# mcveanlab/mccortex

Measured on AMD Instinct MI355X. Metric: k-mers/s inserted (build), k=31, 50M x 150bp synthetic reads, higher is better.
Workload: dtype u64

## Files before the change

### include/mcx_gpu.h

```cpp
#ifndef MCX_GPU_H_
#define MCX_GPU_H_

#include <stddef.h>
#include <stdint.h>

#ifdef __cplusplus
extern "C" {
#endif

typedef enum {
  MCX_OK = 0,
  MCX_ERR_ARG = -1,
  MCX_ERR_NODEVICE = -2,
  MCX_ERR_NOMEM = -3,
  MCX_ERR_FULL = -4,
  MCX_ERR_HIP = -5,
  MCX_ERR_SINK = -6
} mcx_status;

typedef struct {
  uint64_t num_se_reads;
  uint64_t num_good_reads;
  uint64_t num_bad_reads;
  uint64_t total_bases_read;
// ... 132 lines not shown
  uint64_t num_kmers_found;
} mcx_touch_stats;
int mcx_graph_reads_touch(mcx_graph *g, const uint8_t *bases, const uint64_t *read_offsets, uint64_t nreads,
                          uint8_t *hit , mcx_touch_stats *stats_accum );
int mcx_graph_reads_touch_stream_dev(mcx_graph *g, const void *d_stream, uint64_t nbytes,
                                     const void *d_stream_off , uint64_t nreads, void *d_hit);

enum { MCX_INFER_POP = 1, MCX_INFER_PRESENCE_COVG = 2 };
int mcx_graph_infer_edges(mcx_graph *g, void *recs, uint64_t nrecs, int ncols, uint32_t flags, uint64_t *nmodified);
int mcx_graph_infer_edges_dev(mcx_graph *g, void *d_recs, uint64_t nrecs, int ncols, uint32_t flags, uint64_t *nmodified);

int mcx_graph_kmer_covg(mcx_graph *g, uint64_t *nkmers, uint64_t *sumcov);
int mcx_graph_covg_histogram(mcx_graph *g, uint64_t *hist, uint32_t nbins);

int mcx_graph_checksum(mcx_graph *g, uint64_t *checksum, uint64_t *nkmers);
uint64_t mcx_records_checksum(const void *recs, uint64_t nrecs, int kmer_size, int ncols);

int mcx_ubench_stream(int device, uint64_t bytes, double *copy_gbs, double *read_gbs, double *write_gbs);
int mcx_ubench_random_rmw(int device, uint64_t table_bytes, uint64_t nupdates, double *rmw_per_s,
                          double *load16_per_s, double *load_rmw_per_s);

int mcx_sort_records(void *recs, uint64_t nrecs, int kmer_size, int ncols, int device);
int mcx_records_sorted(const void *recs, uint64_t nrecs, int kmer_size, int ncols, int device,
                       int64_t *first_unsorted);

int mcx_superk_supported(int kmer_size);
int mcx_superk_record_bytes(int kmer_size);
uint32_t mcx_superk_owner(const uint64_t *key_words, int kmer_size, int nparts);
int mcx_graph_superk_layout(mcx_graph *g, int nparts, uint64_t positions_per_call, uint32_t *segs_per_owner,
                            uint64_t *seg_cap);
int mcx_graph_superk_bins_dev(mcx_graph *g, const void *d_stream, uint64_t nbytes, int nparts, void *d_recs,
                              void *d_counts, uint64_t seg_cap);
int mcx_graph_add_superk_dev(mcx_graph *g, int colour, const void *d_recs, const void *d_counts, uint32_t nseg,
                             uint64_t seg_cap, uint64_t kmers_upper_bound);

void mcx_pack_bases(const uint8_t *src, uint64_t n, uint32_t *code, uint16_t *inv);

uint64_t mcx_pack_reads_host(const uint8_t *bases, const uint64_t *off, uint64_t nreads, uint32_t *code,
                             uint16_t *inv, uint64_t cap_pos, int fused);

int mcx_graph_sync(mcx_graph *g);

int mcx_graph_nkmers(mcx_graph *g, uint64_t *n);
int mcx_graph_device_stats(mcx_graph *g, mcx_load_stats *out);

typedef struct {
  uint64_t fallback_inserts;
  uint64_t foreign_inserts;
  uint64_t spilled;
  uint64_t flushes;
} mcx_insert_stats;
int mcx_graph_insert_stats(mcx_graph *g, mcx_insert_stats *out);

void *mcx_graph_stream(mcx_graph *g);

typedef int (*mcx_sink_fn)(void *ctx, const void *records, size_t nbytes);
int mcx_graph_export(mcx_graph *g, int sorted, mcx_sink_fn sink, void *ctx);

enum { MCX_UNITIGS_FASTA = 0, MCX_UNITIGS_GFA = 1, MCX_UNITIGS_DOT = 2 };
enum { MCX_UNITIGS_POINTS = 1 };
#define MCX_UNITIGS_BYTES_PER_KMER 65
#define MCX_UNITIGS_BYTES_PER_UNITIG 170
typedef struct { uint64_t num_unitigs, num_kmers, num_bytes, num_cycles; } mcx_unitigs_stats;
typedef struct {
  uint64_t *keys;
  uint32_t *unitig, *rank;
  uint8_t *orient;
  uint32_t *first, *length;
} mcx_unitigs_arrays;
int mcx_graph_unitigs(mcx_graph *g, int format, uint32_t flags, mcx_sink_fn sink, void *ctx, mcx_unitigs_stats *stats);
int mcx_graph_unitigs_dev(mcx_graph *g, const mcx_unitigs_arrays *out, mcx_unitigs_stats *stats);

void mcx_kmer_from_str(const char *seq, int kmer_size, uint64_t *words_out);
void mcx_kmer_canonical(const uint64_t *words_in, int kmer_size, uint64_t *key_out, int *orient_out);
uint32_t mcx_kmer_hash(const uint64_t *key_words, int kmer_size, uint32_t initval);

#ifdef __cplusplus
}
#endif
#endif
```

### mccortex_amd/csrc/mcx_api.hip

```cpp
#include <hip/hip_runtime.h>

#include <stdarg.h>
#include <stdio.h>
#include <stdlib.h>
#include <string.h>
#include <cstring>

#include <rocprim/device/device_radix_sort.hpp>
#include <rocprim/device/device_scan.hpp>

#include <algorithm>
#include <array>
#include <cmath>
#include <memory>
#include <vector>
#include <thread>
#include <atomic>
#include <chrono>
#include <mutex>
#include <condition_variable>
#include <functional>

#include "../../include/mcx_gpu.h"
#include "mcx_kernels.h"
// ... 112 lines not shown
constexpr uint64_t kCarry = 128;
constexpr uint32_t kL1Sets = 32;
static uint64_t stage_bytes()
{
  static uint64_t v = 0;
  if (!v) {
    const char *e = getenv("MCX_STAGE_BYTES");
    v = e ? strtoull(e, nullptr, 10) : (128ull << 20);
    if (v < 1024) v = 1024;
    v = (v + 63) / 64 * 64;
  }
  return v;
}
#define kStageBytes stage_bytes()

struct mcx_group;
struct mcx_graph {
  int k = 0, W = 0, ncols = 0, device = 0;
  hipStream_t stream = nullptr;
  TableView t{};
  uint64_t table_bytes = 0;
  uint64_t touch_bytes = 0;
  Counters *d_ctr = nullptr;
  Counters *h_ctr = nullptr;
  uint32_t *h_full = nullptr;
  static constexpr int kStageBufs = 3;
  uint8_t *h_stage[kStageBufs] = {nullptr, nullptr, nullptr};
  uint8_t *d_stage[kStageBufs] = {nullptr, nullptr, nullptr};
  hipEvent_t ev[kStageBufs] = {nullptr, nullptr, nullptr};
  hipStream_t cstream = nullptr;
  hipEvent_t ev_copy[kStageBufs] = {nullptr, nullptr, nullptr}, ev_wait0[kStageBufs] = {nullptr, nullptr, nullptr}, ev_wait1[kStageBufs] = {nullptr, nullptr, nullptr};
  bool ev_wait_used[kStageBufs] = {false, false, false};
  uint64_t stage_alloc = 0;
  int cur = 0;
  int grid = 0;
  uint64_t unitigs_chunk = 0;
  int grid_stream = 0, grid_split = 0, grid_insert = 0;
  bool defer = true;
  uint64_t defer_tuples = 0;
  uint32_t nsub = 0;
  uint32_t b1 = 0, subs_per_bin = 0;
  uint64_t cap1 = 0, cap2 = 0;
  uint32_t rep1 = 8;
  bool rep1_forced = false;
  uint64_t *l1_keys = nullptr, *l2_keys = nullptr;
  uint64_t *l2_hi = nullptr;
  uint64_t l2_hi_off = 0;
  uint64_t *l2_base = nullptr;
  int place_tries = 1;
  uint64_t l2_off = 0;
  hipStream_t stream2 = nullptr;
  hipEvent_t ev_split[2] = {nullptr, nullptr}, ev_ins[2] = {nullptr, nullptr};
  unsigned long long *l1_cnt = nullptr, *l2_cnt = nullptr;
  uint32_t nsets = 1;
  uint64_t set_cap = 0;
  std::vector<int> set_colour;
  std::vector<uint64_t> set_pending;
  uint64_t pending = 0;
  uint64_t pending_l2 = 0;
  uint32_t l2_regions = 0;
  uint32_t flush_regions = 0;
  uint32_t idle_next = 0;
  uint64_t idle_base = 0;
  std::vector<uint64_t> idle_mark;
  static constexpr uint32_t kSnap = 32;
  struct Snap { uint64_t ub; int set; int which; bool is_base; hipEvent_t ev; };
  Counters *h_snap = nullptr;
  Snap snap[kSnap] = {};
  uint32_t snap_head = 0, snap_tail = 0;
  uint64_t snap_last[2] = {0, 0};
  bool snap_base_known = true;
  uint64_t n_flushes = 0;
  int hidden = -1;
  int ncols_vis = 0;
  uint32_t *d_readstrt = nullptr;
  bool must_exist = false;
  int pending_colour = 0;
  bool profile = false;
  int overlap = -1;
  struct Span { const char *name; hipEvent_t a, b; };
  std::vector<Span> spans;
  mcx_group *group = nullptr;
  int gidx = 0;
  mcx_group *as_group = nullptr;
  uint32_t own_lbo = 0;
  unsigned long long *d_infer = nullptr;
  struct CleanCache *clean = nullptr;
  struct SubgraphState *subgraph = nullptr;
  uint32_t subgraph_narrow = 0;
  unsigned long long *d_rt_cnt = nullptr;
  uint64_t *d_rt_mask = nullptr;
  uint64_t rt_mask_bytes = 0;
  uint64_t reads_chunk = 0;
};

static uint8_t *touch_base(const mcx_graph *g) { return reinterpret_cast<uint8_t *>(g->t.touch) - kTouchHdr; }

static OwnerSpec owner_spec(const mcx_graph *g)
{
  if (g->own_lbo) return OwnerSpec{2u, g->own_lbo, (uint32_t)g->gidx, g->k};
  return OwnerSpec{g->t.lbo ? 1u : 0u, 0u, 0u, g->k};
}

static int flush_deferred(mcx_graph *g);
static void free_defer(mcx_graph *g);
static void snap_push(mcx_graph *g, bool is_base);
// ... 67 lines not shown
  while (lb1 < lb1_max && (2ull << lb1) <= nsub) lb1++;
  while (lb1 < 11 && ((nsub + (1ull << lb1) - 1) >> lb1) > (uint64_t)kMaxBins) lb1++;
  return lb1;
}

extern "C" int mcx_graph_create_shard(mcx_graph **out, int kmer_size, int ncols, uint64_t capacity_kmers, int device,
                                      int nparts, int part)
{
  if (!out) return fail(MCX_ERR_ARG, "null handle pointer");
  *out = nullptr;
  if (check_k(kmer_size) != MCX_OK) return MCX_ERR_ARG;
  if (nparts < 1 || nparts > 32 || (nparts & (nparts - 1)) || part < 0 || part >= nparts)
    return fail(MCX_ERR_ARG, "shards must be a power of two <= 32 and 0 <= part < shards (got %d of %d)", part, nparts);
  if (ncols < 1 || ncols > 4096) return fail(MCX_ERR_ARG, "ncols out of range: %d", ncols);
  if (kmer_size > 63 && nparts != 1)
    return fail(MCX_ERR_ARG, "k > 63 (three- and four-word keys) builds on one device: the exchange formats carry at most two key words");
  int ndev = 0;
  if (hipGetDeviceCount(&ndev) != hipSuccess || ndev <= 0)
    return fail(MCX_ERR_NODEVICE, "no HIP device available (this library has no CPU path)");
  if (device < 0 || device >= ndev) return fail(MCX_ERR_NODEVICE, "device %d out of range (%d devices)", device, ndev);
  HIP_TRY(hipSetDevice(device));

  mcx_graph *g = new mcx_graph();
  g->k = kmer_size;
  g->W = words_for_k(kmer_size);
  g->ncols = ncols;
  g->ncols_vis = ncols;
  g->device = device;
  const uint64_t sub_slots = 1ull << sub_shift_for_words(g->W);
  uint64_t nsub = (std::max<uint64_t>(capacity_kmers, 1024) + sub_slots - 1) / sub_slots;
  uint32_t lbo = 0;
  while ((1 << lbo) < nparts) lbo++;
  uint32_t lb1 = region_bits(nsub, lbo);
  if (const char *e = getenv("MCX_LB1")) { const uint32_t v = (uint32_t)atoi(e); if (!lbo && v >= 6 && v <= 11 && ((nsub + (1ull << v) - 1) >> v) <= (uint64_t)kMaxBins && ((nsub + (1ull << v) - 1) >> v) >= 1) lb1 = v; }
  if (lbo && lb1 + lbo > 11) {
    const uint64_t max_slots = ((uint64_t)kMaxBins << (11 - lbo)) * sub_slots;
    delete g;
    return fail(MCX_ERR_ARG, "capacity per device too large for a table split over %d devices: %llu slots requested, at most %llu "
                "(use more devices or a smaller -n / -m)", nparts, (unsigned long long)(nsub * sub_slots), (unsigned long long)max_slots);
  }
  const uint64_t spb = (nsub + (1ull << lb1) - 1) >> lb1;
  nsub = spb << lb1;
  if (nsub >= (1ull << 31)) { delete g; return fail(MCX_ERR_ARG, "capacity too large"); }
  uint64_t novf = std::max<uint64_t>(sub_slots, (nsub * sub_slots / 32 + sub_slots - 1) / sub_slots * sub_slots);
  if (const char *e = getenv("MCX_OVERFLOW_SLOTS")) novf = strtoull(e, nullptr, 10) / kBucket * kBucket;
  if (novf / kBucket >= (1ull << 32)) novf = ((1ull << 32) - 1) * kBucket;
  const uint64_t slots = nsub * sub_slots + novf;
  g->t.nmain = nsub * sub_slots;
  g->t.nslots = slots;
  g->t.lb1 = lb1;
  g->t.lbo = lbo;
  g->t.part = (uint32_t)part;
  g->t.spb = (uint32_t)spb;
  g->t.S = (uint32_t)(g->W + ncols);
  g->t.max_probe = (uint32_t)sub_slots;
  { const char *e = getenv("MCX_DEFER"); if (e) g->defer = atoi(e) != 0; }
  if (g->W > 2) g->defer = false;
  { const char *e = getenv("MCX_GRID_STREAM"); if (e) g->grid_stream = atoi(e); }
  { const char *e = getenv("MCX_REP1"); if (e && atoi(e) >= 1 && atoi(e) <= 4096) { g->rep1 = (uint32_t)atoi(e); g->rep1_forced = true; } }
  { const char *e = getenv("MCX_GRID_SPLIT"); if (e) g->grid_split = atoi(e); }
  { const char *e = getenv("MCX_GRID_INSERT"); if (e) g->grid_insert = atoi(e); }
  g->table_bytes = slots * g->t.S * 8;

  hipDeviceProp_t prop;
  HIP_TRY(hipGetDeviceProperties(&prop, device));
  g->grid = prop.multiProcessorCount * 8;

#define CREATE_TRY(expr)                                                            \
  do {                                                                              \
    hipError_t _e = (expr);                                                         \
    if (_e != hipSuccess) {                                                         \
      int rc = fail(_e == hipErrorOutOfMemory ? MCX_ERR_NOMEM : MCX_ERR_HIP, "%s: %s", #expr, hipGetErrorString(_e)); \
      mcx_graph_destroy(g);                                                         \
      return rc;                                                                    \
    }                                                                               \
  } while (0)
  CREATE_TRY(hipStreamCreateWithFlags(&g->stream, hipStreamNonBlocking));
  CREATE_TRY(hipMalloc((void **)&g->t.rec, g->table_bytes));
  if (ncols == 1) {
    g->t.KS = g->t.VS = (uint32_t)(g->W + 1);
    g->t.val = g->t.rec + g->W;
    g->t.VC = 0;
  } else {
    g->t.KS = (uint32_t)g->W;
    g->t.VS = 1;
    g->t.val = g->t.rec + g->t.nslots * (uint64_t)g->W;
    g->t.VC = g->t.nslots;
  }
  CREATE_TRY(hipMalloc((void **)&g->d_ctr, sizeof(Counters)));
  CREATE_TRY(hipHostMalloc((void **)&g->h_ctr, sizeof(Counters), hipHostMallocDefault));
  CREATE_TRY(hipHostMalloc((void **)&g->h_full, sizeof(uint32_t), hipHostMallocDefault));
  *g->h_full = 0;
  g->touch_bytes = (1 + ((g->t.nmain >> sub_shift_for_words(g->W)) + 31) / 32) * 4;
  {
    uint8_t *tb = nullptr;
    CREATE_TRY(hipMalloc((void **)&tb, kTouchHdr + g->touch_bytes));
    g->t.touch = reinterpret_cast<uint32_t *>(tb + kTouchHdr);
  }
  CREATE_TRY(hipMemsetAsync(g->t.rec, 0, g->table_bytes, g->stream));
  CREATE_TRY(hipMemsetAsync(touch_base(g), 0, kTouchHdr + g->touch_bytes, g->stream));
  CREATE_TRY(hipMemsetAsync(g->d_ctr, 0, sizeof(Counters), g->stream));
  CREATE_TRY(hipStreamSynchronize(g->stream));
#undef CREATE_TRY
  *out = g;
  return MCX_OK;
}

static void clean_drop(mcx_graph *g);
static void subgraph_drop(mcx_graph *g);

// ... 4 lines not shown
  (void)hipSetDevice(g->device);
  if (g->stream) (void)hipStreamSynchronize(g->stream);
  if (g->cstream) { (void)hipStreamSynchronize(g->cstream); (void)hipStreamDestroy(g->cstream); }
  for (int i = 0; i < mcx_graph::kStageBufs; i++) {
    if (g->h_stage[i]) (void)hipHostFree(g->h_stage[i]);
    if (g->d_stage[i]) (void)hipFree(g->d_stage[i]);
    if (g->ev[i]) (void)hipEventDestroy(g->ev[i]);
    if (g->ev_copy[i]) (void)hipEventDestroy(g->ev_copy[i]);
    if (g->ev_wait0[i]) (void)hipEventDestroy(g->ev_wait0[i]);
    if (g->ev_wait1[i]) (void)hipEventDestroy(g->ev_wait1[i]);
  }
  free_defer(g);
  for (auto &sp : g->spans) { (void)hipEventDestroy(sp.a); (void)hipEventDestroy(sp.b); }
  if (g->t.rec) (void)hipFree(g->t.rec);
  if (g->t.touch) (void)hipFree(touch_base(g));
  if (g->stream2) {
    (void)hipStreamDestroy(g->stream2);
    for (int i = 0; i < 2; i++) { (void)hipEventDestroy(g->ev_split[i]); (void)hipEventDestroy(g->ev_ins[i]); }
  }
  if (g->d_ctr) (void)hipFree(g->d_ctr);
  if (g->d_readstrt) (void)hipFree(g->d_readstrt);
  if (g->d_infer) (void)hipFree(g->d_infer);
  if (g->d_rt_cnt) (void)hipFree(g->d_rt_cnt);
  if (g->d_rt_mask) (void)hipFree(g->d_rt_mask);
  clean_drop(g);
  subgraph_drop(g);
  if (g->h_ctr) (void)hipHostFree(g->h_ctr);
  if (g->h_full) (void)hipHostFree(g->h_full);
  if (g->h_snap) {
    (void)hipHostFree(g->h_snap);
    for (uint32_t i = 0; i < mcx_graph::kSnap; i++) (void)hipEventDestroy(g->snap[i].ev);
  }
  if (g->stream) (void)hipStreamDestroy(g->stream);
  delete g;
}

extern "C" int mcx_graph_reset(mcx_graph *g)
{
  if (g && g->as_group) {
    int rc = grp_drain(g->as_group);
    for (int i = 0; rc == MCX_OK && i < grp_n(g->as_group); i++) rc = mcx_graph_reset(grp_part(g->as_group, i));
    return rc;
  }
  if (!g) return fail(MCX_ERR_ARG, "null graph");
  HIP_TRY(hipSetDevice(g->device));
  clean_drop(g);
  subgraph_drop(g);
  HIP_TRY(hipMemsetAsync(g->t.rec, 0, g->table_bytes, g->stream));
  HIP_TRY(hipMemsetAsync(touch_base(g), 0, kTouchHdr + g->touch_bytes, g->stream));
  HIP_TRY(hipMemsetAsync(g->d_ctr, 0, sizeof(Counters), g->stream));
  g->n_flushes = 0;
  if (g->h_full) { HIP_TRY(hipStreamSynchronize(g->stream)); *g->h_full = 0; }
  if (g->l1_cnt) HIP_TRY(hipMemsetAsync(g->l1_cnt, 0, (size_t)g->nsets * g->b1 * g->rep1 * 8, g->stream));
  if (g->l2_cnt) HIP_TRY(hipMemsetAsync(g->l2_cnt, 0, (size_t)g->l2_regions * g->subs_per_bin * 8, g->stream));
  if (g->d_readstrt) HIP_TRY(hipMemsetAsync(g->d_readstrt, 0xff, g->t.nslots * 8, g->stream));
  g->pending = g->pending_l2 = 0;
  g->idle_next = 0; g->idle_base = 0; g->idle_mark.clear();
  sets_release(g);
  snap_push(g, true);
  return MCX_OK;
}

extern "C" int mcx_graph_capacity(const mcx_graph *g, uint64_t *slots, uint64_t *bytes)
{
  if (g && g->as_group) {
    uint64_t s_ = 0, b_ = 0;
    for (int i = 0; i < grp_n(g->as_group); i++) { uint64_t s1 = 0, b1 = 0; mcx_graph_capacity(grp_part(g->as_group, i), &s1, &b1); s_ += s1; b_ += b1; }
    if (slots) *slots = s_;
    if (bytes) *bytes = b_;
    return MCX_OK;
  }
  if (!g) return fail(MCX_ERR_ARG, "null graph");
  if (slots) *slots = g->t.nslots;
  if (bytes) *bytes = g->table_bytes;
  return MCX_OK;
}

extern "C" void *mcx_graph_stream(mcx_graph *g) { return !g ? nullptr : g->as_group ? (void *)grp_part(g->as_group, 0)->stream : (void *)g->stream; }

struct StreamLaunch {
  const uint8_t *stream;
  uint64_t nbytes, pos_lo, pos_hi;
  unsigned char *flag;
  const uint32_t *code = nullptr;
  const uint16_t *inv = nullptr;
};

#define DISPATCH_WC(g, F, ...)                                                        \
  do {                                                                                \
    if ((g)->W == 1) { if ((g)->ncols == 1) F<1, true>(__VA_ARGS__); else F<1, false>(__VA_ARGS__); } \
    else { if ((g)->ncols == 1) F<2, true>(__VA_ARGS__); else F<2, false>(__VA_ARGS__); }            \
  } while (0)

#define DISPATCH_WC4(g, F, ...)                                                       \
  do {                                                                                \
    const bool one_ = (g)->ncols == 1;                                                \
    switch ((g)->W) {                                                                 \
      case 1: if (one_) F<1, true>(__VA_ARGS__); else F<1, false>(__VA_ARGS__); break; \
      case 2: if (one_) F<2, true>(__VA_ARGS__); else F<2, false>(__VA_ARGS__); break; \
      case 3: if (one_) F<3, true>(__VA_ARGS__); else F<3, false>(__VA_ARGS__); break; \
      default: if (one_) F<4, true>(__VA_ARGS__); else F<4, false>(__VA_ARGS__); break; \
    }                                                                                 \
  } while (0)
#define LAUNCH_W4(W_, KERNEL, ...)                                       \
  do {                                                                   \
    switch (W_) {                                                        \
      case 1: hipLaunchKernelGGL((KERNEL<1>), __VA_ARGS__); break;       \
// ... 75 lines not shown
{
  InsertSink<W, ONECOL> is{g->t, (uint32_t)colour};
  static bool once_dev[64] = {false};
  bool &once = once_dev[g->device & 63];
  if (!once) {
    allow_lds(k_stream_bin<W, ONECOL, 512, FULL, SH, PK>, sizeof(BinLds<W, 512, FULL>));
    allow_lds(k_stream_bin<W, ONECOL, 1024, FULL, SH, PK>, sizeof(BinLds<W, 1024, FULL>));
    allow_lds(k_stream_bin<W, ONECOL, kMaxBins, FULL, SH, PK>, sizeof(BinLds<W, kMaxBins, FULL>));
    once = true;
  }
  SpanGuard sp(g, "k_stream_bin");
  if constexpr (W == 1 && !FULL && SH == 0) {
    static const int fc_cap = [] { const char *e = getenv("MCX_STREAM_FC"); return e ? atoi(e) : 0; }();
    if (fc_cap && bs.nlocal <= 512) {
      const dim3 gridf((unsigned)std::min<uint64_t>(nt, (uint64_t)(g->grid_stream ? g->grid_stream : g->grid)));
#define MCX_FC_LAUNCH(CAPV, PRIVV) { \
        static bool once_f[64] = {false}; \
        if (!once_f[g->device & 63]) { allow_lds(k_stream_fc<ONECOL, PK, CAPV, PRIVV>, sizeof(FcLds<CAPV>)); once_f[g->device & 63] = true; } \
        hipLaunchKernelGGL((k_stream_fc<ONECOL, PK, CAPV, PRIVV>), gridf, dim3(kThreads), sizeof(FcLds<CAPV>), g->stream, a, bs, out, is); }
      if (bs.rep >= gridf.x && bs.rep > 8) MCX_FC_LAUNCH(10, true)
      else MCX_FC_LAUNCH(10, false)
#undef MCX_FC_LAUNCH
      return;
    }
    static const bool wide = [] { const char *e = getenv("MCX_STREAM_T"); return !e || atoi(e) == 512; }();
    if (wide && bs.nlocal <= 512) {
      using GeoW = Geo<512, 512 * kPosPerLane>;
      static bool once_w[64] = {false};
      if (!once_w[g->device & 63]) { allow_lds(k_stream_bin<W, ONECOL, 512, FULL, SH, PK, 512>, sizeof(BinLds<W, 512, FULL, GeoW>)); once_w[g->device & 63] = true; }
      const dim3 gridw((unsigned)std::min<uint64_t>((nt + 1) / 2, (uint64_t)(g->grid_stream ? g->grid_stream : g->grid)));
      hipLaunchKernelGGL((k_stream_bin<W, ONECOL, 512, FULL, SH, PK, 512>), gridw, dim3(512), sizeof(BinLds<W, 512, FULL, GeoW>), g->stream, a, bs, out, is);
      return;
    }
  }
  const dim3 grid((unsigned)std::min<uint64_t>(nt, (uint64_t)(g->grid_stream ? g->grid_stream : g->grid)));
  if (bs.nlocal <= 512)
    hipLaunchKernelGGL((k_stream_bin<W, ONECOL, 512, FULL, SH, PK>), grid, dim3(kThreads), sizeof(BinLds<W, 512, FULL>), g->stream, a, bs, out, is);
  else if (bs.nlocal <= 1024)
    hipLaunchKernelGGL((k_stream_bin<W, ONECOL, 1024, FULL, SH, PK>), grid, dim3(kThreads), sizeof(BinLds<W, 1024, FULL>), g->stream, a, bs, out, is);
  else
    hipLaunchKernelGGL((k_stream_bin<W, ONECOL, kMaxBins, FULL, SH, PK>), grid, dim3(kThreads), sizeof(BinLds<W, kMaxBins, FULL>), g->stream, a, bs, out, is);
}

template <int W, bool ONECOL, bool FULL, int SH>
static void launch_bin_stream_t(mcx_graph *g, const StreamLaunch &L, int colour, BinSpec bs, BinOut out)
{
  const StreamArgs a = make_args(g, L);
  const uint64_t nt = a.ntiles > a.tile0 ? a.ntiles - a.tile0 : 0;
  if (!nt) return;
  if (!FULL && a.code) launch_bin_stream_pk<W, ONECOL, FULL, SH, !FULL>(g, a, nt, colour, bs, out);
  else launch_bin_stream_pk<W, ONECOL, FULL, SH, false>(g, a, nt, colour, bs, out);
}

template <int W, bool ONECOL, bool IN_FULL, bool SHARD>
static void launch_bin_tuples_t(mcx_graph *g, TupleIn in, int colour, BinSpec bs, BinOut out)
{
  constexpr bool kWide = W == 1 && !IN_FULL;
  static const bool wide = kWide && [] { const char *e = getenv("MCX_SPLIT_T"); return !e || atoi(e) == 512; }();
  const bool use_wide = wide && bs.nlocal <= 1024;
  const bool use_huge = wide && !use_wide && bs.nlocal <= (uint32_t)kMaxBins;
  const uint64_t tile = use_huge ? 1024 * 16 : use_wide ? 512 * 16 : kTile;
  const uint64_t nchunks = (in.seg_cap + tile - 1) / tile * in.nseg;
  if (!nchunks) return;
  InsertSink<W, ONECOL> is{g->t, (uint32_t)colour};
  using GeoW = Geo<512, 512 * 16>;
  static bool once_dev[64] = {false};
  bool &once = once_dev[g->device & 63];
  if (!once) {
    allow_lds(k_tuples_bin<W, ONECOL, 512, IN_FULL, SHARD>, sizeof(BinLds<W, 512, false>));
    allow_lds(k_tuples_bin<W, ONECOL, 1024, IN_FULL, SHARD>, sizeof(BinLds<W, 1024, false>));
    allow_lds(k_tuples_bin<W, ONECOL, kMaxBins, IN_FULL, SHARD>, sizeof(BinLds<W, kMaxBins, false>));
    if constexpr (kWide) allow_lds(k_tuples_bin<W, ONECOL, 512, IN_FULL, SHARD, 512>, sizeof(BinLds<W, 512, false, GeoW>));
    if constexpr (kWide) allow_lds(k_tuples_bin<W, ONECOL, 1024, IN_FULL, SHARD, 512>, sizeof(BinLds<W, 1024, false, GeoW>));
    if constexpr (kWide) allow_lds(k_tuples_bin<W, ONECOL, kMaxBins, IN_FULL, SHARD, 1024>, sizeof(BinLds<W, kMaxBins, false, Geo<1024, 1024 * 16>>));
    once = true;
  }
  SpanGuard sp(g, "k_tuples_bin");
  const uint64_t gmax = (uint64_t)(g->grid_split ? g->grid_split : g->grid * 4);
  if constexpr (kWide) {
    if (use_huge) {
      using GeoH = Geo<1024, 1024 * 16>;
      const dim3 gridh((unsigned)std::min<uint64_t>(nchunks, g->grid_split ? gmax : gmax / 4));
      hipLaunchKernelGGL((k_tuples_bin<W, ONECOL, kMaxBins, IN_FULL, SHARD, 1024>), gridh, dim3(1024), sizeof(BinLds<W, kMaxBins, false, GeoH>), g->stream, in, bs, out, is, g->d_ctr);
      return;
    }
    if (use_wide) {
      const dim3 gridw((unsigned)std::min<uint64_t>(nchunks, g->grid_split ? gmax : gmax / 2));
      if (bs.nlocal <= 512)
        hipLaunchKernelGGL((k_tuples_bin<W, ONECOL, 512, IN_FULL, SHARD, 512>), gridw, dim3(512), sizeof(BinLds<W, 512, false, GeoW>), g->stream, in, bs, out, is, g->d_ctr);
      else
        hipLaunchKernelGGL((k_tuples_bin<W, ONECOL, 1024, IN_FULL, SHARD, 512>), gridw, dim3(512), sizeof(BinLds<W, 1024, false, GeoW>), g->stream, in, bs, out, is, g->d_ctr);
      return;
    }
  }
  const dim3 grid((unsigned)std::min<uint64_t>(nchunks, gmax));
  if (bs.nlocal <= 512)
    hipLaunchKernelGGL((k_tuples_bin<W, ONECOL, 512, IN_FULL, SHARD>), grid, dim3(kThreads), sizeof(BinLds<W, 512, false>), g->stream, in, bs, out, is, g->d_ctr);
  else if (bs.nlocal <= 1024)
    hipLaunchKernelGGL((k_tuples_bin<W, ONECOL, 1024, IN_FULL, SHARD>), grid, dim3(kThreads), sizeof(BinLds<W, 1024, false>), g->stream, in, bs, out, is, g->d_ctr);
  else
    hipLaunchKernelGGL((k_tuples_bin<W, ONECOL, kMaxBins, IN_FULL, SHARD>), grid, dim3(kThreads), sizeof(BinLds<W, kMaxBins, false>), g->stream, in, bs, out, is, g->d_ctr);
}
template <int W, bool ONECOL> static void launch_bin_region_stream(mcx_graph *g, const StreamLaunch &L, int colour, BinSpec bs, BinOut out)
{
  if (g->t.lbo) launch_bin_stream_t<W, ONECOL, false, 1>(g, L, colour, bs, out);
  else launch_bin_stream_t<W, ONECOL, false, 0>(g, L, colour, bs, out);
}
template <int W, bool ONECOL> static void launch_split_regions(mcx_graph *g, TupleIn in, int colour, BinSpec bs, BinOut out)
{ launch_bin_tuples_t<W, ONECOL, false, false>(g, in, colour, bs, out); }
template <int W, bool ONECOL> static void launch_bin_received(mcx_graph *g, TupleIn in, int colour, BinSpec bs, BinOut out)
{
  if (g->t.lbo) launch_bin_tuples_t<W, ONECOL, true, true>(g, in, colour, bs, out);
  else launch_bin_tuples_t<W, ONECOL, true, false>(g, in, colour, bs, out);
}

static uint64_t *l2_ptr(const mcx_graph *g, uint64_t off)
{
  if (g->l2_hi && off >= g->l2_hi_off) return g->l2_hi + (off - g->l2_hi_off) * g->cap2 * g->W;
  return g->l2_keys + off * g->cap2 * g->W;
}

template <int W, bool ONECOL> static void launch_lds_insert_t(mcx_graph *g, int colour, uint32_t sub0, uint32_t nsub)
{
  const size_t lds = Sub<W>::kSlots * (W + 1) * 8 + LdsQueue<W>::kTuples * 8 * W;
  static bool once_dev[64] = {false};
  bool &once = once_dev[g->device & 63];
  if (!once) { allow_lds(k_lds_insert<W, ONECOL>, lds); once = true; }
  BinOut bins{l2_ptr(g, g->l2_off), nullptr, g->l2_cnt + g->l2_off, g->cap2, nullptr, nullptr, nullptr, 0};
  SpanGuard sp(g, "k_lds_insert");
  hipLaunchKernelGGL((k_lds_insert<W, ONECOL>), dim3((unsigned)std::min<uint64_t>(nsub, (uint64_t)(g->grid_insert ? g->grid_insert : g->grid * 4))),
                     dim3(LdsCfg<W>::kThreads), lds, g->stream, g->t, (uint32_t)colour, bins, sub0, nsub, g->d_ctr);
}

template <int W, bool ONECOL>
static void launch_insert_tuples_t(mcx_graph *g, int colour, const uint64_t *keys, const uint8_t *edges, uint64_t n, uint32_t only_own = 0)
{
  const int grid = (int)std::min<uint64_t>((n + kThreads * kBatch - 1) / (kThreads * kBatch), (uint64_t)g->grid);
  InsertSink<W, ONECOL> s{g->t, (uint32_t)colour};
  SpanGuard sp(g, "k_insert_tuples");
  hipLaunchKernelGGL((k_insert_tuples<W, ONECOL>), dim3(grid), dim3(kThreads), 0, g->stream, s, keys, edges, n, g->d_ctr, only_own);
}

static void free_defer(mcx_graph *g)
{
  (void)hipFree(g->l1_keys); (void)hipFree(g->l1_cnt);
  (void)hipFree(g->l2_base); (void)hipFree(g->l2_hi); (void)hipFree(g->l2_cnt);
  g->l1_keys = g->l2_keys = g->l2_base = g->l2_hi = nullptr; g->l1_cnt = g->l2_cnt = nullptr;
  g->cap1 = g->cap2 = 0;
  g->l2_regions = 0;
  g->set_colour.clear(); g->set_pending.clear();
}

__global__ __launch_bounds__(512) void k_l2_probe(uint64_t *keys, uint64_t cap, uint32_t nregions, uint32_t spb, uint32_t iters,
                                                  uint32_t jit_mask = 0 )
{
  const uint32_t region = blockIdx.x % nregions, blk = blockIdx.x / nregions, nblk = gridDim.x / nregions;
  const uint32_t w = threadIdx.x >> 6, l = threadIdx.x & 63u;
  for (uint32_t it = 0; it < iters; it++)
    for (uint32_t k = 0; k < spb / 32u; k++) {
      const uint32_t front = w * 4u + (l >> 4) + 32u * k;
      const uint32_t seg = region * spb + front;
      const uint64_t jit = ((seg * 0x9E3779B1u) >> 8) & jit_mask & ~15u;
      const uint64_t at = (uint64_t)seg * cap + jit + ((uint64_t)it * nblk + blk) * 16u + (l & 15u);
      if (jit + ((uint64_t)it * nblk + blk) * 16u + 16u <= cap) keys[at] = at;
    }
}

static uint64_t *l2_place(mcx_graph *g, size_t bytes, uint32_t nreg, int tries, float *ms_out)
{
  std::vector<uint64_t *> cand;
  std::vector<float> ms;
  hipEvent_t e0 = nullptr, e1 = nullptr;
  if (tries > 1 && (hipEventCreate(&e0) != hipSuccess || hipEventCreate(&e1) != hipSuccess)) { (void)hipGetLastError(); tries = 1; }
  const uint32_t iters = (uint32_t)std::max<uint64_t>(8, g->cap2 * g->W / 1024);
  for (int i = 0; i < std::max(tries, 1); i++) {
    if (i > 0) {
      size_t fr = 0, tot = 0;
      if (hipMemGetInfo(&fr, &tot) != hipSuccess || fr < bytes + (size_t)(tot / 16)) { (void)hipGetLastError(); break; }
    }
    uint64_t *p = nullptr;
    if (hipMalloc((void **)&p, bytes) != hipSuccess) { (void)hipGetLastError(); break; }
    cand.push_back(p);
    float t = 0.f;
    if (tries > 1)
      for (int rep = 0; rep < 2; rep++) {
        (void)hipEventRecord(e0, g->stream);
        hipLaunchKernelGGL(k_l2_probe, dim3(nreg * 64), dim3(512), 0, g->stream, p, g->cap2 * g->W, nreg, g->subs_per_bin, iters);
        (void)hipEventRecord(e1, g->stream);
        if (hipEventSynchronize(e1) != hipSuccess || hipEventElapsedTime(&t, e0, e1) != hipSuccess) { (void)hipGetLastError(); t = 0.f; }
      }
    ms.push_back(t);
    float worst = 0.f, best_t = 0.f;
    for (float x : ms) { worst = std::max(worst, x); if (x > 0.f && (best_t == 0.f || x < best_t)) best_t = x; }
    if (tries > 1 && best_t > 0.f && best_t < 0.70f * worst) break;
  }
  if (e0) (void)hipEventDestroy(e0);
  if (e1) (void)hipEventDestroy(e1);
  if (cand.empty()) return nullptr;
  size_t best = 0;
  for (size_t i = 1; i < cand.size(); i++) if (ms[i] > 0.f && (ms[best] <= 0.f || ms[i] < ms[best])) best = i;
  for (size_t i = 0; i < cand.size(); i++) if (i != best) (void)hipFree(cand[i]);
  if (getenv("MCX_TIMING") && cand.size() > 1) {
    fprintf(stderr, "[timing] sub-table bins (%u regions): %zu placements probed:", nreg, cand.size());
    for (size_t i = 0; i < cand.size(); i++) fprintf(stderr, " %.3f%s", ms[i], i == best ? "*" : "");
    fprintf(stderr, " ms\n");
  }
  if (ms_out) *ms_out = ms[best];
  return cand[best];
}

static uint32_t flush_group(const mcx_graph *g);
static int ensure_l2(mcx_graph *g, uint32_t regions, bool whole = false)
{
  if (g->l2_keys && g->l2_regions >= regions && !(g->l2_hi && (whole || (regions > g->l2_regions / 2 && regions != g->l2_regions)))) return MCX_OK;
  if (g->pending_l2) return fail(MCX_ERR_ARG, "internal: sub-table bins resized while in use");
  HIP_TRY(hipStreamSynchronize(g->stream));
  (void)hipFree(g->l2_base); (void)hipFree(g->l2_hi); (void)hipFree(g->l2_cnt);
  g->l2_keys = g->l2_base = g->l2_hi = nullptr; g->l2_cnt = nullptr; g->l2_regions = 0; g->l2_hi_off = 0;
  const uint64_t nb = (uint64_t)regions * g->subs_per_bin;
  int tries = g->place_tries;
  { const char *e = getenv("MCX_PLACE_BINS"); if (e) tries = atoi(e); }
  if (g->subs_per_bin % 32 || regions < 8) tries = 1;
  const uint32_t G = flush_group(g);
  const bool halves = !whole && tries > 1 && regions == 2 * G && !g->t.lbo && !g->group;
  if (halves) {
    const size_t hbytes = (nb / 2) * g->cap2 * 8 * g->W;
    g->l2_base = l2_place(g, hbytes, G, tries, nullptr);
    if (g->l2_base) g->l2_hi = l2_place(g, hbytes, G, tries, nullptr);
    if (g->l2_base && !g->l2_hi) { (void)hipFree(g->l2_base); g->l2_base = nullptr; }
    g->l2_hi_off = nb / 2;
  } else {
    g->l2_base = l2_place(g, nb * g->cap2 * 8 * g->W, std::min<uint32_t>(regions, 32), tries, nullptr);
  }
  if (!g->l2_base || hipMalloc((void **)&g->l2_cnt, nb * 8) != hipSuccess) {
    (void)hipGetLastError();
    (void)hipFree(g->l2_base); (void)hipFree(g->l2_hi); g->l2_base = g->l2_hi = nullptr;
    return fail(MCX_ERR_NOMEM, "out of device memory for the sub-table bins (%llu regions)", (unsigned long long)regions);
  }
  HIP_TRY(hipMemsetAsync(g->l2_cnt, 0, nb * 8, g->stream));
  g->l2_keys = g->l2_base;
  g->l2_regions = regions;
  return MCX_OK;
}

static bool flush_overlap(const mcx_graph *g)
{
  static const bool on = [] { const char *e = getenv("MCX_FLUSH_OVERLAP"); return !e || atoi(e) != 0; }();
  return g->overlap < 0 ? on : g->overlap != 0;
}

static uint32_t flush_group(const mcx_graph *g)
{
  uint32_t G = g->flush_regions;
  if (!G) {
    const char *e = getenv("MCX_FLUSH_REGIONS");
    G = e ? (uint32_t)strtoul(e, nullptr, 10) : 0;
  }
  if (!G) G = std::max<uint32_t>(32u, 16384u / std::max<uint32_t>(1u, g->subs_per_bin));
  return std::min<uint32_t>(G, g->b1);
}

static int ensure_defer(mcx_graph *g)
{
  if (g->l1_keys) return MCX_OK;
  g->nsub = (uint32_t)(g->t.nmain >> sub_shift_for_words(g->W));
  g->b1 = 1u << g->t.lb1;
  g->subs_per_bin = g->t.spb;
  if (g->t.lb1 < 6 || g->b1 > (uint32_t)kMaxBins || g->subs_per_bin > (uint32_t)kMaxBins) { g->defer = false; return MCX_OK; }
  uint64_t tcap = g->defer_tuples;
  if (!tcap) {
    const char *e = getenv("MCX_DEFER_TUPLES");
    if (e) {
      tcap = strtoull(e, nullptr, 10);
    } else {
      size_t fr = 0, tot = 0;
      (void)hipMemGetInfo(&fr, &tot);
      const uint64_t per_tuple = 8ull * g->W * (g->t.lbo ? 240 : 118) / 100 + 1;
      const uint64_t by_mem = (uint64_t)((double)fr * 0.40) / per_tuple;
      tcap = std::max<uint64_t>(std::min<uint64_t>(std::min<uint64_t>(64 * g->t.nslots, by_mem), 1ull << 33), 1ull << 20);
    }
  }
  for (;; tcap /= 2) {
    if (tcap < (1ull << 20)) { g->defer = false; g->defer_tuples = 0; (void)hipGetLastError(); return MCX_OK; }
    g->defer_tuples = tcap;
    g->nsets = g->ncols > 1 ? kL1Sets : 1;
    if (const char *e = getenv("MCX_L1_SETS")) { const int v = atoi(e); if (v >= 1 && v <= 32) g->nsets = (uint32_t)v; }
    g->set_cap = tcap / g->nsets;
    if (!g->rep1_forced) g->rep1 = g->nsets != 1 ? 8 : g->set_cap / g->b1 / 64 >= (1u << 16) ? 64 : g->set_cap / g->b1 / 32 >= (1u << 16) ? 32 : 8;
    g->cap1 = (uint64_t)((double)g->set_cap / g->b1 / g->rep1 * (g->b1 == 1 ? 1.02 : 1.06)) + (g->nsets > 1 ? 2048 : 8192);
    static const double cap2_slack = [] { const char *e = getenv("MCX_CAP2_SLACK"); const double v = e ? atof(e) : 0; return v >= 1.0 && v <= 4.0 ? v : 1.25; }();
    g->cap2 = g->nsub == 1 ? tcap + 8192 : (uint64_t)((double)tcap / g->nsub * cap2_slack) + 1024;
    g->cap1 = (g->cap1 + 1) & ~1ull;
    g->cap2 = (g->cap2 + 1) & ~1ull;
    if (g->cap1 >= 0xFFFFFFFFull || g->cap2 >= 0xFFFFFFFFull) continue;
    const uint64_t n1 = (uint64_t)g->nsets * g->b1 * g->rep1 * g->cap1;
    const bool ok = hipMalloc((void **)&g->l1_keys, n1 * 8 * g->W) == hipSuccess &&
                    hipMalloc((void **)&g->l1_cnt, (size_t)g->nsets * g->b1 * g->rep1 * 8) == hipSuccess &&
                    ensure_l2(g, flush_overlap(g) ? std::min<uint32_t>(2 * flush_group(g), g->b1) : flush_group(g)) == MCX_OK;
    if (ok) break;
    free_defer(g);
    (void)hipGetLastError();
  }
  HIP_TRY(hipMemsetAsync(g->l1_cnt, 0, (size_t)g->nsets * g->b1 * g->rep1 * 8, g->stream));
  g->set_colour.assign(g->nsets, -1);
  g->set_pending.assign(g->nsets, 0);
  return MCX_OK;
}

static BinOut l1_out(const mcx_graph *g, int set)
{
  const uint64_t segs = (uint64_t)g->b1 * g->rep1;
  return BinOut{g->l1_keys + (uint64_t)set * segs * g->cap1 * g->W, nullptr, g->l1_cnt + (uint64_t)set * segs, g->cap1, nullptr, nullptr, nullptr, 0};
}

static int ensure_flush_stream(mcx_graph *g)
{
  if (g->stream2) return MCX_OK;
  HIP_TRY(hipStreamCreateWithFlags(&g->stream2, hipStreamNonBlocking));
  for (int i = 0; i < 2; i++) {
    if (!g->ev_split[i]) HIP_TRY(hipEventCreateWithFlags(&g->ev_split[i], hipEventDisableTiming));
    if (!g->ev_ins[i]) HIP_TRY(hipEventCreateWithFlags(&g->ev_ins[i], hipEventDisableTiming));
  }
  return MCX_OK;
}

static int flush_deferred(mcx_graph *g)
{
  if (!g->pending && !g->pending_l2) {
    sets_release(g);
    if (!g->idle_mark.empty()) {
      g->idle_next = 0; g->idle_base = 0; g->idle_mark.clear();
      snap_push(g, true);
    }
    return MCX_OK;
  }
  HIP_TRY(hipSetDevice(g->device));
  const uint32_t G = g->pending_l2 ? g->b1 : std::min(flush_group(g), g->l2_regions);
  if (g->pending_l2 && g->l2_regions < g->b1) return fail(MCX_ERR_ARG, "internal: split tuples without bins");
  const bool overlap = flush_overlap(g) && g->pending && !g->pending_l2 && g->l2_regions >= 2 * G && G < g->b1;
  hipStream_t s1 = g->stream;
  if (overlap) {
    int rc2 = ensure_flush_stream(g);
    if (rc2 != MCX_OK) return rc2;
    HIP_TRY(hipEventRecord(g->ev_split[0], s1));
    HIP_TRY(hipStreamWaitEvent(g->stream2, g->ev_split[0], 0));
  }
  std::vector<int> colours;
  if (g->pending_l2) colours.push_back(g->pending_colour);
  for (uint32_t s = 0; s < g->nsets && g->pending; s++) {
    const int c = g->set_colour[s];
    if (c >= 0 && g->set_pending[s] && std::find(colours.begin(), colours.end(), c) == colours.end()) colours.push_back(c);
  }
  uint32_t gi = 0;
  for (size_t ci = 0; ci < colours.size(); ci++) {
    const int colour = colours[ci];
    TupleIn in{};
    uint32_t nmine = 0;
    for (uint32_t s = 0; s < g->nsets && g->pending; s++)
      if (g->set_colour[s] == colour && g->set_pending[s]) in.set_map[nmine++] = (uint8_t)s;
    for (uint32_t r0 = 0; r0 < g->b1; r0 += G, gi++) {
      const uint32_t ng = std::min(G, g->b1 - r0);
      const int hb = overlap ? (int)(gi & 1u) : 0;
      g->l2_off = (uint64_t)hb * G * g->subs_per_bin;
      if (overlap && gi >= 2) HIP_TRY(hipStreamWaitEvent(s1, g->ev_ins[hb], 0));
      if (nmine) {
        in.keys = g->l1_keys + (uint64_t)r0 * g->cap1 * g->W;
        in.edges = nullptr;
        in.counts = g->l1_cnt + r0;
        in.seg_cap = g->cap1;
        in.nseg = ng * g->rep1 * nmine;
        in.seg_group = ng;
        in.seg_stride = g->b1;
        in.set_rep = g->nsets > 1 ? g->rep1 : 0;
        BinSpec bs{BIN_SUBLOCAL, 0, g->subs_per_bin, 1, ng * g->subs_per_bin, ng, 0, r0};
        BinOut out{l2_ptr(g, g->l2_off), nullptr, g->l2_cnt + g->l2_off, g->cap2, nullptr, nullptr, nullptr, 0};
        DISPATCH_WC(g, launch_split_regions, g, in, colour, bs, out);
        HIP_TRY(hipGetLastError());
      }
      if (overlap) {
        HIP_TRY(hipEventRecord(g->ev_split[hb], s1));
        HIP_TRY(hipStreamWaitEvent(g->stream2, g->ev_split[hb], 0));
        g->stream = g->stream2;
      }
      DISPATCH_WC(g, launch_lds_insert_t, g, colour, r0 * g->subs_per_bin, ng * g->subs_per_bin);
      g->stream = s1;
      HIP_TRY(hipGetLastError());
      if (overlap) HIP_TRY(hipEventRecord(g->ev_ins[hb], g->stream2));
    }
  }
  g->l2_off = 0;
  if (overlap)
    for (int i = 0; i < 2; i++) HIP_TRY(hipStreamWaitEvent(s1, g->ev_ins[i], 0));
  if (g->pending) HIP_TRY(hipMemsetAsync(g->l1_cnt, 0, (size_t)g->nsets * g->b1 * g->rep1 * 8, g->stream));
  g->pending = 0;
  g->pending_l2 = 0;
  g->n_flushes++;
  g->idle_next = 0; g->idle_base = 0; g->idle_mark.clear();
  sets_release(g);
  snap_push(g, true);
  return MCX_OK;
}

static void snap_push(mcx_graph *g, bool is_base, uint64_t ub, int set, int which)
{
  if (!g->h_snap) {
    if (hipHostMalloc((void **)&g->h_snap, sizeof(Counters) * mcx_graph::kSnap, hipHostMallocDefault) != hipSuccess) { (void)hipGetLastError(); g->h_snap = nullptr; return; }
    for (uint32_t i = 0; i < mcx_graph::kSnap; i++)
      if (hipEventCreateWithFlags(&g->snap[i].ev, hipEventDisableTiming) != hipSuccess) {
        (void)hipGetLastError();
        for (uint32_t j = 0; j < i; j++) { (void)hipEventDestroy(g->snap[j].ev); g->snap[j].ev = nullptr; }
        (void)hipHostFree(g->h_snap);
        g->h_snap = nullptr;
        return;
      }
  }
  if (is_base) {
    g->snap_tail = g->snap_head;
    g->snap_base_known = false;
  }
  if (g->snap_head - g->snap_tail >= mcx_graph::kSnap) return;
  const uint32_t i = g->snap_head % mcx_graph::kSnap;
  if (hipMemcpyAsync(&g->h_snap[i], g->d_ctr, sizeof(Counters), hipMemcpyDeviceToHost, g->stream) != hipSuccess ||
      hipEventRecord(g->snap[i].ev, g->stream) != hipSuccess) { (void)hipGetLastError(); return; }
  g->snap[i].ub = ub;
  g->snap[i].set = set;
  g->snap[i].which = which;
  g->snap[i].is_base = is_base;
  g->snap_head++;
}
static void snap_push(mcx_graph *g, bool is_base) { snap_push(g, is_base, 0, 0, 0); }

static void snap_poll(mcx_graph *g)
{
  if (!g->h_snap) return;
  while (g->snap_tail != g->snap_head) {
    const uint32_t i = g->snap_tail % mcx_graph::kSnap;
    if (hipEventQuery(g->snap[i].ev) != hipSuccess) { (void)hipGetLastError(); break; }
    const uint64_t v[2] = {g->h_snap[i].kmers, g->h_snap[i].binned};
    const mcx_graph::Snap &e = g->snap[i];
    if (e.is_base) {
      g->snap_base_known = true;
    } else if (g->snap_base_known && g->idle_mark.empty() && (size_t)e.set < g->set_pending.size()) {
      const uint64_t yielded = std::min<uint64_t>(e.ub, v[e.which] - g->snap_last[e.which]);
      const uint64_t d = e.ub - yielded;
      g->pending -= std::min(g->pending, d);
      g->set_pending[e.set] -= std::min(g->set_pending[e.set], d);
    }
    g->snap_last[0] = v[0];
    g->snap_last[1] = v[1];
    g->snap_tail++;
  }
}

static bool defer_has_room(const mcx_graph *g, int colour, uint64_t need)
{
  for (uint32_t s = 0; s < g->nsets; s++)
    if (g->set_colour[s] < 0 || (g->set_colour[s] == colour && g->set_pending[s] + need <= g->set_cap)) return true;
  return false;
}
static void settle_for_room(mcx_graph *g, int colour, uint64_t need)
{
  if (!g->h_snap) return;
  while (!defer_has_room(g, colour, need) && g->snap_tail != g->snap_head) {
    if (hipEventSynchronize(g->snap[g->snap_tail % mcx_graph::kSnap].ev) != hipSuccess) { (void)hipGetLastError(); return; }
    const uint32_t before = g->snap_tail;
    snap_poll(g);
    if (g->snap_tail == before) return;
  }
}

static int defer_reserve(mcx_graph *g, int colour, uint64_t ub, int *set_out = nullptr)
{
  if (set_out) *set_out = 0;
  int rc = ensure_defer(g);
  if (rc != MCX_OK || !g->defer) return rc;
  snap_poll(g);
  settle_for_room(g, colour, ub);
  for (int pass = 0; pass < 2; pass++) {
    int free_set = -1;
    for (uint32_t s = 0; s < g->nsets; s++) {
      if (g->set_colour[s] == colour && g->set_pending[s] + ub <= g->set_cap) {
        g->set_pending[s] += ub; g->pending += ub;
        if (set_out) *set_out = (int)s;
        return MCX_OK;
      }
      if (g->set_colour[s] < 0 && free_set < 0) free_set = (int)s;
    }
    if (free_set >= 0) {
      g->set_colour[free_set] = colour;
      g->set_pending[free_set] = ub; g->pending += ub;
      if (set_out) *set_out = free_set;
      return MCX_OK;
    }
    rc = flush_deferred(g);
    if (rc != MCX_OK) return rc;
  }
  return fail(MCX_ERR_ARG, "internal: no L1 bin set after a flush");
}

static int l2_reserve(mcx_graph *g, int colour, uint64_t ub)
{
  int rc = ensure_defer(g);
  if (rc != MCX_OK || !g->defer) return rc;
  if ((g->pending_l2 && colour != g->pending_colour) ||
      ((g->pending_l2 || g->pending) && g->pending_l2 + g->pending + ub > g->defer_tuples)) {
    rc = flush_deferred(g);
    if (rc != MCX_OK) return rc;
  }
  g->pending_colour = colour;
  return MCX_OK;
}

static int full_poll(mcx_graph *g)
{
  if (!g->h_full || !g->t.touch) return MCX_OK;
  if (*g->h_full) return fail(MCX_ERR_FULL, "Hash table is full");
  HIP_TRY(hipMemcpyAsync(g->h_full, g->t.touch - 2, sizeof(uint32_t), hipMemcpyDeviceToHost, g->stream));
  return MCX_OK;
}

static int submit_stream(mcx_graph *g, const StreamLaunch &L, int colour)
{
  if (g->group) return group_submit_stream(g->group, g->gidx, L, colour);
  { int rc = full_poll(g); if (rc != MCX_OK) return rc; }
  if (g->defer) { int rc = ensure_defer(g); if (rc != MCX_OK) return rc; }
  if (!g->defer) {
    DISPATCH_WC4(g, launch_direct_t, g, L, colour);
    HIP_TRY(hipGetLastError());
    return MCX_OK;
  }
  snap_poll(g);
  for (uint64_t lo = L.pos_lo; lo < L.pos_hi;) {
    settle_for_room(g, colour, std::min<uint64_t>(L.pos_hi - lo, g->set_cap));
    uint64_t room = g->set_cap;
    for (uint32_t s = 0; s < g->nsets; s++)
      if (g->set_colour[s] == colour && g->set_pending[s] < g->set_cap) { room = g->set_cap - g->set_pending[s]; break; }
    if (room < (uint64_t)kTile * 16 && room < L.pos_hi - lo) room = g->set_cap;
    const uint64_t hi = std::min(L.pos_hi, lo + room);
    int set = 0;
    int rc = defer_reserve(g, colour, hi - lo, &set);
    if (rc != MCX_OK) return rc;
    StreamLaunch P = L;
    P.pos_lo = lo; P.pos_hi = hi;
    BinSpec bs{BIN_GROUP, 0, g->b1, g->rep1, g->b1, 1, 0, 0};
    BinOut out = l1_out(g, set);
    DISPATCH_WC(g, launch_bin_region_stream, g, P, colour, bs, out);
    HIP_TRY(hipGetLastError());
    snap_push(g, false, hi - lo, set, 0);
    lo = hi;
  }
  return MCX_OK;
}

static int ensure_stage(mcx_graph *g);



extern "C" int mcx_graph_configure(mcx_graph *g, const char *key, uint64_t value)
{
  if (g && key && g->as_group) {
    const bool isec = !strcmp(key, "intersect");
    if (isec && g->ncols < 2) return fail(MCX_ERR_ARG, "intersect mode needs one colour more than the output has");
    if (!strcmp(key, "defer") && !value) return fail(MCX_ERR_ARG, "a multi-GPU table always uses the partitioned insert");
    int rc = grp_drain(g->as_group);
    for (int i = 0; rc == MCX_OK && i < grp_n(g->as_group); i++) rc = mcx_graph_configure(grp_part(g->as_group, i), key, value);
    if (isec && rc == MCX_OK) {
      g->hidden = g->ncols - 1;
      g->ncols_vis = g->ncols - 1;
    }
    return rc;
  }
  if (!g || !key) return fail(MCX_ERR_ARG, "null argument");
  HIP_TRY(hipSetDevice(g->device));
  if (!strcmp(key, "defer")) {
    int rc = flush_deferred(g);
    if (rc != MCX_OK) return rc;
    g->defer = value != 0 && g->W <= 2;
    return MCX_OK;
  }
  if (!strcmp(key, "debug_realloc_l2")) {
    int rc = flush_deferred(g);
    if (rc != MCX_OK) return rc;
    if (!g->l2_keys || g->l2_hi) return MCX_OK;
    HIP_TRY(hipStreamSynchronize(g->stream));
    if (g->stream2) HIP_TRY(hipStreamSynchronize(g->stream2));
    static std::vector<void *> holes;
    void *hole = nullptr;
    if (value && hipMalloc(&hole, value) == hipSuccess) holes.push_back(hole);
    uint64_t *nk = nullptr;
    HIP_TRY(hipMalloc((void **)&nk, (uint64_t)g->l2_regions * g->subs_per_bin * g->cap2 * 8 * g->W));
    (void)hipFree(g->l2_base);
    g->l2_base = g->l2_keys = nk;
    return MCX_OK;
  }
  if (!strcmp(key, "place_bins")) {
    if (value < 1 || value > 32) return fail(MCX_ERR_ARG, "place_bins: 1..32");
    g->place_tries = (int)value;
    return MCX_OK;
  }
  if (!strcmp(key, "defer_tuples")) {
    int rc = flush_deferred(g);
    if (rc != MCX_OK) return rc;
    HIP_TRY(hipStreamSynchronize(g->stream));
    free_defer(g);
    g->defer_tuples = value;
    return MCX_OK;
  }
  if (!strcmp(key, "flush_overlap")) {
    int rc = flush_deferred(g);
    if (rc != MCX_OK) return rc;
    HIP_TRY(hipStreamSynchronize(g->stream));
    g->overlap = value != 0;
    if (g->l1_keys && g->overlap) return ensure_l2(g, std::min<uint32_t>(2 * flush_group(g), g->b1));
    return MCX_OK;
  }
  if (!strcmp(key, "flush_regions")) {
    int rc = flush_deferred(g);
    if (rc != MCX_OK) return rc;
    g->flush_regions = (uint32_t)value;
    if (g->l1_keys) return ensure_l2(g, flush_group(g));
    return MCX_OK;
  }
  if (!strcmp(key, "intersect")) {
    if (!value) return fail(MCX_ERR_ARG, "intersect mode cannot be switched off");
    if (g->ncols < 2) return fail(MCX_ERR_ARG, "intersect mode needs one colour more than the output has");
    HIP_TRY(hipStreamSynchronize(g->stream));
    g->hidden = g->ncols - 1;
    g->ncols_vis = g->ncols - 1;
    g->defer = false;
    return MCX_OK;
  }
  if (!strcmp(key, "must_exist")) {
    int rc = flush_deferred(g);
    if (rc != MCX_OK) return rc;
    g->must_exist = value != 0;
    if (g->must_exist) g->defer = false;
    return MCX_OK;
  }
  if (!strcmp(key, "prepare")) {
    const double t0 = now_s();
    int rc = ensure_stage(g);
    const double t1 = now_s();
    if (rc == MCX_OK && g->defer && !g->must_exist) rc = ensure_defer(g);
    const double t2 = now_s();
    if (rc == MCX_OK && g->defer && !g->must_exist && flush_overlap(g)) rc = ensure_flush_stream(g);
    if (getenv("MCX_TIMING"))
      fprintf(stderr, "[timing] prepare: pinned staging + copy stream %.1f ms, partition workspace (%.1f GB) %.1f ms, flush stream %.1f ms\n", (t1 - t0) * 1e3,
// ... 105 lines not shown
  if (!npos) return MCX_OK;
  if (g->must_exist) return fail(MCX_ERR_ARG, "device streams cannot be loaded in must-exist mode");
  HIP_TRY(hipSetDevice(g->device));
  StreamLaunch L{nullptr, npos, 0, npos, nullptr, (const uint32_t *)d_code, (const uint16_t *)d_inv};
  return submit_stream(g, L, colour);
}

extern "C" int mcx_graph_partition_stream_dev(mcx_graph *g, const void *d_stream, uint64_t nbytes, int nparts,
                                              uint64_t bin_capacity, void *d_keys, void *d_edges, void *d_counts)
{
  NO_GROUP(g, "mcx_graph_partition_stream_dev");
  if (!g) return fail(MCX_ERR_ARG, "null graph");
  NO_WIDE(g, "mcx_graph_partition_stream_dev");
  if (nparts < 1 || nparts > kMaxBins) return fail(MCX_ERR_ARG, "nparts must be 1..%d", kMaxBins);
  if (bin_capacity >= 0xFFFFFFFFull) return fail(MCX_ERR_ARG, "bin capacity must be below 2^32 tuples");
  if (((uintptr_t)d_stream & 15) != 0) return fail(MCX_ERR_ARG, "stream must be 16-byte aligned");
  if (!nbytes) return MCX_OK;
  HIP_TRY(hipSetDevice(g->device));
  StreamLaunch L{(const uint8_t *)d_stream, nbytes, 0, nbytes, nullptr};
  BinSpec bs{BIN_OWNER, (uint32_t)nparts, (uint32_t)nparts, 1, (uint32_t)nparts, 1, 0, 0};
  BinOut out{(uint64_t *)d_keys, (uint8_t *)d_edges, (unsigned long long *)d_counts, bin_capacity, nullptr, nullptr, nullptr, 0};
  if (g->W == 1) launch_bin_stream_t<1, true, true, 0>(g, L, 0, bs, out);
  else launch_bin_stream_t<2, true, true, 0>(g, L, 0, bs, out);
  HIP_TRY(hipGetLastError());
  return MCX_OK;
}

extern "C" int mcx_graph_insert_tuples_dev(mcx_graph *g, int colour, const void *d_keys, const void *d_edges, uint64_t n)
{
  NO_GROUP(g, "mcx_graph_insert_tuples_dev");
  if (!g) return fail(MCX_ERR_ARG, "null graph");
  if (colour < 0 || colour >= g->ncols) return fail(MCX_ERR_ARG, "colour %d out of range", colour);
  if (!n) return MCX_OK;
  HIP_TRY(hipSetDevice(g->device));
  if (g->defer) { int rc = ensure_defer(g); if (rc != MCX_OK) return rc; }
  if (!g->defer) {
    DISPATCH_WC4(g, launch_insert_tuples_t, g, colour, (const uint64_t *)d_keys, (const uint8_t *)d_edges, n);
    HIP_TRY(hipGetLastError());
    return MCX_OK;
  }
  for (uint64_t lo = 0; lo < n;) {
    const uint64_t cnt = std::min(n - lo, g->set_cap);
    int set = 0;
    int rc = defer_reserve(g, colour, cnt, &set);
    if (rc != MCX_OK) return rc;
    TupleIn in{(const uint64_t *)d_keys + lo * g->W, (const uint8_t *)d_edges + lo, nullptr, cnt, 1, 1, 1};
    BinSpec bs{BIN_GROUP, 0, g->b1, g->rep1, g->b1, 1, 0, 0};
    BinOut out = l1_out(g, set);
    DISPATCH_WC(g, launch_bin_received, g, in, colour, bs, out);
    HIP_TRY(hipGetLastError());
    lo += cnt;
  }
  return MCX_OK;
}

extern "C" int mcx_debug_probe(void *d_buf, uint64_t cap_words, uint32_t nregions, uint32_t spb, uint32_t iters, uint32_t jit_mask, float *ms_out)
{
  hipEvent_t e0, e1;
  HIP_TRY(hipEventCreate(&e0)); HIP_TRY(hipEventCreate(&e1));
  float t = 0.f;
  for (int rep = 0; rep < 2; rep++) {
    (void)hipEventRecord(e0, 0);
    hipLaunchKernelGGL(k_l2_probe, dim3(nregions * 64), dim3(512), 0, 0, (uint64_t *)d_buf, cap_words, nregions, spb, iters, jit_mask);
    (void)hipEventRecord(e1, 0);
    HIP_TRY(hipEventSynchronize(e1));
    HIP_TRY(hipEventElapsedTime(&t, e0, e1));
  }
  (void)hipEventDestroy(e0); (void)hipEventDestroy(e1);
  if (ms_out) *ms_out = t;
  return MCX_OK;
}

template <int W> __global__ void k_hashtest_keys(uint64_t *keys, uint64_t first, uint64_t n)
{
  for (uint64_t i = (uint64_t)blockIdx.x * blockDim.x + threadIdx.x; i < n; i += (uint64_t)gridDim.x * blockDim.x) {
    keys[i * W] = first + i;
    for (int w = 1; w < W; w++) keys[i * W + w] = 0;
  }
}
template <int W> __global__ void k_hashtest_func(uint64_t lo, uint64_t hi, unsigned int *out)
{
  uint32_t h = 0;
  for (uint64_t i = lo + (uint64_t)blockIdx.x * blockDim.x + threadIdx.x; i < hi; i += (uint64_t)gridDim.x * blockDim.x) {
    Kmer<W> key;
    key.w[0] = i;
    for (int w = 1; w < W; w++) key.w[w] = 0;
    h ^= kmer_hash<W>(key, 0, nullptr);
  }
  for (int d = 32; d; d >>= 1) h ^= __shfl_xor(h, d, 64);
  if ((threadIdx.x & 63) == 0 && h) atomicXor(out, h);
}

extern "C" int mcx_graph_hashtest(mcx_graph *g, uint64_t first, uint64_t n)
{
  NO_GROUP(g, "mcx_graph_hashtest");
  if (!g) return fail(MCX_ERR_ARG, "null graph");
  if (first + n < first) return fail(MCX_ERR_ARG, "key range wraps");
  HIP_TRY(hipSetDevice(g->device));
  const uint64_t chunk = std::min<uint64_t>(n, 1ull << 26);
  if (!chunk) return mcx_graph_sync(g);
  uint64_t *d_keys = nullptr;
  uint8_t *d_edges = nullptr;
  if (hipMalloc((void **)&d_keys, chunk * 8 * g->W) != hipSuccess || hipMalloc((void **)&d_edges, chunk) != hipSuccess) {
    (void)hipGetLastError(); (void)hipFree(d_keys); (void)hipFree(d_edges);
    return fail(MCX_ERR_NOMEM, "out of device memory for the hashtest key buffer");
  }
  int rc = MCX_OK;
  if (hipMemsetAsync(d_edges, 0, chunk, g->stream) != hipSuccess) rc = fail(MCX_ERR_HIP, "hipMemsetAsync failed");
  for (uint64_t lo = 0; lo < n && rc == MCX_OK; lo += chunk) {
    const uint64_t cnt = std::min(chunk, n - lo);
    LAUNCH_W4(g->W, k_hashtest_keys, dim3(4096), dim3(256), 0, g->stream, d_keys, first + lo, cnt);
    rc = mcx_graph_insert_tuples_dev(g, 0, d_keys, d_edges, cnt);
  }
  const int rc2 = mcx_graph_sync(g);
  (void)hipFree(d_keys); (void)hipFree(d_edges);
  return rc != MCX_OK ? rc : rc2;
}

extern "C" int mcx_hashtest_func(int device, int kmer_size, uint64_t n, uint32_t nparts, uint64_t *hash_out)
{
  int ndev = 0;
  if (hipGetDeviceCount(&ndev) != hipSuccess || device < 0 || device >= ndev) return fail(MCX_ERR_NODEVICE, "no HIP device %d", device);
  if (kmer_size < 3 || kmer_size > 127 || !(kmer_size & 1)) return fail(MCX_ERR_ARG, "kmer size %d", kmer_size);
  if (!nparts || !hash_out) return fail(MCX_ERR_ARG, "nparts / hash_out");
  HIP_TRY(hipSetDevice(device));
  unsigned int *d = nullptr;
  HIP_TRY(hipMalloc((void **)&d, (size_t)nparts * 4));
  std::vector<unsigned int> h(nparts, 0);
  bool ok = hipMemset(d, 0, (size_t)nparts * 4) == hipSuccess;
  const int W = words_for_k(kmer_size);
  for (uint32_t p = 0; p < nparts && ok; p++) {
    const uint64_t lo = (uint64_t)p * (n / nparts), hi = p + 1 == nparts ? n : lo + n / nparts;
    if (hi <= lo) continue;
    const unsigned grid = (unsigned)std::min<uint64_t>((hi - lo + 255) / 256, 8192);
    LAUNCH_W4(W, k_hashtest_func, dim3(grid), dim3(256), 0, 0, lo, hi, d + p);
  }
  ok = ok && hipMemcpy(h.data(), d, (size_t)nparts * 4, hipMemcpyDeviceToHost) == hipSuccess;
  (void)hipFree(d);
  if (!ok) { (void)hipGetLastError(); return fail(MCX_ERR_HIP, "hashtest kernels failed"); }
  uint64_t sum = 0;
  for (uint32_t p = 0; p < nparts; p++) sum += h[p];
  *hash_out = sum;
  return MCX_OK;
}

extern "C" int mcx_graph_insert_tuple_segments_dev(mcx_graph *g, int colour, const void *d_keys, const void *d_edges,
                                                   const void *d_counts, uint32_t nseg, uint64_t seg_cap)
{
  NO_GROUP(g, "mcx_graph_insert_tuple_segments_dev");
  if (!g) return fail(MCX_ERR_ARG, "null graph");
  if (colour < 0 || colour >= g->ncols) return fail(MCX_ERR_ARG, "colour %d out of range", colour);
  if (!nseg || !seg_cap) return MCX_OK;
  if (!d_keys || !d_edges || !d_counts) return fail(MCX_ERR_ARG, "null tuple buffers");
  HIP_TRY(hipSetDevice(g->device));
  int rc = ensure_defer(g);
  if (rc != MCX_OK) return rc;
  if (!g->defer) return fail(MCX_ERR_ARG, "tuple segments need the deferred insert path (table too small or defer=0)");
  const uint64_t ub = std::min<uint64_t>((uint64_t)nseg * seg_cap, g->set_cap);
  int set = 0;
  rc = defer_reserve(g, colour, ub, &set);
  if (rc != MCX_OK) return rc;
  TupleIn in{(const uint64_t *)d_keys, (const uint8_t *)d_edges, (const unsigned long long *)d_counts, seg_cap, nseg, nseg, nseg};
  BinSpec bs{BIN_GROUP, 0, g->b1, g->rep1, g->b1, 1, 0, 0};
  BinOut out = l1_out(g, set);
  DISPATCH_WC(g, launch_bin_received, g, in, colour, bs, out);
  HIP_TRY(hipGetLastError());
  return MCX_OK;
}

static const uint32_t kShardRep = 8;

extern "C" int mcx_graph_shard_layout(mcx_graph *g, uint64_t tuples_per_call, uint32_t *segs_per_owner,
                                      uint64_t *seg_cap, uint64_t *ov_cap)
{
  NO_GROUP(g, "mcx_graph_shard_layout");
  if (!g) return fail(MCX_ERR_ARG, "null graph");
  NO_WIDE(g, "mcx_graph_shard_layout");
  const uint32_t nparts = 1u << g->t.lbo, b1 = 1u << g->t.lb1;
  const uint64_t nseg = (uint64_t)nparts * kShardRep * b1;
  if (segs_per_owner) *segs_per_owner = kShardRep * b1;
  if (seg_cap) *seg_cap = (uint64_t)((double)tuples_per_call / (double)nseg * 1.06) + 2048;
  if (ov_cap) *ov_cap = std::max<uint64_t>(1u << 16, tuples_per_call / nparts / 64);
  return MCX_OK;
}

static int shard_bins_launch(mcx_graph *g, const StreamLaunch &L, void *d_keys, void *d_counts, uint64_t seg_cap,
                             void *d_ov_keys, void *d_ov_edges, void *d_ov_counts, uint64_t ov_cap, bool spill = false);

extern "C" int mcx_graph_shard_bins_dev(mcx_graph *g, const void *d_stream, uint64_t nbytes, void *d_keys,
                                        void *d_counts, uint64_t seg_cap, void *d_ov_keys, void *d_ov_edges,
                                        void *d_ov_counts, uint64_t ov_cap)
{
  if (!g) return fail(MCX_ERR_ARG, "null graph");
  NO_WIDE(g, "mcx_graph_shard_bins_dev");
  if (g->as_group) return fail(MCX_ERR_ARG, "device-pointer exchange calls take a shard, not the multi-GPU handle");
  if (!nbytes) return MCX_OK;
  StreamLaunch L{(const uint8_t *)d_stream, nbytes, 0, nbytes, nullptr};
  return shard_bins_launch(g, L, d_keys, d_counts, seg_cap, d_ov_keys, d_ov_edges, d_ov_counts, ov_cap);
}

static int shard_bins_launch(mcx_graph *g, const StreamLaunch &L, void *d_keys, void *d_counts, uint64_t seg_cap,
                             void *d_ov_keys, void *d_ov_edges, void *d_ov_counts, uint64_t ov_cap, bool spill)
{
  if (!L.code && ((uintptr_t)L.stream & 15) != 0) return fail(MCX_ERR_ARG, "stream must be 16-byte aligned");
  if (g->t.lb1 + g->t.lbo > 11) return fail(MCX_ERR_ARG, "too many (owner, region) bins");
  if (seg_cap >= 0xFFFFFFFFull) return fail(MCX_ERR_ARG, "segment capacity must be below 2^32 tuples");
  HIP_TRY(hipSetDevice(g->device));
  const uint32_t nparts = 1u << g->t.lbo, b1 = 1u << g->t.lb1;
  BinSpec bs{BIN_GLOBAL, nparts, nparts * b1, kShardRep, b1, 1, g->t.lb1, spill ? 1u : 0u};
  BinOut out{(uint64_t *)d_keys, nullptr, (unsigned long long *)d_counts, seg_cap,
             (uint64_t *)d_ov_keys, (uint8_t *)d_ov_edges, (unsigned long long *)d_ov_counts, ov_cap};
  if (g->W == 1) launch_bin_stream_t<1, true, false, 2>(g, L, 0, bs, out);
  else launch_bin_stream_t<2, true, false, 2>(g, L, 0, bs, out);
// ... 84 lines not shown
  const StreamArgs a = make_args(g, L);
  const uint64_t nt = a.ntiles > a.tile0 ? a.ntiles - a.tile0 : 0;
  if (!nt) return MCX_OK;
  SpanGuard sp(g, "k_stream_superk");
  const dim3 grid((unsigned)std::min<uint64_t>(nt, (uint64_t)g->grid));
  if (g->W == 1) {
    if (a.code) hipLaunchKernelGGL((k_stream_superk<1, true>), grid, dim3(kThreads), 0, g->stream, a, out);
    else hipLaunchKernelGGL((k_stream_superk<1, false>), grid, dim3(kThreads), 0, g->stream, a, out);
  } else {
    if (a.code) hipLaunchKernelGGL((k_stream_superk<2, true>), grid, dim3(kThreads), 0, g->stream, a, out);
    else hipLaunchKernelGGL((k_stream_superk<2, false>), grid, dim3(kThreads), 0, g->stream, a, out);
  }
  HIP_TRY(hipGetLastError());
  return MCX_OK;
}

template <int W, bool ONECOL> static void launch_superk_bin(mcx_graph *g, SuperkIn in, int colour, BinSpec bs, BinOut out)
{
  const uint64_t nunits = (in.seg_cap + kSkChunk - 1) / kSkChunk * in.nseg;
  InsertSink<W, ONECOL> is{g->t, (uint32_t)colour};
  const size_t lds512 = ((sizeof(BinLds<W, 512, false>) + 15) & ~(size_t)15) + kSkMapBytes;
  const size_t ldsmax = ((sizeof(BinLds<W, kMaxBins, false>) + 15) & ~(size_t)15) + kSkMapBytes;
  static bool once_dev[64] = {false};
  bool &once = once_dev[g->device & 63];
  if (!once) {
    allow_lds(k_superk_bin<W, ONECOL, 512>, lds512);
    allow_lds(k_superk_bin<W, ONECOL, kMaxBins>, ldsmax);
    once = true;
  }
  SpanGuard sp(g, "k_superk_bin");
  const dim3 grid((unsigned)std::min<uint64_t>(nunits, (uint64_t)g->grid * 4));
  if (bs.nlocal <= 512)
    hipLaunchKernelGGL((k_superk_bin<W, ONECOL, 512>), grid, dim3(kThreads), lds512, g->stream, in, g->k, bs, out, is, g->d_ctr);
  else
    hipLaunchKernelGGL((k_superk_bin<W, ONECOL, kMaxBins>), grid, dim3(kThreads), ldsmax, g->stream, in, g->k, bs, out, is, g->d_ctr);
}

extern "C" int mcx_graph_add_superk_dev(mcx_graph *g, int colour, const void *d_recs, const void *d_counts, uint32_t nseg,
                                        uint64_t seg_cap, uint64_t kmers_upper_bound)
{
  NO_GROUP(g, "mcx_graph_add_superk_dev");
  if (!g) return fail(MCX_ERR_ARG, "null graph");
  NO_WIDE(g, "mcx_graph_add_superk_dev");
  if (colour < 0 || colour >= g->ncols_vis) return fail(MCX_ERR_ARG, "colour %d out of range", colour);
  if (!mcx_superk_supported(g->k)) return fail(MCX_ERR_ARG, "super-k-mer records need an odd k in %d..63 (got %d)", kSuperkMinK, g->k);
  if (g->t.lbo) return fail(MCX_ERR_ARG, "super-k-mer shards use ordinary (unsharded) tables");
  if (!nseg || !seg_cap) return MCX_OK;
  HIP_TRY(hipSetDevice(g->device));
  int rc = ensure_defer(g);
  if (rc != MCX_OK) return rc;
  if (!g->defer) return fail(MCX_ERR_ARG, "super-k-mer records need the deferred insert path (table too small or defer=0)");
  int set = 0;
  const uint64_t ub = std::min(kmers_upper_bound, g->set_cap);
  rc = defer_reserve(g, colour, ub, &set);
  if (rc != MCX_OK) return rc;
  SuperkIn in{d_recs, (const unsigned long long *)d_counts, seg_cap, nseg};
  BinSpec bs{BIN_GROUP, 0, g->b1, g->rep1, g->b1, 1, 0, 0};
  BinOut out = l1_out(g, set);
  DISPATCH_WC(g, launch_superk_bin, g, in, colour, bs, out);
  HIP_TRY(hipGetLastError());
  snap_push(g, false, ub, set, 1);
  return MCX_OK;
}

extern "C" uint32_t mcx_graph_key_owner(const mcx_graph *g, const uint64_t *key_words)
{
  if (!g) return 0;
  if (g->as_group) g = grp_part(g->as_group, 0);
  if (g->W > 2) return 0;
  if (g->own_lbo) return g->W == 1 ? superk_owner(0, key_words[0], g->k, g->own_lbo) : superk_owner(key_words[0], key_words[1], g->k, g->own_lbo);
  const uint32_t lbq = g->t.lb1 + g->t.lbo;
  uint32_t r = 0, m;
  if (g->W == 1) {
    m = region_mix<1>(key_quot<1>(Kmer<1>{{key_words[0]}}, lbq, r));
  } else {
    m = region_mix<2>(key_quot<2>(Kmer<2>{{key_words[0], key_words[1]}}, lbq, r));
  }
  return (r ^ mix_g(m, lbq)) >> g->t.lb1;
}

extern "C" uint32_t mcx_key_owner(const uint64_t *key_words, int kmer_size, int nparts)
{
  uint32_t h2 = 0;
  if (words_for_k(kmer_size) == 1) {
    Kmer<1> k{{key_words[0]}};
    kmer_hash<1>(k, 0, &h2);
  } else {
    Kmer<2> k{{key_words[0], key_words[1]}};
    kmer_hash<2>(k, 0, &h2);
  }
  return (uint32_t)(((uint64_t)h2 * (uint32_t)nparts) >> 32);
}

static inline void pack16_swar(const uint8_t *src, uint32_t *code, uint16_t *inv)
{
  uint32_t c = 0, v = 0;
  for (int h = 0; h < 2; h++) {
    uint64_t x;
    memcpy(&x, src + 8 * h, 8);
    const uint64_t t = ((x >> 1) ^ (x >> 2)) & 0x0303030303030303ULL;
    const uint32_t lo = (uint32_t)t, hi = (uint32_t)(t >> 32);
    c = (c << 16) | ((lo * 0x40100401u) >> 24 << 8) | ((hi * 0x40100401u) >> 24);
    const uint64_t u = x & 0xDFDFDFDFDFDFDFDFULL;
#define MCX_NZ64(z) ((((z) & 0x7F7F7F7F7F7F7F7FULL) + 0x7F7F7F7F7F7F7F7FULL) | (z))
    const uint64_t bad = MCX_NZ64(u ^ 0x4141414141414141ULL) & MCX_NZ64(u ^ 0x4343434343434343ULL) &
                         MCX_NZ64(u ^ 0x4747474747474747ULL) & MCX_NZ64(u ^ 0x5454545454545454ULL) & 0x8080808080808080ULL;
#undef MCX_NZ64
// ... 154 lines not shown
    uint8_t sep[kCarry];
    memset(sep, '\n', sizeof(sep));
    pack_block(sep, (size_t)kCarry, code, inv);
    const PackReads PR{bases, off, 0, nreads, kCarry, false, 0, 0};
    uint64_t p = kCarry;
    for (uint64_t step = 64; p < total; step = total > (1u << 24) ? (1u << 18) : step * 3 % 8191 / 64 * 64 + 64) {
      const uint64_t q = std::min(total, p + step);
      pack_reads_avx512(PR, p, q, code, inv);
      p = q;
    }
#endif
    return total;
  }
  std::vector<uint8_t> txt(total, (uint8_t)'\n');
  for (uint64_t i = 0, p = kCarry; i < nreads; i++) {
    const uint64_t len = off[i + 1] - off[i];
    memcpy(txt.data() + p, bases + off[i], len);
    p += len + 1;
  }
  pack_block(txt.data(), (size_t)total, code, inv);
  return total;
}

extern "C" void mcx_pack_bases(const uint8_t *src, uint64_t n, uint32_t *code, uint16_t *inv)
{
  pack_block(src, (size_t)n, code, inv);
}

static int stage_threads()
{
  static const int n = [] {
    const char *e = getenv("MCX_STAGE_THREADS");
    const int hw = (int)std::thread::hardware_concurrency();
    const int v = e ? atoi(e) : std::max(1, std::min(24, hw / 2));
    return v < 1 ? 1 : v > 64 ? 64 : v;
  }();
  return n;
}

struct StageTiming {
  double wait = 0, prep = 0, pack = 0, submit = 0; uint64_t chunks = 0, flushes = 0;
  ~StageTiming() { if (chunks && getenv("MCX_STAGE_TIMING")) fprintf(stderr, "[stage] %llu chunks: wait for buffer %.1f ms, prepare %.1f ms, pack %.1f ms, copy + launches %.1f ms (%llu background flushes)\n",
                                          (unsigned long long)chunks, wait * 1e3, prep * 1e3, pack * 1e3, submit * 1e3, (unsigned long long)flushes); }
};
static StageTiming g_stage_timing;

static int flush_if_device_idle(mcx_graph *g, int starved = -1 )
{
  static const int mode_env = [] { const char *e = getenv("MCX_IDLE_FLUSH"); return e ? atoi(e) : 1; }();
  if (mode_env == 3 && !(g->idle_base || g->pending >= g->defer_tuples / 4 * 3)) return MCX_OK;
  const int mode = mode_env == 3 ? 2 : mode_env;
  const bool on = mode != 0;
  if (!on || !g->defer || g->group || g->nsets != 1 || !g->pending || g->pending_l2 || g->set_colour.empty() || g->set_colour[0] < 0) return MCX_OK;
  const uint32_t G = std::min(flush_group(g), g->l2_regions);
  if (G >= g->b1) return MCX_OK;
  const uint32_t ngroups = (g->b1 + G - 1) / G;
  if (mode != 2 && g->pending / ngroups < std::max<uint64_t>(g->defer_tuples / 8 / ngroups, 1ull << 24)) return MCX_OK;
  if (mode != 2 && starved == 0) return MCX_OK;
  if (mode != 2 && starved < 0 && hipStreamQuery(g->stream) != hipSuccess) { (void)hipGetLastError(); return MCX_OK; }
  const uint32_t r0 = g->idle_next * G < g->b1 ? g->idle_next * G : 0;
  g->idle_next = (r0 / G + 1) % ngroups;
  g_stage_timing.flushes++;
  const uint32_t ng = std::min(G, g->b1 - r0);
  const int colour = g->set_colour[0];
  g->l2_off = 0;
  TupleIn in{g->l1_keys + (uint64_t)r0 * g->cap1 * g->W, nullptr, g->l1_cnt + r0, g->cap1, ng * g->rep1, ng, g->b1};
  BinSpec bs{BIN_SUBLOCAL, 0, g->subs_per_bin, 1, ng * g->subs_per_bin, ng, 0, r0};
  BinOut out{g->l2_keys, nullptr, g->l2_cnt, g->cap2, nullptr, nullptr, nullptr, 0};
  DISPATCH_WC(g, launch_split_regions, g, in, colour, bs, out);
  HIP_TRY(hipGetLastError());
  DISPATCH_WC(g, launch_lds_insert_t, g, colour, r0 * g->subs_per_bin, ng * g->subs_per_bin);
  HIP_TRY(hipGetLastError());
  HIP_TRY(hipMemset2DAsync(g->l1_cnt + r0, (size_t)g->b1 * 8, 0, (size_t)ng * 8, g->rep1, g->stream));
  if (g->idle_mark.size() != ngroups) g->idle_mark.assign(ngroups, g->idle_base);
  g->idle_mark[r0 / G] = g->idle_base + g->pending;
  const uint64_t base = *std::min_element(g->idle_mark.begin(), g->idle_mark.end());
  const uint64_t freed = base - g->idle_base;
  g->idle_base = base;
  g->pending -= std::min(g->pending, freed);
  g->set_pending[0] -= std::min(g->set_pending[0], freed);
  return MCX_OK;
}

static bool stage_packed()
{
  static const bool packed = [] { const char *e = getenv("MCX_PACKED"); return !e || atoi(e) != 0; }();
  return packed;
}
static uint64_t stage_inv_at() { return (((kCarry + kStageBytes + 64) / 16 * 4) + 63) & ~63ull; }
static uint64_t stage_off_region()
{
  if (!stage_packed()) return kCarry + kStageBytes + 256;
  return (stage_inv_at() + (kCarry + kStageBytes + 64) / 16 * 2 + 255) & ~255ull;
}

static int ensure_stage(mcx_graph *g)
{
  if (g->stage_alloc) return MCX_OK;
  const uint64_t bytes = stage_off_region() + (kStageBytes / 16 + 2) * sizeof(uint64_t);
  for (int i = 0; i < mcx_graph::kStageBufs; i++) {
    if (!g->h_stage[i]) HIP_TRY(hipHostMalloc((void **)&g->h_stage[i], bytes, hipHostMallocDefault));
    if (!g->d_stage[i]) HIP_TRY(hipMalloc((void **)&g->d_stage[i], bytes));
    if (!g->ev[i]) HIP_TRY(hipEventCreateWithFlags(&g->ev[i], hipEventDisableTiming));
    if (!g->ev_copy[i]) HIP_TRY(hipEventCreateWithFlags(&g->ev_copy[i], hipEventDisableTiming));
    if (!g->ev_wait0[i]) HIP_TRY(hipEventCreate(&g->ev_wait0[i]));
    if (!g->ev_wait1[i]) HIP_TRY(hipEventCreate(&g->ev_wait1[i]));
  }
  if (!g->cstream) HIP_TRY(hipStreamCreateWithFlags(&g->cstream, hipStreamNonBlocking));
  g->stage_alloc = bytes;
  return MCX_OK;
}

static int add_reads_qh(mcx_graph *g, int colour, const uint8_t *bases, const uint8_t *quals,
                        const uint64_t *off, uint64_t nreads, uint8_t fq, uint8_t hp);
static int add_reads_must_exist(mcx_graph *g, int colour, const uint8_t *bases, const uint8_t *quals,
                                const uint64_t *off, uint64_t nreads, uint8_t fq, uint8_t hp);

static int add_reads_packed(mcx_graph *g, int colour, const uint8_t *bases, const uint64_t *off, uint64_t nreads,
                            unsigned char *d_flags)
{
  const uint64_t off_region = stage_off_region();
// ... 2248 lines not shown
```

### mccortex_amd/csrc/mcx_defer.h

```cpp
#pragma once
#include "mcx_kernels.h"

namespace mcx {

enum : int { BIN_OWNER = 0, BIN_GROUP = 1, BIN_SUBLOCAL = 2, BIN_GLOBAL = 3 };

struct BinSpec {
  int mode;
  uint32_t nparts;
  uint32_t nlocal;
  uint32_t rep;
  uint32_t nout;
  uint32_t seg_mod;
  uint32_t lb1;
  uint32_t region0;
};

__device__ __forceinline__ uint32_t out_seg(const BinSpec &bs, uint32_t ob0, uint32_t b)
{
  if (bs.mode == BIN_GLOBAL)
    return ((((b >> bs.lb1) * bs.rep + blockIdx.x % bs.rep) << bs.lb1) | (b & ((1u << bs.lb1) - 1u)));
  return ob0 + b;
}

struct BinOut {
  uint64_t *keys;
  uint8_t *edges;
  unsigned long long *counts;
  uint64_t cap;
  uint64_t *ov_keys;
  uint8_t *ov_edges;
  unsigned long long *ov_counts;
  uint64_t ov_cap;
};

#define MCX_LDS_AS __attribute__((address_space(3)))

#ifdef MCX_PHASES
__device__ unsigned long long g_phase[3][8];
#define MCX_PH_DECL unsigned long long ph_t = wall_clock64(), ph_acc[8] = {0, 0, 0, 0, 0, 0, 0, 0};
#define MCX_PH(i) { const unsigned long long n_ = wall_clock64(); ph_acc[i] += n_ - ph_t; ph_t = n_; }
#define MCX_PH_COUNT ph_acc[7]++;
#define MCX_PH_DUMP(kid) { if (threadIdx.x == 0) for (int i_ = 0; i_ < 8; i_++) atomicAdd(&g_phase[kid][i_], ph_acc[i_]); }
#else
#define MCX_PH_DECL
#define MCX_PH(i)
#define MCX_PH_COUNT
#define MCX_PH_DUMP(kid)
#endif
constexpr int kMaxBins = 2048;
constexpr uint64_t kQMask = (1ull << 56) - 1;

template <int W> __device__ __forceinline__ Kmer<W> tuple_pack(const Kmer<W> &q, uint32_t e)
{
  Kmer<W> t = q;
  t.w[0] |= (uint64_t)e << 56;
  return t;
}
template <int W> __device__ __forceinline__ Kmer<W> tuple_q(const Kmer<W> &t)
{
  Kmer<W> q = t;
  q.w[0] &= kQMask;
  return q;
}

constexpr int kRounds = 2;
constexpr int kStage = kTile / kRounds;

template <int T_, int TILE_, int R_ = kRounds> struct Geo {
  static constexpr int kT = T_, kTileG = TILE_, kRoundsG = R_, kStageG = TILE_ / R_;
};
using Geo256 = Geo<kThreads, kTile>;

template <int W, int NB, bool FULL, class G = Geo256> struct BinLds {
  using geo = G;
  uint64_t skey[G::kStageG * W];
  unsigned long long gbase[NB];
  uint32_t cnt[NB + 64];
  uint32_t rnk[NB + 64];
  uint32_t off[NB + 64];
  uint32_t wsum[G::kT / 64];
  uint16_t sbin[G::kStageG];
  uint8_t se[FULL ? G::kStageG : 16];
};

__device__ __forceinline__ uint32_t tid_now()
{
  uint32_t t = threadIdx.x;
  asm volatile("" : "+v"(t));
  return t;
}

template <int NB, int T = kThreads> struct BinRes { unsigned long long g0[(NB + T - 1) / T]; };

template <class LDS, int NB>
__device__ __forceinline__ void bin_reserve(LDS &L, const BinSpec &bs, const BinOut &out, uint32_t ob0, BinRes<NB, LDS::geo::kT> &res,
                                            bool trash_beyond = false)
{
  constexpr int kT = LDS::geo::kT;
  const int tid = threadIdx.x;
  __syncthreads();
  {
    constexpr int PERB = NB / kT;
    static_assert(NB % kT == 0, "bins per thread");
    uint32_t c[PERB], x = 0;
#pragma unroll
    for (int i = 0; i < PERB; i++) {
      const uint32_t b = (uint32_t)tid * PERB + i;
      c[i] = b < bs.nlocal ? L.cnt[b] : 0;
      x += c[i];
    }
    const uint32_t mine = x;
#pragma unroll
    for (int d = 1; d < 64; d <<= 1) {
      const uint32_t y = __shfl_up(x, d, 64);
      if ((tid & 63) >= d) x += y;
    }
    if ((tid & 63) == 63) L.wsum[tid >> 6] = x;
    __syncthreads();
    uint32_t before = 0, total = 0;
#pragma unroll
    for (int w = 0; w < kT / 64; w++) {
      const uint32_t ws = L.wsum[w];
      if (w < (tid >> 6)) before += ws;
      total += ws;
    }
    uint32_t o = before + x - mine;
#pragma unroll
    for (int i = 0; i < PERB; i++) {
      const uint32_t b = (uint32_t)tid * PERB + i;
      if (b < bs.nlocal) L.off[b] = o;
      o += c[i];
    }
    if (tid < 64) L.off[bs.nlocal + tid] = tid && trash_beyond ? (uint32_t)LDS::geo::kTileG : total;
  }
  __syncthreads();
#pragma unroll
  for (int q = 0; q < (NB + kT - 1) / kT; q++) {
    const uint32_t b = (uint32_t)q * kT + tid;
    res.g0[q] = 0;
    if (b < bs.nlocal) {
      const uint32_t c = L.cnt[b];
      if (c) res.g0[q] = atomicAdd(&out.counts[out_seg(bs, ob0, b)], (unsigned long long)c);
    }
  }
}

constexpr unsigned long long kDstMask = (1ULL << 48) - 1;

template <class LDS, int NB>
__device__ __forceinline__ void bin_commit(LDS &L, const BinSpec &bs, const BinOut &out, uint32_t ob0, const BinRes<NB, LDS::geo::kT> &res)
{
  constexpr int kT = LDS::geo::kT;
#pragma unroll
  for (int q = 0; q < (NB + kT - 1) / kT; q++) {
    const uint32_t b = (uint32_t)q * kT + threadIdx.x;
    if (b < bs.nlocal) {
      const uint32_t o0 = L.off[b], o1 = L.off[b + 1];
      const unsigned long long g0 = res.g0[q];
      const unsigned long long room = out.cap > g0 ? out.cap - g0 : 0;
      const uint32_t lim = o0 + (uint32_t)min((unsigned long long)(o1 - o0), room);
      const unsigned long long dst = ((unsigned long long)out_seg(bs, ob0, b) * out.cap + g0 - o0) & kDstMask;
      L.gbase[b] = dst | ((unsigned long long)lim << 48);
    }
  }
}

template <class LDS> __device__ __forceinline__ uint32_t bin_rank(LDS &L, uint32_t local)
{
  return L.off[local] + atomicAdd(&L.rnk[local], 1u);
}

template <int W, bool FULL, class LDS>
__device__ __forceinline__ void bin_place(LDS &L, int round, uint32_t p, uint32_t local, const Kmer<W> &t, uint32_t e)
{
  constexpr uint32_t kSt = LDS::geo::kStageG;
  if ((int)(p / kSt) != round) return;
  const uint32_t q = p % kSt;
  L.skey[q * W] = t.w[0];
  if (W == 2) L.skey[q * W + 1] = t.w[W - 1];
  L.sbin[q] = (uint16_t)local;
  if (FULL) L.se[q] = (uint8_t)e;
}

template <int W, bool ONECOL, bool FULL, int SH, class LDS>
__device__ __forceinline__ void bin_writeout(LDS &L, int round, const BinSpec &bs, const BinOut &out, uint32_t ob0,
                                             uint32_t region_of_seg, const InsertSink<W, ONECOL> &isink,
                                             uint32_t &novel, uint32_t &full)
{
  __syncthreads();
  const uint32_t n = L.off[bs.nlocal];
  constexpr uint32_t kSt = LDS::geo::kStageG;
  const uint32_t lo = (uint32_t)round * kSt;
  const uint32_t hi = min(n, lo + kSt);
  auto emit = [&](uint32_t p, uint32_t b, unsigned long long gb, uint64_t t0, uint64_t t1) {
    if (p < (uint32_t)(gb >> 48)) {
      const uint64_t at = (gb + p) & kDstMask;
      uint64_t *kd = out.keys + at * W;
      kd[0] = t0;
      if (W == 2) kd[1] = t1;
      if (FULL) out.edges[at] = L.se[p - lo];
    } else if (FULL || bs.mode == BIN_OWNER) {
      full = 2;
    } else {
      Kmer<W> tq;
      tq.w[0] = t0;
      if (W == 2) tq.w[W - 1] = t1;
      const uint32_t e = (uint32_t)(tq.w[0] >> 56);
      const Kmer<W> qq = tuple_q<W>(tq);
      const uint32_t lbq = lbq_of(isink.t);
      if (SH == 2) {
        const Kmer<W> key = key_unquot<W>(qq, lbq, b ^ mix_g(region_mix<W>(qq), lbq));
        const uint32_t owner = b >> bs.lb1;
        const unsigned long long pos = atomicAdd(&out.ov_counts[owner], 1ULL);
        if (pos < out.ov_cap) {
          uint64_t *kd = out.ov_keys + ((uint64_t)owner * out.ov_cap + pos) * W;
          kd[0] = key.w[0];
          if (W == 2) kd[1] = key.w[W - 1];
          out.ov_edges[(uint64_t)owner * out.ov_cap + pos] = (uint8_t)e;
        } else {
          const unsigned long long sp_cap = bs.region0 ? out.ov_counts[bs.nparts + 1] : 0;
          const unsigned long long sp = sp_cap ? atomicAdd(&out.ov_counts[bs.nparts], 1ULL) : 0;
          if (sp < sp_cap) {
            const uint64_t at = (uint64_t)bs.nparts * out.ov_cap + sp;
            uint64_t *kd = out.ov_keys + at * W;
            kd[0] = key.w[0];
            if (W == 2) kd[1] = key.w[W - 1];
            out.ov_edges[at] = (uint8_t)e;
          } else {
            full = 2;
          }
        }
      } else {
        table_mark_written(isink.t);
        table_count_fallback(isink.t);
        const uint32_t region = bs.mode == BIN_GROUP ? b : region_of_seg;
        const Kmer<W> key = key_unquot<W>(qq, lbq, r_of<W>(isink.t, region, qq));
        const uint64_t slot = key_slot<W>(isink.t, key);
        const uint64_t cur = *key_ptr_t<W, ONECOL>(isink.t, slot);
        probe_insert<W, ONECOL>(isink.t, key, slot, cur, 0, e, isink.col, novel, full);
      }
    }
  };
  for (uint32_t p = lo + threadIdx.x; p < hi; p += LDS::geo::kT) {
    const uint32_t q = p - lo;
    const uint32_t b = L.sbin[q];
    emit(p, b, L.gbase[b], L.skey[q * W], W == 2 ? L.skey[q * W + W - 1] : 0);
  }
  if (round + 1 < LDS::geo::kRoundsG) __syncthreads();
}

struct LaneWin { uint32_t a2, a1, a0, r2, r1, r0; };
__device__ __forceinline__ uint32_t pairrev32(uint32_t x)
{
// ... 27 lines not shown
{
  table_mark_written(isink.t);
  table_count_foreign(isink.t);
  const uint64_t slot = key_slot<W>(isink.t, key);
  const uint64_t cur = *key_ptr_t<W, ONECOL>(isink.t, slot);
  probe_insert<W, ONECOL>(isink.t, key, slot, cur, 0, e, isink.col, novel, full);
}

template <int W, bool ONECOL, int NB, bool FULL, int SH, bool PK, int T = kThreads>
__global__ __launch_bounds__(T, (W == 1 ? 4 : 3)) void k_stream_bin(StreamArgs a_arg, BinSpec bs, BinOut out_arg,
                                                                  InsertSink<W, ONECOL> isink_arg)
{
  constexpr int H = T / kThreads;
  static_assert(T == kThreads || (T == 2 * kThreads && !FULL), "256 threads, or 512 for packed bins");
  __shared__ uint32_t s_code_h[H][kChunks + 4];
  __shared__ uint32_t s_inv_h[H][kChunks / 2 + 4];
  struct Cold { StreamArgs a; InsertSink<W, ONECOL> isink; };
  __shared__ Cold cold;
  if (threadIdx.x == 0) { cold.a = a_arg; cold.isink = isink_arg; }
  __syncthreads();
  const StreamArgs &a = cold.a;
  const BinOut &out = out_arg;
  const InsertSink<W, ONECOL> &isink = cold.isink;
  const uint64_t a_tile0 = a_arg.tile0, a_ntiles = a_arg.ntiles;
  const uint32_t t_lb1 = isink_arg.t.lb1, t_lbq = isink_arg.t.lb1 + isink_arg.t.lbo, t_part = isink_arg.t.part;
  extern __shared__ __attribute__((aligned(16))) unsigned char dyn_lds[];
  using LDS = BinLds<W, NB, FULL, Geo<T, T * kPosPerLane>>;
  LDS &L = *reinterpret_cast<LDS *>(dyn_lds);

  const int tid0 = threadIdx.x & (kThreads - 1);
  const uint64_t half0 = (uint64_t)(threadIdx.x / kThreads);
  const int k = a_arg.k;
  uint32_t n_kmers = 0, n_contigs = 0, n_novel = 0, full = 0;
  const uint64_t top_mask = (W == 1) ? (~0ULL >> (64 - 2 * k)) : (~0ULL >> (128 - 2 * k));
  const int first_shift = (W == 1) ? (2 * k - 2) : (2 * k - 66);
  const uint32_t ob0 = (blockIdx.x % bs.rep) * bs.nout;

  TileSrc pre;
  pre.a = make_uint4(0, 0, 0, 0); pre.b = make_uint4(0, 0, 0, 0);
  {
    const uint64_t t0 = a_tile0 + (uint64_t)blockIdx.x * H + half0;
    if (t0 < a_ntiles) tile_fetch<PK>(a_arg, t0, tid0, pre);
  }
  MCX_PH_DECL
  for (uint64_t tile_b = a_tile0 + (uint64_t)blockIdx.x * H; tile_b < a_ntiles; tile_b += (uint64_t)gridDim.x * H) {
    const int tid_blk = (int)tid_now();
    const int tid = tid_blk & (kThreads - 1);
    const uint64_t tile = tile_b + (uint64_t)(tid_blk / kThreads);
    const bool have_tile = H == 1 || tile < a_ntiles;
    uint32_t *s_code = s_code_h[H == 1 ? 0 : tid_blk / kThreads];
    uint32_t *s_inv = s_inv_h[H == 1 ? 0 : tid_blk / kThreads];
    MCX_PH(6) MCX_PH_COUNT
    tile_stage<PK>(a_arg, pre, tid, s_code, s_inv);
    for (uint32_t b = tid_blk; b < bs.nlocal + 64; b += T) { L.cnt[b] = 0; L.rnk[b] = 0; }
    if (tid < 4) { s_code[kChunks + tid] = 0; s_inv[kChunks / 2 + tid] = 0xFFFFFFFFu; }
    {
      const uint64_t tn = tile + (uint64_t)gridDim.x * H;
      if (tn < a_ntiles) tile_fetch<PK>(a_arg, tn, tid, pre);
    }
    __syncthreads();
    MCX_PH(0)

    const uint32_t pl = 16u * (uint32_t)(tid + 1);
    const uint64_t Vh = inv_win64(s_inv, pl);
    const uint64_t Vl = (W == 2) ? inv_win64(s_inv, pl + 64) : 0;
    const uint32_t prev_chunk_inv = (s_inv[(pl - 1) >> 5] >> (31 - ((pl - 1) & 31))) & 1u;
    uint32_t range = have_tile ? 0xFFFFu : 0u;
    if (have_tile) {
      const uint64_t plo = a.pos_lo, phi = a.pos_hi, T0 = tile * kTile;
      if (T0 < plo || T0 + kTile > phi) {
        const uint64_t P0 = T0 + 16ull * (uint64_t)tid;
        const int j_lo = plo > P0 ? (int)min((uint64_t)kPosPerLane, plo - P0) : 0;
        const int j_hi = phi > P0 ? (int)min((uint64_t)kPosPerLane, phi - P0) : 0;
        range = ((0x10000u >> j_lo) - 1u) & ~((0x10000u >> j_hi) - 1u);
      }
    }
    uint32_t ok16, nok16, pok16;
    {
      uint64_t Mh = Vh, Ml = Vl;
      for (int c = 1; c < k;) {
        const int s = min(c, k - c);
        if (W == 2) Mh |= (Mh << s) | (Ml >> (64 - s));
        else Mh |= Mh << s;
        if (W == 2) Ml |= Ml << s;
        c += s;
      }
      ok16 = ~(uint32_t)(Mh >> 48) & range;
      const int sh = 112 - k;
      const uint64_t nx = sh >= 64 ? (Vh >> (sh - 64)) : ((Vh << (64 - sh)) | (W == 2 ? (Vl >> sh) : 0));
      nok16 = ~(uint32_t)nx & 0xFFFFu;
      pok16 = ~((prev_chunk_inv << 15) | (uint32_t)(Vh >> 49)) & 0xFFFFu;
    }

    Kmer<W> tk[kPosPerLane];
    uint32_t tle[kPosPerLane];
    const uint32_t trash = bs.nlocal + 1u + ((uint32_t)tid_blk & 31u);
    n_kmers += __popc(ok16);
    n_contigs += __popc(ok16 & ~pok16);
    {
      const uint32_t own = s_code[pl >> 4];
      const uint32_t before = s_code[(pl - 1) >> 4] & 3u;
      const uint32_t lbq = t_lbq;
      const uint32_t qmask = (1u << lbq) - 1u, lmask = (1u << t_lb1) - 1u;
      Kmer<W> fw, rc;
      uint64_t feed;
      LaneWin lw;
      if (W == 1) {
        lw = lane_win(s_code, pl, k);
        feed = code_win64(s_code, pl + (uint32_t)k);
      } else {
        const uint64_t hi = code_win64(s_code, pl), lo = code_win64(s_code, pl + 32);
        const int s = 128 - 2 * k;
        fw.w[0] = hi >> s;
        fw.w[W - 1] = (lo >> s) | (hi << (64 - s));
        rc = revcomp<W>(fw, k);
        feed = code_win64(s_code, pl + (uint32_t)k);
      }
      const uint32_t feed32 = (uint32_t)(feed >> 32);
      uint32_t arr_prev = 0;
      const uint32_t key_sh = 64u - 2u * (uint32_t)k;
      const uint32_t mix_sh = (32u - lbq) & 31u;
#pragma unroll
      for (int j = 0; j < kPosPerLane; j++) {
        const uint32_t prev_nuc = j == 0 ? before : ((own >> (32 - 2 * j)) & 3u);
        const uint32_t nuc_next = (feed32 >> (30 - 2 * j)) & 3u;
        const uint32_t valid = 0u - ((ok16 >> (15 - j)) & 1u);
        const uint32_t nb = (nok16 >> (15 - j)) & 1u, pb = (pok16 >> (15 - j)) & 1u;
        uint32_t o, local;
        Kmer<W> key;
        uint64_t sel = 0;
        if (W == 1) {
          const uint32_t fh = j ? __builtin_amdgcn_alignbit(lw.a2, lw.a1, 32 - 2 * j) : lw.a2;
          const uint32_t fl = j ? __builtin_amdgcn_alignbit(lw.a1, lw.a0, 32 - 2 * j) : lw.a1;
          const uint32_t rh = j < 15 ? __builtin_amdgcn_alignbit(lw.r2, lw.r1, 2 + 2 * j) : lw.r2;
          const uint32_t rl = j < 15 ? __builtin_amdgcn_alignbit(lw.r1, lw.r0, 2 + 2 * j) : lw.r1;
          const uint64_t f = ((uint64_t)fh << 32) | fl, r = ((uint64_t)rh << 32) | rl;
          o = f < r ? 0u : 1u;
          sel = f < r ? f : r;
          key.w[0] = sel >> key_sh;
        } else {
          key = canonical<W>(fw, rc, o);
        }
        const uint32_t o4 = o << 2;
        const uint32_t e = (nb << (nuc_next | o4)) | (pb << ((prev_nuc ^ 7u) ^ o4));
        if (FULL) {
          uint32_t h2;
          kmer_hash<W>(key, 0, &h2);
          local = owner_of(h2, bs.nparts);
          tk[j] = key;
          local = (local & valid) | (trash & ~valid);
          tle[j] = local | (e << 24);
        } else {
          uint32_t G;
          Kmer<W> q;
          if (W == 1) {
            const uint64_t kk = sel >> key_sh;
            q.w[0] = kk >> lbq;
            G = ((uint32_t)kk ^ (region_mix<W>(q) >> mix_sh)) & qmask;
          } else {
            uint32_t r;
            q = key_quot<W>(key, lbq, r);
            G = r ^ mix_g(region_mix<W>(q), lbq);
          }
          local = SH == 1 ? (G & lmask) : G;
          tk[j] = tuple_pack<W>(q, e);
          if (SH == 1 && valid && (G >> t_lb1) != t_part) {
            foreign_insert<W, ONECOL>(isink, key, e, n_novel, full);
            local = trash;
          }
          local = (local & valid) | (trash & ~valid);
          tle[j] = local;
        }
        const uint32_t arr_now = atomicAdd(&L.cnt[local], 1u);
        if (j > 0) { tle[j - 1] |= arr_prev << 12; asm volatile("" : "+v"(tle[j - 1])); }
        arr_prev = arr_now;
        if (j == kPosPerLane - 1) tle[j] |= arr_now << 12;
        if (W == 1) asm volatile("" : "+v"(tle[j]), "+v"(tk[j].w[0]));
        else asm volatile("" : "+v"(tle[j]), "+v"(tk[j].w[0]), "+v"(tk[j].w[W - 1]));
        if (W == 2) {
          fw.w[0] = ((fw.w[0] << 2) | (fw.w[W - 1] >> 62)) & top_mask;
          fw.w[W - 1] = (fw.w[W - 1] << 2) | nuc_next;
          rc.w[W - 1] = (rc.w[W - 1] >> 2) | (rc.w[0] << 62);
          rc.w[0] = (rc.w[0] >> 2) | ((uint64_t)(3u - nuc_next) << first_shift);
        }
      }
    }
    MCX_PH(1)
    BinRes<NB, T> res;
    bin_reserve<LDS, NB>(L, bs, out, ob0, res, !FULL);
    MCX_PH(2)
#pragma unroll
    for (int j = 0; j < kPosPerLane; j++) {
      tle[j] += L.off[tle[j] & 0xfffu] << 12;
      if ((j & 3) == 3) asm volatile("" : "+v"(tle[j - 3]), "+v"(tle[j - 2]), "+v"(tle[j - 1]), "+v"(tle[j]));
    }
    bin_commit<LDS, NB>(L, bs, out, ob0, res);
    MCX_PH(3)
    for (int round = 0; round < kRounds; round++) {
#pragma unroll
      for (int j = 0; j < kPosPerLane; j++)
        bin_place<W, FULL, LDS>(L, round, FULL ? (tle[j] >> 12) & 0xfffu : tle[j] >> 12, tle[j] & 0xfffu, tk[j], tle[j] >> 24);
      bin_writeout<W, ONECOL, FULL, SH, LDS>(L, round, bs, out, ob0, 0, isink, n_novel, full);
      if (round == 0) { MCX_PH(4) } else { MCX_PH(5) }
    }
  }
  MCX_PH_DUMP(0)

  block_add(&a.ctr->kmers, n_kmers);
  block_add(&a.ctr->contigs, n_contigs);
  block_add(&a.ctr->novel, n_novel);
  if (full == 1) a.ctr->full = 1;
  if (full == 2) a.ctr->bin_over = 1;
  if (a.flag && n_contigs) *a.flag = 1;
}

struct TupleIn {
  const uint64_t *keys;
  const uint8_t *edges;
  const unsigned long long *counts;
  uint64_t seg_cap;
  uint32_t nseg;
  uint32_t seg_group, seg_stride;
  uint32_t set_rep;
  uint8_t set_map[32];
};
__device__ __forceinline__ uint64_t tuple_seg_phys(const TupleIn &in, uint32_t seg)
{
  uint32_t q = seg / in.seg_group;
  if (in.set_rep) q = (uint32_t)in.set_map[q / in.set_rep] * in.set_rep + q % in.set_rep;
  return (uint64_t)q * in.seg_stride + seg % in.seg_group;
}

template <int W, bool ONECOL, int NB, bool IN_FULL, bool SHARD, int T = kThreads, int R = kRounds, int P = 16>
__global__ __launch_bounds__(T, (W == 1 || T > kThreads ? 4 : 3)) void k_tuples_bin(TupleIn in, BinSpec bs, BinOut out,
                                                                         InsertSink<W, ONECOL> isink_arg, Counters *ctr)
{
  extern __shared__ __attribute__((aligned(16))) unsigned char dyn_lds[];
  using LDS = BinLds<W, NB, false, Geo<T, T * P, R>>;
  constexpr int kThreads = T, kTile = T * P;
  LDS &L = *reinterpret_cast<LDS *>(dyn_lds);
  __shared__ InsertSink<W, ONECOL> isink;
  if (threadIdx.x == 0) isink = isink_arg;
  __syncthreads();
  const uint32_t t_spb = isink_arg.t.spb, t_lb1 = isink_arg.t.lb1, t_lbq = isink_arg.t.lb1 + isink_arg.t.lbo, t_part = isink_arg.t.part;
  const int tid = threadIdx.x;
  uint32_t n_novel = 0, full = 0;
  const uint64_t chunks_per_seg = (in.seg_cap + kTile - 1) / kTile;
  const bool xcd = bs.mode == BIN_SUBLOCAL && gridDim.x % 8 == 0 && bs.seg_mod % 8 == 0 && in.nseg % bs.seg_mod == 0;
  const uint32_t group = xcd ? blockIdx.x % 8 : 0;
  const uint32_t nseg_g = xcd ? in.nseg / 8 : in.nseg;
  constexpr uint32_t kWin = 2;
  const uint32_t bins_g = xcd ? bs.seg_mod / 8 : 1;
  const uint32_t reps = xcd ? in.nseg / bs.seg_mod : 1;
  const uint32_t win_segs = kWin * reps;
  const uint32_t nwin = (bins_g + kWin - 1) / kWin;
  const uint64_t nchunks = xcd ? (uint64_t)nwin * chunks_per_seg * win_segs : chunks_per_seg * nseg_g;
  const uint64_t v0 = xcd ? blockIdx.x / 8 : blockIdx.x, vstep = xcd ? gridDim.x / 8 : gridDim.x;
  const uint32_t lmask = (1u << t_lb1) - 1u;
  MCX_PH_DECL
  for (uint64_t v = v0; v < nchunks; v += vstep) {
    uint32_t seg;
    uint64_t start;
    if (xcd) {
      const uint64_t per_win = chunks_per_seg * win_segs;
      const uint32_t win = (uint32_t)(v / per_win);
      const uint64_t rem = v % per_win;
      const uint32_t s = (uint32_t)(rem % win_segs);
      const uint32_t rgi = win * kWin + s % kWin;
      if (rgi >= bins_g) continue;
      seg = (s / kWin) * bs.seg_mod + group + 8 * rgi;
      start = (rem / win_segs) * kTile;
    } else {
      seg = (uint32_t)(v % nseg_g);
      start = (v / nseg_g) * kTile;
    }
    const uint64_t pseg = tuple_seg_phys(in, seg);
    uint64_t cnt = in.counts ? (uint64_t)in.counts[pseg] : in.seg_cap;
    if (cnt > in.seg_cap) cnt = in.seg_cap;
    if (start >= cnt) continue;
    const uint32_t n = (uint32_t)min((uint64_t)kTile, cnt - start);
    const uint32_t lregion = bs.mode == BIN_SUBLOCAL ? seg % bs.seg_mod : 0;
    const uint32_t region = bs.region0 + lregion;
    const uint32_t ob0 = (bs.mode == BIN_SUBLOCAL ? lregion * t_spb : 0) + (blockIdx.x % bs.rep) * bs.nout;
    MCX_PH(6) MCX_PH_COUNT
    __syncthreads();
    for (uint32_t b = tid; b < bs.nlocal + 64; b += kThreads) { L.cnt[b] = 0; L.rnk[b] = 0; }
    __syncthreads();
    MCX_PH(0)
    const uint32_t trash = bs.nlocal + 1u + ((uint32_t)tid & 31u);
    const uint64_t *kin = in.keys + (pseg * in.seg_cap + start) * W;
    const uint8_t *ein = IN_FULL ? in.edges + pseg * in.seg_cap + start : nullptr;
    constexpr int PER = kTile / kThreads;
    Kmer<W> tk[PER];
    uint32_t ev[IN_FULL ? PER : 1], loc[PER];
    uint32_t okm = 0;
    const bool vec16 = !IN_FULL && (((uintptr_t)in.keys & 15u) == 0) && (W == 2 || (in.seg_cap & 1u) == 0);
    if (vec16) {
      const ulonglong2 *kin2 = reinterpret_cast<const ulonglong2 *>(kin);
#pragma unroll
      for (int q = 0; q < PER; q += (W == 1 ? 2 : 1)) {
        const uint32_t p = (uint32_t)(q / (W == 1 ? 2 : 1)) * kThreads + tid;
        const uint32_t i = W == 1 ? 2 * p : p;
        tk[q].w[0] = 0; tk[q + (W == 1 ? 1 : 0)].w[W - 1] = 0;
        if (i < n) {
          const ulonglong2 x = kin2[p];
          okm |= 1u << q;
          if (W == 1) {
            tk[q].w[0] = x.x;
            tk[q + (W == 1 ? 1 : 0)].w[0] = x.y;
            if (i + 1 < n) okm |= 2u << q;
          } else {
            tk[q].w[0] = x.x;
            tk[q].w[W - 1] = x.y;
          }
        }
      }
    } else {
#pragma unroll
    for (int q = 0; q < PER; q++) {
      const uint32_t i = (uint32_t)q * kThreads + tid;
      if (i < n) okm |= 1u << q;
      tk[q].w[0] = 0; if (W == 2) tk[q].w[W - 1] = 0;
      if (IN_FULL) ev[q] = 0;
      if (i < n) {
        tk[q].w[0] = kin[(uint64_t)i * W];
        if (W == 2) tk[q].w[W - 1] = kin[(uint64_t)i * W + 1];
        if (IN_FULL) ev[q] = ein[i];
      }
    }
    }
#pragma unroll
    for (int q = 0; q < PER; q++) {
      const uint32_t i = (uint32_t)q * kThreads + tid;
      uint32_t hb;
      if (IN_FULL) {
        uint32_t r;
        const uint32_t lbq = t_lbq;
        const Kmer<W> key = tk[q];
        const Kmer<W> qq = key_quot<W>(key, lbq, r);
        const uint32_t G = r ^ mix_g(region_mix<W>(qq), lbq);
        hb = 0;
        loc[q] = G & lmask;
        tk[q] = tuple_pack<W>(qq, ev[q]);
        if (SHARD && (okm >> q & 1u) && (G >> t_lb1) != t_part) {
          foreign_insert<W, ONECOL>(isink, key, ev[q], n_novel, full);
          okm &= ~(1u << q);
        }
      } else {
        hb = sub_hash<W>(tuple_q<W>(tk[q]));
        loc[q] = __umulhi(hb, t_spb);
      }
      if (loc[q] >= bs.nlocal) loc[q] = bs.nlocal - 1;
      loc[q] = (okm >> q & 1u) ? loc[q] : trash;
      atomicAdd(&L.cnt[loc[q]], 1u);
      (void)i;
    }
    MCX_PH(1)
    BinRes<NB, T> res;
    bin_reserve<LDS, NB>(L, bs, out, ob0, res, true);
    MCX_PH(2)
#pragma unroll
    for (int q = 0; q < PER; q++)
      loc[q] |= bin_rank<LDS>(L, loc[q]) << 16;
    bin_commit<LDS, NB>(L, bs, out, ob0, res);
    MCX_PH(3)
    for (int round = 0; round < R; round++) {
#pragma unroll
      for (int q = 0; q < PER; q++)
        bin_place<W, false, LDS>(L, round, loc[q] >> 16, loc[q] & 0xffffu, tk[q], 0);
      bin_writeout<W, ONECOL, false, 0, LDS>(L, round, bs, out, ob0, region, isink, n_novel, full);
      if (round == 0) { MCX_PH(4) } else { MCX_PH(5) }
    }
  }
  MCX_PH_DUMP(1)
  block_add(&ctr->novel, n_novel);
  if (full == 1) ctr->full = 1;
  if (full == 2) ctr->bin_over = 1;
}

template <int W> struct LdsCfg {
  static constexpr int kThreads = 512;
  static constexpr int kMinWaves = 4;
  static constexpr bool kPrefetch = true;
  static constexpr int kBatch = 4;
};
template <int W> struct LdsQueue { static constexpr uint32_t kTuples = W == 1 ? 1856 : 288; };

__device__ __forceinline__ uint32_t lds_phys1(uint32_t slot)
{
  return slot ^ ((slot >> 4) & 2u);
}
constexpr uint32_t kLdsVal1 = 4096;

template <int W>
__device__ __forceinline__ bool lds_apply(unsigned long long *lds, const Kmer<W> &key, uint32_t bucket, uint32_t e,
                                          uint32_t &n_novel, uint32_t &full)
{
  const unsigned long long want = key.w[0] | kFlag;
  uint32_t steps = 0;
  if constexpr (W == 1) {
    typedef unsigned long long u64x2 __attribute__((ext_vector_type(2)));
    typedef MCX_LDS_AS const volatile u64x2 lds_cv;
    uint32_t b = bucket;
    for (;;) {
      const uint32_t sw = (b >> 3) & 1u;
      unsigned long long *b0 = lds + b * kBucket;
      unsigned long long *h0 = b0 + 2 * sw, *h1 = b0 + 2 * (sw ^ 1u);
      const u64x2 lo = *(lds_cv *)h0;
      const u64x2 hi = *(lds_cv *)h1;
      unsigned long long *hit = nullptr, *emp = nullptr;
      if (hi.y == 0) emp = h1 + 1;
      if (hi.x == 0) emp = h1;
      if (lo.y == 0) emp = h0 + 1;
      if (lo.x == 0) emp = h0;
      if (hi.y == want) hit = h1 + 1;
      if (hi.x == want) hit = h1;
      if (lo.y == want) hit = h0 + 1;
      if (lo.x == want) hit = h0;
      if (hit) {
        unsigned long long *val = hit + kLdsVal1;
        const unsigned long long old = atomicAdd(val, 256ULL);
        if (e & ~(uint32_t)old) atomicOr(val, (unsigned long long)e);
        return true;
// ... 178 lines not shown
  } else if (W == 1) {
#define MCX_PUT1(q, kv, vv) { const uint32_t ph = lds_phys1(2u * (uint32_t)(q * T + tid)) >> 1; dst[ph] = make_ulonglong2(kv.x, kv.y); dst[kLdsVal1 / 2 + ph] = make_ulonglong2(vv.x, vv.y); }
    MCX_PUT1(0, v.a, v.e) MCX_PUT1(1, v.b, v.f) MCX_PUT1(2, v.c, v.g) MCX_PUT1(3, v.d, v.h)
#undef MCX_PUT1
  } else {
#define MCX_PUT2(j, k0, k1, vv) { const int p = j * T + tid; dst[3 * p] = make_ulonglong2(k0.x, k0.y); dst[3 * p + 1] = make_ulonglong2(vv.x, k1.x); dst[3 * p + 2] = make_ulonglong2(k1.y, vv.y); }
    MCX_PUT2(0, v.a, v.b, v.c) MCX_PUT2(1, v.d, v.e, v.f)
#undef MCX_PUT2
  }
}

template <int W, bool ONECOL, int T>
__device__ __forceinline__ void slice_store(const TableView &t, uint32_t sub, uint32_t col, int tid, const unsigned long long *lds)
{
  const ulonglong2 *src = reinterpret_cast<const ulonglong2 *>(lds);
  const uint64_t s0 = (uint64_t)sub * Sub<W>::kSlots;
  if (ONECOL && W == 1) {
    ulonglong2 *dst = reinterpret_cast<ulonglong2 *>(t.rec + s0 * 2);
#pragma unroll
    for (int q = 0; q < 8; q++) {
      const uint32_t sl = (uint32_t)(q * T + tid), ph = lds_phys1(sl);
      dst[sl] = make_ulonglong2(lds[ph], lds[kLdsVal1 + ph]);
    }
  } else if (ONECOL) {
    ulonglong2 *dst = reinterpret_cast<ulonglong2 *>(t.rec + s0 * (W + 1));
    constexpr int PER = (int)(Sub<W>::kSlots * (W + 1) * 8 / 16 / T);
#pragma unroll
    for (int q = 0; q < PER; q++) {
      dst[q * T + tid] = src[q * T + tid];
    }
  } else if (W == 1) {
    ulonglong2 *K = reinterpret_cast<ulonglong2 *>(t.rec + s0);
    ulonglong2 *V = reinterpret_cast<ulonglong2 *>(t.val + (uint64_t)col * t.VC + s0);
#pragma unroll
    for (int q = 0; q < 4; q++) {
      const uint32_t p = (uint32_t)(q * T + tid), ph = lds_phys1(2u * p) >> 1;
      K[p] = src[ph];
      V[p] = src[kLdsVal1 / 2 + ph];
    }
  } else {
    ulonglong2 *K = reinterpret_cast<ulonglong2 *>(t.rec + s0 * 2);
    ulonglong2 *V = reinterpret_cast<ulonglong2 *>(t.val + (uint64_t)col * t.VC + s0);
#pragma unroll
    for (int j = 0; j < 2; j++) {
      const int p = j * T + tid;
      const ulonglong2 x = src[3 * p], y = src[3 * p + 1], z = src[3 * p + 2];
      K[2 * p] = x;
      K[2 * p + 1] = make_ulonglong2(y.y, z.x);
      V[p] = make_ulonglong2(y.x, z.y);
    }
  }
}

template <int W, bool ONECOL>
__global__ __launch_bounds__(LdsCfg<W>::kThreads, LdsCfg<W>::kMinWaves) void k_lds_insert(TableView t, uint32_t col, BinOut bins,
                                                                       uint32_t sub0, uint32_t nsub, Counters *ctr)
{
  constexpr int kLdsThreads = LdsCfg<W>::kThreads;
  constexpr int kLdsBatch = LdsCfg<W>::kBatch;
  extern __shared__ __attribute__((aligned(16))) unsigned char dyn_lds[];
  unsigned long long *lds = reinterpret_cast<unsigned long long *>(dyn_lds);
  const int tid = threadIdx.x;
  uint32_t n_novel = 0, full = 0;
  unsigned long long *queue = lds + Sub<W>::kSlots * (W + 1);
  constexpr uint32_t kQueueCap = LdsQueue<W>::kTuples;
  __shared__ uint32_t s_nq;
  if (tid == 0) s_nq = 0;

  auto next_bin = [&](uint32_t from) {
    while (from < nsub && bins.counts[from] == 0) from += gridDim.x;
    return from;
  };
  uint32_t bi = next_bin(blockIdx.x);
  SliceRegs v{};
  const bool zeros_known = t.touch && t.touch[0] == 0;
  constexpr bool kPrefetch = LdsCfg<W>::kPrefetch;
  if (kPrefetch && bi < nsub) slice_fetch<W, ONECOL, kLdsThreads>(t, sub0 + bi, col, tid, v, zeros_known);
  auto idx = [&](int q) -> uint32_t { return (uint32_t)q * kLdsThreads + tid; };
  auto load_batch_of = [&](uint32_t bin, uint64_t nfill, uint64_t j0, Kmer<W> (&tk)[kLdsBatch]) {
    const uint64_t *kin = bins.keys + (uint64_t)bin * bins.cap * W;
#pragma unroll
    for (int q = 0; q < kLdsBatch; q++) {
      uint64_t i = j0 + idx(q);
      i = i < nfill ? i : 0;
      tk[q].w[0] = kin[i * W];
      if (W == 2) tk[q].w[W - 1] = kin[i * W + 1];
    }
  };
  constexpr uint64_t kStep = (uint64_t)kLdsThreads * kLdsBatch;
  MCX_PH_DECL
  while (bi < nsub) {
    const uint32_t sub = sub0 + bi;
    const uint32_t region = sub / t.spb;
    MCX_PH(6) MCX_PH_COUNT
    uint64_t n = bins.counts[bi];
    if (n > bins.cap) n = bins.cap;
    const uint32_t nb = next_bin(bi + gridDim.x);
    __syncthreads();
    MCX_PH(0)
    if (tid == 0) bins.counts[bi] = 0;
    if (!kPrefetch) slice_fetch<W, ONECOL, kLdsThreads>(t, sub, col, tid, v, zeros_known);
    slice_to_lds<W, ONECOL, kLdsThreads>(lds, tid, v);
    __syncthreads();
    MCX_PH(1)

    auto load_batch = [&](uint64_t j0, Kmer<W> (&tk)[kLdsBatch]) { load_batch_of(bi, n, j0, tk); };
    auto unpack = [&](const Kmer<W> &tp, Kmer<W> &key, uint32_t &bucket, uint32_t &e) {
      e = (uint32_t)(tp.w[0] >> 56);
      const Kmer<W> qq = tuple_q<W>(tp);
      const uint32_t m = region_mix<W>(qq);
      key = key_unquot<W>(qq, lbq_of(t), ((t.part << t.lb1) | region) ^ mix_g(m, lbq_of(t)));
      bucket = mix_bucket(m, lbq_of(t), Sub<W>::kBuckets);
    };
    auto apply_slow = [&](const Kmer<W> &key, uint32_t bucket, uint32_t e) {
      if (!lds_apply<W>(lds, key, bucket, e, n_novel, full))
        probe_insert<W, ONECOL>(t, key, ovf_start<W>(t, key), 0, 0, e, col, n_novel, full, true);
    };
    auto apply_batch = [&](uint64_t j0, const Kmer<W> (&tk)[kLdsBatch]) {
#pragma unroll
      for (int q = 0; q < kLdsBatch; q++)
        if (j0 + idx(q) < n) {
          Kmer<W> key;
          uint32_t bucket, e;
          unpack(tk[q], key, bucket, e);
          if (!lds_try<W>(lds, key, bucket, e, n_novel)) {
            const uint32_t qi = atomicAdd(&s_nq, 1u);
            if (qi < kQueueCap) {
              queue[qi * W] = tk[q].w[0];
              if (W == 2) queue[qi * W + 1] = tk[q].w[W - 1];
            } else {
              apply_slow(key, bucket, e);
            }
          }
        }
    };
    auto run = [&](auto has_next) {
      Kmer<W> ta[kLdsBatch], tb[kLdsBatch];
      load_batch(0, ta);
      load_batch(kStep, tb);
      if (decltype(has_next)::value) slice_fetch<W, ONECOL, kLdsThreads>(t, sub0 + nb, col, tid, v, zeros_known);
      for (uint64_t j0 = 0; j0 < n; j0 += 2 * kStep) {
        apply_batch(j0, ta);
        load_batch(j0 + 2 * kStep, ta);
        apply_batch(j0 + kStep, tb);
        load_batch(j0 + 3 * kStep, tb);
      }
    };
    if (kPrefetch && nb < nsub) run(std::true_type{}); else run(std::false_type{});
    MCX_PH(2)
    __syncthreads();
    MCX_PH(3)
    {
      const uint32_t nq = min(s_nq, kQueueCap);
      for (uint32_t i = tid; i < nq; i += kLdsThreads) {
        Kmer<W> tp, key;
        uint32_t bucket, e;
        tp.w[0] = queue[i * W];
        if (W == 2) tp.w[W - 1] = queue[i * W + 1];
        unpack(tp, key, bucket, e);
        apply_slow(key, bucket, e);
      }
      __syncthreads();
      if (tid == 0) s_nq = 0;
    }
    MCX_PH(4)
    slice_store<W, ONECOL, kLdsThreads>(t, sub, col, tid, lds);
    if (tid == 0 && t.touch) atomicOr(&t.touch[1 + (sub >> 5)], 1u << (sub & 31u));
    bi = nb;
    MCX_PH(5)
  }
  MCX_PH_DUMP(2)
  block_add(&ctr->novel, n_novel);
  if (full) ctr->full = 1;
}

}
```

### mccortex_amd/csrc/mcx_kernels.h

```cpp
#pragma once
#include <hip/hip_runtime.h>
#include <stdint.h>
#include "mcx_kmer.h"

namespace mcx {

constexpr int kBucket = 4;
template <int W> struct Sub {
  static constexpr int kShift = W == 1 ? 12 : 11;
  static constexpr uint64_t kSlots = 1ull << kShift;
  static constexpr uint32_t kBuckets = (uint32_t)(kSlots / kBucket);
};
__host__ __device__ constexpr int sub_shift_for_words(int W) { return W == 1 ? 12 : 11; }

struct TableView {
  uint64_t *rec;
  uint64_t nslots;
  uint64_t nmain;
  uint32_t lb1;
  uint32_t lbo;
  uint32_t part;
  uint32_t spb;
  uint32_t S;
  uint32_t max_probe;
  uint32_t KS;
  uint32_t VS;
  uint64_t *val;
  uint64_t VC;
  uint32_t *touch;
};
constexpr int kTouchHdr = 32;
__device__ __forceinline__ void table_mark_written(const TableView &t)
{
  if (t.touch) t.touch[0] = 1u;
}
__device__ __forceinline__ void table_count_slow(unsigned long long *ctr)
{
  const unsigned long long act = __builtin_amdgcn_ballot_w64(true);
  const uint32_t lane = __builtin_amdgcn_mbcnt_hi((uint32_t)(act >> 32), __builtin_amdgcn_mbcnt_lo((uint32_t)act, 0u));
  if (lane == 0) atomicAdd(ctr, (unsigned long long)__popcll(act));
}
__device__ __forceinline__ void table_count_fallback(const TableView &t)
{
  if (t.touch) table_count_slow(reinterpret_cast<unsigned long long *>(t.touch) - 4);
}
__device__ __forceinline__ void table_count_foreign(const TableView &t)
{
  if (t.touch) table_count_slow(reinterpret_cast<unsigned long long *>(t.touch) - 3);
}
template <class T> __device__ __forceinline__ uint64_t wave_append(T *cursor, bool take)
{
  const unsigned long long act = __builtin_amdgcn_ballot_w64(take);
  if (!act) return 0;
  const uint32_t below = __builtin_amdgcn_mbcnt_hi((uint32_t)(act >> 32), __builtin_amdgcn_mbcnt_lo((uint32_t)act, 0u));
  const uint32_t leader = (uint32_t)__ffsll((long long)act) - 1u;
  T at = 0;
  if (take && below == 0) at = atomicAdd(cursor, (T)__popcll(act));
  at = __shfl(at, (int)leader, 64);
  return (uint64_t)at + below;
}
__device__ __forceinline__ bool table_full_flagged(const TableView &t)
{
  return t.touch && __hip_atomic_load(t.touch - 2, __ATOMIC_RELAXED, __HIP_MEMORY_SCOPE_AGENT) != 0u;
}
__device__ __forceinline__ void table_flag_full(const TableView &t)
{
  if (t.touch) __hip_atomic_store(t.touch - 2, 1u, __ATOMIC_RELAXED, __HIP_MEMORY_SCOPE_AGENT);
}
__device__ __forceinline__ uint64_t *key_ptr(const TableView &t, uint64_t slot) { return t.rec + slot * t.KS; }
__device__ __forceinline__ uint64_t *val_ptr(const TableView &t, uint64_t slot, uint32_t col)
{
  return t.val + slot * t.VS + (uint64_t)col * t.VC;
}
template <int W, bool ONECOL> __device__ __forceinline__ uint64_t *key_ptr_t(const TableView &t, uint64_t slot)
{
  return t.rec + slot * (ONECOL ? (uint64_t)(W + 1) : (uint64_t)W);
}
template <int W, bool ONECOL> __device__ __forceinline__ uint64_t *val_ptr_t(const TableView &t, uint64_t slot, uint32_t col)
{
  return ONECOL ? t.rec + slot * (uint64_t)(W + 1) + W : t.val + (uint64_t)col * t.VC + slot;
}

// ... 6 lines not shown
  return x * 0x9E3779B1u;
}
template <int W> __device__ __host__ __forceinline__ uint32_t sub_hash(const Kmer<W> &q)
{
  uint32_t x = (uint32_t)q.w[0] + (uint32_t)(q.w[0] >> 32) * 0xC2B2AE35u;
  if (W == 2) x += (uint32_t)q.w[W - 1] * 0x27D4EB2Fu + (uint32_t)(q.w[W - 1] >> 32) * 0x165667B1u;
  if (W > 2)
    for (int i = 1; i < W; i++) x += (uint32_t)q.w[i] * (0x27D4EB2Fu + 0x3C6EF372u * (uint32_t)(i - 1)) + (uint32_t)(q.w[i] >> 32) * (0x165667B1u + 0x7F4A7C16u * (uint32_t)(i - 1));
  x *= 0x85EBCA6Bu;
  x ^= x >> 15;
  return x * 0x2C1B3C6Du;
}
__device__ __host__ __forceinline__ uint32_t mix_g(uint32_t m, uint32_t lbq) { return (uint32_t)(((uint64_t)m << lbq) >> 32); }
__device__ __host__ __forceinline__ uint32_t mix_bucket(uint32_t m, uint32_t lbq, uint32_t nbuckets)
{
  return (m >> (22u - lbq)) & (nbuckets - 1u);
}
template <int W> __device__ __host__ __forceinline__ Kmer<W> key_quot(const Kmer<W> &key, uint32_t lb1 , uint32_t &r)
{
  Kmer<W> q = key;
  if (W == 1) {
    r = (uint32_t)key.w[0] & ((1u << lb1) - 1u);
    q.w[0] = key.w[0] >> lb1;
    return q;
  }
  r = 0;
  if (lb1) {
    r = (uint32_t)key.w[W - 1] & ((1u << lb1) - 1u);
    if (W == 2) q.w[W - 1] = (key.w[W - 1] >> lb1) | (key.w[0] << (64 - lb1));
    if (W > 2)
      for (int i = W - 1; i >= 1; i--) q.w[i] = (key.w[i] >> lb1) | (key.w[i - 1] << (64 - lb1));
    q.w[0] = key.w[0] >> lb1;
  }
  return q;
}
template <int W> __device__ __host__ __forceinline__ Kmer<W> key_unquot(const Kmer<W> &q, uint32_t lb1, uint32_t r)
{
  Kmer<W> key = q;
  if (W == 1) {
    key.w[0] = (q.w[0] << lb1) | r;
    return key;
  }
  if (lb1) {
    key.w[0] = q.w[0] << lb1;
    if (W == 2) { key.w[0] |= q.w[W - 1] >> (64 - lb1); key.w[W - 1] = q.w[W - 1] << lb1; }
    if (W > 2)
      for (int i = 0; i < W; i++) key.w[i] = (q.w[i] << lb1) | (i + 1 < W ? q.w[i + 1] >> (64 - lb1) : 0ull);
    key.w[W - 1] |= r;
  }
  return key;
}
__device__ __host__ __forceinline__ uint32_t lbq_of(const TableView &t) { return t.lb1 + t.lbo; }

struct TableAddr { uint32_t G, region, sub, bucket; };
template <int W> __device__ __forceinline__ TableAddr addr_of(const TableView &t, const Kmer<W> &q, uint32_t r)
{
  const uint32_t b = sub_hash<W>(q);
  const uint32_t lbq = lbq_of(t), m = region_mix<W>(q);
  TableAddr a;
  a.G = r ^ mix_g(m, lbq);
  a.region = a.G & ((1u << t.lb1) - 1u);
  a.sub = a.region * t.spb + __umulhi(b, t.spb);
  a.bucket = mix_bucket(m, lbq, Sub<W>::kBuckets);
  return a;
}
template <int W> __device__ __forceinline__ uint32_t key_owner(const TableView &t, const Kmer<W> &key)
{
  uint32_t r;
  const Kmer<W> q = key_quot<W>(key, lbq_of(t), r);
  return (r ^ mix_g(region_mix<W>(q), lbq_of(t))) >> t.lb1;
}
template <int W> __device__ __forceinline__ uint32_t r_of(const TableView &t, uint32_t region, const Kmer<W> &q)
{
  return ((t.part << t.lb1) | region) ^ mix_g(region_mix<W>(q), lbq_of(t));
}
template <int W> __device__ __forceinline__ uint64_t key_slot(const TableView &t, const Kmer<W> &key)
{
  uint32_t r;
  const Kmer<W> q = key_quot<W>(key, lbq_of(t), r);
  const TableAddr a = addr_of<W>(t, q, r);
  return ((uint64_t)a.sub << Sub<W>::kShift) + (uint64_t)a.bucket * kBucket;
}

constexpr int kMmer = 13;
constexpr uint32_t kMmerMask = (1u << (2 * kMmer)) - 1u;
constexpr int kSuperkMinK = kMmer + 16;

MCX_HD uint32_t mmer_hash(uint32_t c)
{
  const uint32_t x = c * 0x9E3779B1u;
  return x ^ (x >> 15);
}
MCX_HD uint32_t owner_of_minimizer(uint32_t min_hash, uint32_t lbo)
{
  return lbo ? ((min_hash * 0x85EBCA6Bu) ^ (min_hash >> 13)) * 0xC2B2AE35u >> (32u - lbo) : 0u;
}

MCX_HD uint32_t superk_owner(uint64_t w0, uint64_t w1, int k, uint32_t lbo)
{
  uint32_t best = 0xFFFFFFFFu;
  for (int p = 0; p + kMmer <= k; p++) {
    const int sh = 2 * (k - kMmer - p);
    const uint64_t low = sh >= 64 ? (w0 >> (sh - 64)) : (sh ? (w1 >> sh) | (w0 << (64 - sh)) : w1);
    const uint32_t f = (uint32_t)low & kMmerMask;
    uint32_t r = 0;
    for (int i = 0; i < kMmer; i++) r |= (3u - ((f >> (2 * i)) & 3u)) << (2 * (kMmer - 1 - i));
    const uint32_t h = mmer_hash(f < r ? f : r);
    best = h < best ? h : best;
  }
  return owner_of_minimizer(best, lbo);
}


struct OwnerSpec {
  uint32_t mode;
// ... 1114 lines not shown
```

### mccortex_amd/csrc/mcx_streamfc.h

```cpp
#pragma once
#include "mcx_defer.h"

namespace mcx {

constexpr int kFcPool = 384;
constexpr int kFcBins = 512;

template <int CAP> struct FcLds {
  uint64_t seg[kFcBins * CAP];
  uint64_t pool_t[kFcPool];
  uint32_t pool_b[kFcPool];
  uint32_t cnt[2][kFcBins + 64];
  uint32_t code[2][kChunks + 4];
  uint32_t inv[2][kChunks / 2 + 4];
  uint32_t pool_n[2];
  uint32_t left[2];
};

template <bool ONECOL>
__device__ __noinline__ uint32_t fc_direct(const InsertSink<1, ONECOL> &isink, uint32_t region, uint64_t t0)
{
  uint32_t novel = 0, full = 0;
  Kmer<1> tq;
  tq.w[0] = t0;
// ... 84 lines not shown
    uint32_t range = 0xFFFFu;
    {
      const uint64_t plo = a.pos_lo, phi = a.pos_hi, T0 = tile * kTile;
      if (T0 < plo || T0 + kTile > phi) {
        const uint64_t P0 = T0 + 16ull * (uint64_t)tid;
        const int j_lo = plo > P0 ? (int)min((uint64_t)kPosPerLane, plo - P0) : 0;
        const int j_hi = phi > P0 ? (int)min((uint64_t)kPosPerLane, phi - P0) : 0;
        range = ((0x10000u >> j_lo) - 1u) & ~((0x10000u >> j_hi) - 1u);
      }
    }
    uint32_t ok16, nok16, pok16;
    {
      uint64_t Mh = Vh;
      for (int c = 1; c < k;) {
        const int s = min(c, k - c);
        Mh |= Mh << s;
        c += s;
      }
      ok16 = ~(uint32_t)(Mh >> 48) & range;
      const int sh = 112 - k;
      const uint64_t nx = Vh >> (sh - 64);
      nok16 = ~(uint32_t)nx & 0xFFFFu;
      pok16 = ~((prev_chunk_inv << 15) | (uint32_t)(Vh >> 49)) & 0xFFFFu;
    }
    n_kmers += __popc(ok16);
    n_contigs += __popc(ok16 & ~pok16);
    const uint32_t trash = nlocal + 1u + ((uint32_t)tid & 31u);
    uint64_t tk[kPosPerLane];
    uint32_t tb[kPosPerLane];
    uint32_t ovmask = 0;
    {
      uint32_t arr[kPosPerLane];
      const uint32_t own = s_code[pl >> 4];
      const uint32_t before = s_code[(pl - 1) >> 4] & 3u;
      const uint32_t lbq = t_lbq;
      const uint32_t qmask = (1u << lbq) - 1u;
      const LaneWin lw = lane_win(s_code, pl, k);
      const uint32_t feed32 = (uint32_t)(code_win64(s_code, pl + (uint32_t)k) >> 32);
      const uint32_t key_sh = 64u - 2u * (uint32_t)k;
      const uint32_t mix_sh = (32u - lbq) & 31u;
#pragma unroll
      for (int j = 0; j < kPosPerLane; j++) {
        const uint32_t prev_nuc = j == 0 ? before : ((own >> (32 - 2 * j)) & 3u);
        const uint32_t nuc_next = (feed32 >> (30 - 2 * j)) & 3u;
        const uint32_t valid = 0u - ((ok16 >> (15 - j)) & 1u);
        const uint32_t nb = (nok16 >> (15 - j)) & 1u, pb = (pok16 >> (15 - j)) & 1u;
        const uint32_t fh = j ? __builtin_amdgcn_alignbit(lw.a2, lw.a1, 32 - 2 * j) : lw.a2;
        const uint32_t fl = j ? __builtin_amdgcn_alignbit(lw.a1, lw.a0, 32 - 2 * j) : lw.a1;
        const uint32_t rh = j < 15 ? __builtin_amdgcn_alignbit(lw.r2, lw.r1, 2 + 2 * j) : lw.r2;
        const uint32_t rl = j < 15 ? __builtin_amdgcn_alignbit(lw.r1, lw.r0, 2 + 2 * j) : lw.r1;
        const uint64_t f = ((uint64_t)fh << 32) | fl, r = ((uint64_t)rh << 32) | rl;
        const uint32_t o = f < r ? 0u : 1u;
        const uint64_t sel = f < r ? f : r;
        const uint32_t o4 = o << 2;
        const uint32_t e = (nb << (nuc_next | o4)) | (pb << ((prev_nuc ^ 7u) ^ o4));
        const uint64_t kk = sel >> key_sh;
        Kmer<W> q;
        q.w[0] = kk >> lbq;
        const uint32_t Gr = ((uint32_t)kk ^ (region_mix<W>(q) >> mix_sh)) & qmask;
        const uint32_t local = (Gr & valid) | (trash & ~valid);
        tk[j] = q.w[0] | ((uint64_t)e << 56);
        tb[j] = local;
        arr[j] = atomicAdd(&cnt[local], 1u);
        asm volatile("" : "+v"(tb[j]), "+v"(tk[j]));
      }
#pragma unroll
      for (int j = 0; j < kPosPerLane; j++) {
        const uint32_t bj = tb[j];
        if (bj < nlocal) {
          if (arr[j] < (uint32_t)CAP) L.seg[bj * CAP + arr[j]] = tk[j];
          else { ovmask |= 1u << j; tb[j] = bj | (arr[j] << 16); }
        }
      }
    }
    MCX_PH(0)
    if (ovmask) {
      const uint32_t ov0 = ovmask;
      const uint32_t base = atomicAdd(&L.pool_n[par], (uint32_t)__popc(ov0));
#pragma unroll
      for (int j = 0; j < kPosPerLane; j++) {
        if ((ov0 >> j) & 1u) {
          const uint32_t p = base + __popc(ov0 & ((1u << j) - 1u));
          if (p < (uint32_t)kFcPool) { L.pool_t[p] = tk[j]; L.pool_b[p] = PRIV ? tb[j] : tb[j] & 0xffffu; ovmask &= ~(1u << j); }
        }
      }
      if (ovmask) L.left[par] = 1;
    }
    MCX_PH(1)
    __syncthreads();
    MCX_PH(2)

    const uint32_t lane = (uint32_t)tid & 63u, wbin0 = ((uint32_t)tid >> 6) * (64u * ROWS);
    uint32_t c_row[ROWS], fit_tot[ROWS];
    unsigned long long g_row[ROWS];
#pragma unroll
    for (int r = 0; r < ROWS; r++) {
      const uint32_t b = wbin0 + 64u * r + lane;
      const uint32_t call = b < nlocal ? cnt[b] : 0u;
      const uint32_t c = min(call, (uint32_t)CAP);
      c_row[r] = c;
      if (PRIV) {
        g_row[r] = fill[r];
        fit_tot[r] = (uint32_t)min((unsigned long long)call, out.cap > g_row[r] ? out.cap - g_row[r] : 0ull);
        fill[r] = (uint32_t)min((unsigned long long)fill[r] + call, 0xFFFF0000ull);
      } else {
        g_row[r] = c ? atomicAdd(&out.counts[ob0 + b], (unsigned long long)c) : 0ull;
        fit_tot[r] = 0;
      }
// ... 101 lines not shown
```

### mccortex_amd/graph.py

```python
import ctypes as C
import os

import numpy as np

from . import _build

MCX_OK, MCX_ERR_ARG, MCX_ERR_NODEVICE, MCX_ERR_NOMEM, MCX_ERR_FULL, MCX_ERR_HIP, MCX_ERR_SINK = 0, -1, -2, -3, -4, -5, -6

_LIB = None

SYMBOLS = [
    "mcx_last_error", "mcx_version", "mcx_device_count", "mcx_device_memory", "mcx_graph_create", "mcx_graph_create_multi", "mcx_graph_ndevices",
    "mcx_graph_create_shard", "mcx_graph_shard_layout", "mcx_graph_shard_bins_dev", "mcx_graph_add_segments_dev",
    "mcx_graph_key_owner", "mcx_graph_insert_tuple_segments_dev", "mcx_graph_add_records", "mcx_graph_kmer_covg", "mcx_graph_covg_histogram", "mcx_sort_records",
    "mcx_records_sorted", "mcx_graph_intersect_finish", "mcx_superk_supported", "mcx_superk_record_bytes", "mcx_superk_owner", "mcx_graph_checksum", "mcx_records_checksum",
    "mcx_graph_superk_layout", "mcx_graph_superk_bins_dev", "mcx_graph_add_superk_dev", "mcx_graph_destroy",
    "mcx_graph_reset", "mcx_graph_configure", "mcx_graph_profile", "mcx_graph_capacity", "mcx_graph_add_reads", "mcx_graph_add_reads_pcr", "mcx_graph_pcr_reset", "mcx_graph_add_stream_dev",
    "mcx_graph_partition_stream_dev", "mcx_graph_insert_tuples_dev", "mcx_key_owner", "mcx_graph_sync",
    "mcx_graph_nkmers", "mcx_graph_device_stats", "mcx_graph_stream", "mcx_graph_export",
    "mcx_kmer_from_str", "mcx_kmer_canonical", "mcx_kmer_hash", "mcx_pack_bases", "mcx_pack_reads_host", "mcx_pack_stream_dev", "mcx_graph_add_packed_dev",
    "mcx_ubench_stream", "mcx_ubench_random_rmw", "mcx_graph_insert_stats", "mcx_multi_exchange_bytes", "mcx_graph_hashtest", "mcx_hashtest_func", "mcx_debug_probe",
    "mcx_graph_infer_edges", "mcx_graph_infer_edges_dev", "mcx_graph_unitig_stats", "mcx_graph_clean",
    "mcx_graph_unitigs", "mcx_graph_unitigs_dev", "mcx_graph_pop_bubbles",
    "mcx_graph_subgraph_begin", "mcx_graph_subgraph_seed_reads", "mcx_graph_subgraph_seed_stream_dev", "mcx_graph_subgraph_finish",
    "mcx_graph_reads_touch", "mcx_graph_reads_touch_stream_dev",
]


class McxError(RuntimeError):
    def __init__(self, code, msg):
        super().__init__("mcx error %d: %s" % (code, msg))
        self.code = code


class LoadStats(C.Structure):
    _fields_ = [(n, C.c_uint64) for n in (
        "num_se_reads", "num_good_reads", "num_bad_reads", "total_bases_read",
        "total_bases_loaded", "contigs_parsed", "num_kmers_loaded", "num_kmers_novel",
        "num_pe_reads", "num_dup_se_reads", "num_dup_pe_pairs")]

    def as_dict(self):
        return {n: int(getattr(self, n)) for n, _ in self._fields_}


class RecordStats(C.Structure):
    _fields_ = [("nkmers_read", C.c_uint64), ("nkmers_loaded", C.c_uint64), ("nkmers_novel", C.c_uint64),
                ("first_oversized", C.c_int64), ("first_zero_covg", C.c_int64), ("first_edges_no_covg", C.c_int64)]

    def __init__(self):
        super().__init__(0, 0, 0, -1, -1, -1)

    def as_dict(self):
        return {n: int(getattr(self, n)) for n, _ in self._fields_}


class CleanStats(C.Structure):
    _fields_ = [(n, C.c_uint64) for n in ("num_tips", "num_tip_kmers", "num_low_covg_unitigs", "num_low_covg_unitig_kmers",
                                          "num_tip_and_low_unitigs", "num_tip_and_low_unitig_kmers", "nkmers_before",
                                          "nkmers_removed")]

    def as_dict(self):
        return {n: int(getattr(self, n)) for n, _ in self._fields_}


class PopStats(C.Structure):
    _fields_ = [(n, C.c_uint64) for n in ("num_popped", "num_pairs", "nkmers_before", "nkmers_removed", "num_unitigs_removed")] + \
               [("rounds", C.c_uint32)]

    def as_dict(self):
        return {n: int(getattr(self, n)) for n, _ in self._fields_}


class SubgraphStats(C.Structure):
    _fields_ = [(n, C.c_uint64) for n in ("num_seed_kmers", "num_seed_found", "nkmers_before", "nkmers_kept", "nkmers_removed")] + \
# ... 7 lines not shown
    _fields_ = [(n, C.c_uint64) for n in ("num_reads", "num_reads_hit", "num_kmers", "num_kmers_found")]

    def as_dict(self):
        return {n: int(getattr(self, n)) for n, _ in self._fields_}


class UnitigsStats(C.Structure):
    _fields_ = [(n, C.c_uint64) for n in ("num_unitigs", "num_kmers", "num_bytes", "num_cycles")]

    def as_dict(self):
        return {n: int(getattr(self, n)) for n, _ in self._fields_}


class UnitigsArrays(C.Structure):
    _fields_ = [(n, C.c_void_p) for n in ("keys", "unitig", "rank", "orient", "first", "length")]


CLEAN_NBINS = 1000
UNITIGS_FORMATS = {"fasta": 0, "gfa": 1, "dot": 2}
UNITIGS_POINTS = 1
RECORDS_MUST_EXIST = 1
INFER_POP, INFER_PRESENCE_COVG = 1, 2
SUBGRAPH_UNITIGS, SUBGRAPH_INVERT = 1, 2
SINK_FN = C.CFUNCTYPE(C.c_int, C.c_void_p, C.c_void_p, C.c_size_t)


def lib():
    global _LIB
    if _LIB is not None:
        return _LIB
    try:
        import torch
    except ImportError:
        pass
    path = os.environ.get("MCX_LIB") or _build.LIB
    if not os.path.exists(path):
        raise RuntimeError("HIP extension missing: %s (run __graft_entry__.build())" % path)
    L = C.CDLL(path)
    vp, u64p = C.c_void_p, C.POINTER(C.c_uint64)
    L.mcx_last_error.restype = C.c_char_p
    L.mcx_version.restype = C.c_char_p
    L.mcx_device_count.restype = C.c_int
    L.mcx_graph_create.argtypes = [C.POINTER(vp), C.c_int, C.c_int, C.c_uint64, C.c_int]
    L.mcx_graph_create_shard.argtypes = [C.POINTER(vp), C.c_int, C.c_int, C.c_uint64, C.c_int, C.c_int, C.c_int]
    L.mcx_graph_create_multi.argtypes = [C.POINTER(vp), C.c_int, C.c_int, C.c_uint64, C.POINTER(C.c_int), C.c_int]
    L.mcx_graph_ndevices.argtypes = [vp]
    L.mcx_graph_shard_layout.argtypes = [vp, C.c_uint64, C.POINTER(C.c_uint32), u64p, u64p]
    L.mcx_graph_shard_bins_dev.argtypes = [vp, vp, C.c_uint64, vp, vp, C.c_uint64, vp, vp, vp, C.c_uint64]
    L.mcx_graph_add_segments_dev.argtypes = [vp, C.c_int, vp, vp, C.c_uint32, C.c_uint64, C.c_uint64]
    L.mcx_graph_insert_tuple_segments_dev.argtypes = [vp, C.c_int, vp, vp, vp, C.c_uint32, C.c_uint64]
    L.mcx_graph_add_records.argtypes = [vp, vp, C.c_uint64, C.c_int, vp, vp, C.c_int, C.c_uint32, C.POINTER(RecordStats)]
    L.mcx_graph_kmer_covg.argtypes = [vp, u64p, u64p]
    L.mcx_graph_insert_stats.argtypes = [vp, vp]
    L.mcx_graph_covg_histogram.argtypes = [vp, u64p, C.c_uint32]
    L.mcx_sort_records.argtypes = [vp, C.c_uint64, C.c_int, C.c_int, C.c_int]
    L.mcx_records_sorted.argtypes = [vp, C.c_uint64, C.c_int, C.c_int, C.c_int, C.POINTER(C.c_int64)]
    L.mcx_graph_intersect_finish.argtypes = [vp, u64p]
    L.mcx_graph_unitig_stats.argtypes = [vp, vp]
    L.mcx_graph_clean.argtypes = [vp, C.c_uint32, C.c_uint32, C.POINTER(CleanStats), vp]
    L.mcx_graph_pop_bubbles.argtypes = [vp, C.c_int32, C.c_int32, C.c_int32, C.POINTER(PopStats)]
    L.mcx_graph_subgraph_begin.argtypes = [vp, C.c_uint32]
    L.mcx_graph_subgraph_seed_reads.argtypes = [vp, vp, vp, C.c_uint64]
    L.mcx_graph_subgraph_seed_stream_dev.argtypes = [vp, vp, C.c_uint64]
    L.mcx_graph_subgraph_finish.argtypes = [vp, C.c_uint32, C.c_uint32, C.POINTER(SubgraphStats)]
    L.mcx_graph_reads_touch.argtypes = [vp, vp, vp, C.c_uint64, vp, C.POINTER(TouchStats)]
    L.mcx_graph_reads_touch_stream_dev.argtypes = [vp, vp, C.c_uint64, vp, C.c_uint64, vp]
    L.mcx_graph_unitigs.argtypes = [vp, C.c_int, C.c_uint32, SINK_FN, vp, C.POINTER(UnitigsStats)]
    L.mcx_graph_unitigs_dev.argtypes = [vp, C.POINTER(UnitigsArrays), C.POINTER(UnitigsStats)]
    L.mcx_graph_infer_edges.argtypes = [vp, vp, C.c_uint64, C.c_int, C.c_uint32, u64p]
    L.mcx_graph_infer_edges_dev.argtypes = [vp, vp, C.c_uint64, C.c_int, C.c_uint32, u64p]
    L.mcx_superk_supported.argtypes = [C.c_int]
    L.mcx_superk_record_bytes.argtypes = [C.c_int]
    L.mcx_superk_owner.restype = C.c_uint32
    L.mcx_superk_owner.argtypes = [u64p, C.c_int, C.c_int]
    L.mcx_graph_superk_layout.argtypes = [vp, C.c_int, C.c_uint64, C.POINTER(C.c_uint32), u64p]
    L.mcx_graph_superk_bins_dev.argtypes = [vp, vp, C.c_uint64, C.c_int, vp, vp, C.c_uint64]
    L.mcx_graph_add_superk_dev.argtypes = [vp, C.c_int, vp, vp, C.c_uint32, C.c_uint64, C.c_uint64]
    L.mcx_graph_checksum.argtypes = [vp, u64p, u64p]
    L.mcx_records_checksum.restype = C.c_uint64
    L.mcx_records_checksum.argtypes = [vp, C.c_uint64, C.c_int, C.c_int]
    L.mcx_ubench_stream.argtypes = [C.c_int, C.c_uint64, C.POINTER(C.c_double), C.POINTER(C.c_double), C.POINTER(C.c_double)]
    L.mcx_ubench_random_rmw.argtypes = [C.c_int, C.c_uint64, C.c_uint64, C.POINTER(C.c_double), C.POINTER(C.c_double), C.POINTER(C.c_double)]
    L.mcx_graph_key_owner.restype = C.c_uint32
    L.mcx_graph_key_owner.argtypes = [vp, u64p]
    L.mcx_graph_destroy.argtypes = [vp]
    L.mcx_graph_destroy.restype = None
    L.mcx_graph_reset.argtypes = [vp]
    L.mcx_graph_capacity.argtypes = [vp, u64p, u64p]
    L.mcx_graph_configure.argtypes = [vp, C.c_char_p, C.c_uint64]
    L.mcx_graph_profile.argtypes = [vp, C.c_char_p, C.c_size_t]
    L.mcx_graph_add_reads.argtypes = [vp, C.c_int, vp, vp, vp, C.c_uint64, C.c_uint8, C.c_uint8,
                                      C.POINTER(LoadStats)]
    L.mcx_graph_add_reads_pcr.argtypes = [vp, C.c_int, vp, vp, vp, C.c_uint64, C.c_uint8, C.c_uint8, C.c_uint8,
                                          C.c_int, C.c_int, C.POINTER(LoadStats)]
    L.mcx_graph_pcr_reset.argtypes = [vp]
    L.mcx_graph_add_stream_dev.argtypes = [vp, C.c_int, vp, C.c_uint64]
    L.mcx_pack_stream_dev.argtypes = [vp, C.c_uint64, vp, vp, vp]
    L.mcx_graph_add_packed_dev.argtypes = [vp, C.c_int, vp, vp, C.c_uint64]
    L.mcx_graph_partition_stream_dev.argtypes = [vp, vp, C.c_uint64, C.c_int, C.c_uint64, vp, vp, vp]
    L.mcx_graph_insert_tuples_dev.argtypes = [vp, C.c_int, vp, vp, C.c_uint64]
    L.mcx_graph_hashtest.argtypes = [vp, C.c_uint64, C.c_uint64]
    L.mcx_hashtest_func.argtypes = [C.c_int, C.c_int, C.c_uint64, C.c_uint32, C.POINTER(C.c_uint64)]
    L.mcx_key_owner.restype = C.c_uint32
    L.mcx_key_owner.argtypes = [u64p, C.c_int, C.c_int]
    L.mcx_graph_sync.argtypes = [vp]
    L.mcx_graph_nkmers.argtypes = [vp, u64p]
# ... 219 lines not shown

    def add_stream_dev(self, colour, d_stream, nbytes):
        _check(self.L.mcx_graph_add_stream_dev(self.h, colour, _ptr(d_stream), nbytes))

    def partition_stream_dev(self, d_stream, nbytes, nparts, bin_capacity, d_keys, d_edges, d_counts):
        _check(self.L.mcx_graph_partition_stream_dev(self.h, _ptr(d_stream), nbytes, nparts, bin_capacity,
                                                     _ptr(d_keys), _ptr(d_edges), _ptr(d_counts)))

    def hashtest(self, first, n):
        _check(self.L.mcx_graph_hashtest(self.h, first, n))

    def insert_tuples_dev(self, colour, d_keys, d_edges, n):
        _check(self.L.mcx_graph_insert_tuples_dev(self.h, colour, _ptr(d_keys), _ptr(d_edges), n))

    def shard_layout(self, tuples_per_call):
        segs, cap, ov = C.c_uint32(), C.c_uint64(), C.c_uint64()
        _check(self.L.mcx_graph_shard_layout(self.h, int(tuples_per_call), C.byref(segs), C.byref(cap), C.byref(ov)))
        return int(segs.value), int(cap.value), int(ov.value)

    def shard_bins_dev(self, d_stream, nbytes, d_keys, d_counts, seg_cap, d_ov_keys, d_ov_edges, d_ov_counts, ov_cap):
        _check(self.L.mcx_graph_shard_bins_dev(self.h, _ptr(d_stream), nbytes, _ptr(d_keys), _ptr(d_counts), seg_cap,
                                               _ptr(d_ov_keys), _ptr(d_ov_edges), _ptr(d_ov_counts), ov_cap))

    def add_segments_dev(self, colour, d_keys, d_counts, nseg, seg_cap, ntuples):
        _check(self.L.mcx_graph_add_segments_dev(self.h, colour, _ptr(d_keys), _ptr(d_counts), nseg, seg_cap, int(ntuples)))

    def insert_tuple_segments_dev(self, colour, d_keys, d_edges, d_counts, nseg, seg_cap):
        _check(self.L.mcx_graph_insert_tuple_segments_dev(self.h, colour, _ptr(d_keys), _ptr(d_edges), _ptr(d_counts),
                                                          nseg, seg_cap))

    def key_owner(self, words):
        a = (C.c_uint64 * 2)(*words)
        return int(self.L.mcx_graph_key_owner(self.h, a))

    def sync(self):
        _check(self.L.mcx_graph_sync(self.h))

    @property
    def nkmers(self):
        n = C.c_uint64()
        _check(self.L.mcx_graph_nkmers(self.h, C.byref(n)))
        return int(n.value)

    def device_stats(self):
        st = LoadStats()
        _check(self.L.mcx_graph_device_stats(self.h, C.byref(st)))
        return st

    def insert_stats(self):
        st = (C.c_uint64 * 4)()
        _check(self.L.mcx_graph_insert_stats(self.h, st))
        return dict(zip(("fallback_inserts", "foreign_inserts", "spilled", "flushes"), (int(x) for x in st)))

    @property
    def stream(self):
        return self.L.mcx_graph_stream(self.h)

    def pop_bubbles(self, max_covg=-1, max_klen=-1, max_kdiff=-1):
        st = PopStats()
        _check(self.L.mcx_graph_pop_bubbles(self.h, int(max_covg), int(max_klen), int(max_kdiff), C.byref(st)))
        return st.as_dict()

    def subgraph_begin(self, unitigs=False):
        _check(self.L.mcx_graph_subgraph_begin(self.h, SUBGRAPH_UNITIGS if unitigs else 0))

    def subgraph_seed(self, bases, offsets):
        bases = np.ascontiguousarray(bases, dtype=np.uint8)
        offsets = np.ascontiguousarray(offsets, dtype=np.uint64)
        _check(self.L.mcx_graph_subgraph_seed_reads(self.h, _ptr(bases), _ptr(offsets), len(offsets) - 1))

    def subgraph_seed_stream_dev(self, d_stream, nbytes):
        _check(self.L.mcx_graph_subgraph_seed_stream_dev(self.h, _ptr(d_stream), int(nbytes)))

    def subgraph_finish(self, dist=0, invert=False, unitigs=False):
        st = SubgraphStats()
        _check(self.L.mcx_graph_subgraph_finish(self.h, int(dist), (SUBGRAPH_UNITIGS if unitigs else 0) | (SUBGRAPH_INVERT if invert else 0),
                                                C.byref(st)))
        return st.as_dict()

    def reads_touch(self, bases, offsets, stats=None):
        bases = np.ascontiguousarray(bases, dtype=np.uint8)
        offsets = np.ascontiguousarray(offsets, dtype=np.uint64)
        nreads = max(len(offsets) - 1, 0)
        hit = np.zeros(nreads, dtype=np.uint8)
        st = stats if stats is not None else TouchStats()
        _check(self.L.mcx_graph_reads_touch(self.h, _ptr(bases), _ptr(offsets), nreads, _ptr(hit), C.byref(st)))
        return hit, st

    def reads_touch_stream_dev(self, d_stream, nbytes, d_stream_off, nreads, d_hit):
        _check(self.L.mcx_graph_reads_touch_stream_dev(self.h, _ptr(d_stream), int(nbytes), _ptr(d_stream_off), int(nreads), _ptr(d_hit)))

    def subgraph(self, seeds, dist=0, invert=False, unitigs=False):
        seqs = [s.encode() if isinstance(s, str) else bytes(s) for s in seeds]
        offs = np.zeros(len(seqs) + 1, dtype=np.uint64)
        offs[1:] = np.cumsum([len(s) for s in seqs])
        self.subgraph_begin(unitigs)
        if seqs:
            self.subgraph_seed(np.frombuffer(b"".join(seqs) or b"\n", dtype=np.uint8), offs)
        return self.subgraph_finish(dist, invert, unitigs)

    def unitigs_chunks(self, format="fasta", points=False, stats=None):
        if format not in UNITIGS_FORMATS:
            raise ValueError("unitigs format: one of %s" % ", ".join(sorted(UNITIGS_FORMATS)))
        parts = []

        def sink(_ctx, ptr, n):
# ... 113 lines not shown
```

Baseline: 104.1 billion.

## Add optional 6-byte narrow tuple encoding for sub-table bin flushes

Adds an opt-in mode that packs deferred k-mer tuples into 48-bit records. Bits implied by the destination sub-table are dropped, using a bijective sub-local hash so they can be rebuilt at insert time. The goal is less memory traffic in the L2 bins during split and LDS insert. This needs new kernel variants, a separate overflow area for odd tuples, double-sized count arrays and capacity rounding. It is off by default, but the sub-table index function changes whenever the bijective bits are available.

```diff
diff --git a/include/mcx_gpu.h b/include/mcx_gpu.h
--- a/include/mcx_gpu.h
+++ b/include/mcx_gpu.h
@@ -208,6 +208,8 @@
 } mcx_insert_stats;
 int mcx_graph_insert_stats(mcx_graph *g, mcx_insert_stats *out);
 
+int mcx_graph_tuple_bytes(const mcx_graph *g);
+
 void *mcx_graph_stream(mcx_graph *g);
 
 typedef int (*mcx_sink_fn)(void *ctx, const void *records, size_t nbytes);
diff --git a/mccortex_amd/csrc/mcx_api.hip b/mccortex_amd/csrc/mcx_api.hip
--- a/mccortex_amd/csrc/mcx_api.hip
+++ b/mccortex_amd/csrc/mcx_api.hip
@@ -188,6 +188,10 @@
   hipStream_t stream2 = nullptr;
   hipEvent_t ev_split[2] = {nullptr, nullptr}, ev_ins[2] = {nullptr, nullptr};
   unsigned long long *l1_cnt = nullptr, *l2_cnt = nullptr;
+  uint32_t l2_half_regions = 0;
+  bool narrow = false;
+  bool window_wide = false;
+  bool flush_narrow = false;
   uint32_t nsets = 1;
   uint64_t set_cap = 0;
   std::vector<int> set_colour;
@@ -361,10 +365,12 @@
   g->t.lbo = lbo;
   g->t.part = (uint32_t)part;
   g->t.spb = (uint32_t)spb;
+  g->t.sub_s = sub_bij_bits(g->W, kmer_size, lb1 + lbo, (uint32_t)spb, &g->t.sub_qlb);
   g->t.S = (uint32_t)(g->W + ncols);
   g->t.max_probe = (uint32_t)sub_slots;
   { const char *e = getenv("MCX_DEFER"); if (e) g->defer = atoi(e) != 0; }
   if (g->W > 2) g->defer = false;
+  { const char *e = getenv("MCX_NARROW_TUPLES"); if (e) g->narrow = atoi(e) != 0; }
   { const char *e = getenv("MCX_GRID_STREAM"); if (e) g->grid_stream = atoi(e); }
   { const char *e = getenv("MCX_REP1"); if (e && atoi(e) >= 1 && atoi(e) <= 4096) { g->rep1 = (uint32_t)atoi(e); g->rep1_forced = true; } }
   { const char *e = getenv("MCX_GRID_SPLIT"); if (e) g->grid_split = atoi(e); }
@@ -475,7 +481,8 @@
   g->n_flushes = 0;
   if (g->h_full) { HIP_TRY(hipStreamSynchronize(g->stream)); *g->h_full = 0; }
   if (g->l1_cnt) HIP_TRY(hipMemsetAsync(g->l1_cnt, 0, (size_t)g->nsets * g->b1 * g->rep1 * 8, g->stream));
-  if (g->l2_cnt) HIP_TRY(hipMemsetAsync(g->l2_cnt, 0, (size_t)g->l2_regions * g->subs_per_bin * 8, g->stream));
+  if (g->l2_cnt) HIP_TRY(hipMemsetAsync(g->l2_cnt, 0, (size_t)g->l2_regions * g->subs_per_bin * 16, g->stream));
+  g->window_wide = false;
   if (g->d_readstrt) HIP_TRY(hipMemsetAsync(g->d_readstrt, 0xff, g->t.nslots * 8, g->stream));
   g->pending = g->pending_l2 = 0;
   g->idle_next = 0; g->idle_base = 0; g->idle_mark.clear();
@@ -657,11 +664,16 @@
   else launch_bin_stream_pk<W, ONECOL, FULL, SH, false>(g, a, nt, colour, bs, out);
 }
 
+static bool split_wide_blocks()
+{
+  static const bool on = [] { const char *e = getenv("MCX_SPLIT_T"); return !e || atoi(e) == 512; }();
+  return on;
+}
 template <int W, bool ONECOL, bool IN_FULL, bool SHARD>
 static void launch_bin_tuples_t(mcx_graph *g, TupleIn in, int colour, BinSpec bs, BinOut out)
 {
   constexpr bool kWide = W == 1 && !IN_FULL;
-  static const bool wide = kWide && [] { const char *e = getenv("MCX_SPLIT_T"); return !e || atoi(e) == 512; }();
+  static const bool wide = kWide && split_wide_blocks();
   const bool use_wide = wide && bs.nlocal <= 1024;
   const bool use_huge = wide && !use_wide && bs.nlocal <= (uint32_t)kMaxBins;
   const uint64_t tile = use_huge ? 1024 * 16 : use_wide ? 512 * 16 : kTile;
@@ -678,6 +690,11 @@
     if constexpr (kWide) allow_lds(k_tuples_bin<W, ONECOL, 512, IN_FULL, SHARD, 512>, sizeof(BinLds<W, 512, false, GeoW>));
     if constexpr (kWide) allow_lds(k_tuples_bin<W, ONECOL, 1024, IN_FULL, SHARD, 512>, sizeof(BinLds<W, 1024, false, GeoW>));
     if constexpr (kWide) allow_lds(k_tuples_bin<W, ONECOL, kMaxBins, IN_FULL, SHARD, 1024>, sizeof(BinLds<W, kMaxBins, false, Geo<1024, 1024 * 16>>));
+    if constexpr (kWide) {
+      allow_lds(k_tuples_bin<W, ONECOL, 512, IN_FULL, SHARD, 512, kRounds, 16, true>, sizeof(BinLds<W, 512, false, GeoW>));
+      allow_lds(k_tuples_bin<W, ONECOL, 1024, IN_FULL, SHARD, 512, kRounds, 16, true>, sizeof(BinLds<W, 1024, false, GeoW>));
+      allow_lds(k_tuples_bin<W, ONECOL, kMaxBins, IN_FULL, SHARD, 1024, kRounds, 16, true>, sizeof(BinLds<W, kMaxBins, false, Geo<1024, 1024 * 16>>));
+    }
     once = true;
   }
   SpanGuard sp(g, "k_tuples_bin");
@@ -686,12 +703,19 @@
     if (use_huge) {
       using GeoH = Geo<1024, 1024 * 16>;
       const dim3 gridh((unsigned)std::min<uint64_t>(nchunks, g->grid_split ? gmax : gmax / 4));
+      if (out.ncap)
+        hipLaunchKernelGGL((k_tuples_bin<W, ONECOL, kMaxBins, IN_FULL, SHARD, 1024, kRounds, 16, true>), gridh, dim3(1024), sizeof(BinLds<W, kMaxBins, false, GeoH>), g->stream, in, bs, out, is, g->d_ctr);
+      else
       hipLaunchKernelGGL((k_tuples_bin<W, ONECOL, kMaxBins, IN_FULL, SHARD, 1024>), gridh, dim3(1024), sizeof(BinLds<W, kMaxBins, false, GeoH>), g->stream, in, bs, out, is, g->d_ctr);
       return;
     }
     if (use_wide) {
       const dim3 gridw((unsigned)std::min<uint64_t>(nchunks, g->grid_split ? gmax : gmax / 2));
-      if (bs.nlocal <= 512)
+      if (out.ncap && bs.nlocal <= 512)
+        hipLaunchKernelGGL((k_tuples_bin<W, ONECOL, 512, IN_FULL, SHARD, 512, kRounds, 16, true>), gridw, dim3(512), sizeof(BinLds<W, 512, false, GeoW>), g->stream, in, bs, out, is, g->d_ctr);
+      else if (out.ncap)
+        hipLaunchKernelGGL((k_tuples_bin<W, ONECOL, 1024, IN_FULL, SHARD, 512, kRounds, 16, true>), gridw, dim3(512), sizeof(BinLds<W, 1024, false, GeoW>), g->stream, in, bs, out, is, g->d_ctr);
+      else if (bs.nlocal <= 512)
         hipLaunchKernelGGL((k_tuples_bin<W, ONECOL, 512, IN_FULL, SHARD, 512>), gridw, dim3(512), sizeof(BinLds<W, 512, false, GeoW>), g->stream, in, bs, out, is, g->d_ctr);
       else
         hipLaunchKernelGGL((k_tuples_bin<W, ONECOL, 1024, IN_FULL, SHARD, 512>), gridw, dim3(512), sizeof(BinLds<W, 1024, false, GeoW>), g->stream, in, bs, out, is, g->d_ctr);
@@ -725,16 +749,44 @@
   return g->l2_keys + off * g->cap2 * g->W;
 }
 
+static bool narrow_capable(const mcx_graph *g)
+{
+  return g->narrow && g->t.sub_s && g->W == 1 && split_wide_blocks() && g->cap2 % 6 == 0 && 2 * g->subs_per_bin <= (uint32_t)kMaxBins;
+}
+struct NarrowOff { mcx_graph *g; ~NarrowOff() { g->flush_narrow = false; } };
+static uint64_t odd_cap_of(const mcx_graph *g) { return std::max<uint64_t>(64, g->cap2 / 16); }
+static uint64_t narrow_cap_of(const mcx_graph *g) { return ((g->cap2 - odd_cap_of(g)) * 8 / 6) & ~1ull; }
+static BinOut l2_out(const mcx_graph *g)
+{
+  BinOut b{l2_ptr(g, g->l2_off), nullptr, g->l2_cnt + g->l2_off, g->cap2, nullptr, nullptr, nullptr, 0, nullptr, 0, 0};
+  if (g->flush_narrow) {
+    b.odd_counts = g->l2_cnt + (uint64_t)g->l2_regions * g->subs_per_bin + g->l2_off;
+    b.odd_cap = odd_cap_of(g);
+    b.ncap = narrow_cap_of(g);
+  }
+  return b;
+}
+
 template <int W, bool ONECOL> static void launch_lds_insert_t(mcx_graph *g, int colour, uint32_t sub0, uint32_t nsub)
 {
   const size_t lds = Sub<W>::kSlots * (W + 1) * 8 + LdsQueue<W>::kTuples * 8 * W;
   static bool once_dev[64] = {false};
   bool &once = once_dev[g->device & 63];
-  if (!once) { allow_lds(k_lds_insert<W, ONECOL>, lds); once = true; }
-  BinOut bins{l2_ptr(g, g->l2_off), nullptr, g->l2_cnt + g->l2_off, g->cap2, nullptr, nullptr, nullptr, 0};
+  if (!once) {
+    allow_lds(k_lds_insert<W, ONECOL>, lds);
+    if constexpr (W == 1) allow_lds(k_lds_insert<W, ONECOL, true>, lds);
+    once = true;
+  }
+  const BinOut bins = l2_out(g);
   SpanGuard sp(g, "k_lds_insert");
-  hipLaunchKernelGGL((k_lds_insert<W, ONECOL>), dim3((unsigned)std::min<uint64_t>(nsub, (uint64_t)(g->grid_insert ? g->grid_insert : g->grid * 4))),
-                     dim3(LdsCfg<W>::kThreads), lds, g->stream, g->t, (uint32_t)colour, bins, sub0, nsub, g->d_ctr);
+  const dim3 grid((unsigned)std::min<uint64_t>(nsub, (uint64_t)(g->grid_insert ? g->grid_insert : g->grid * 4)));
+  if constexpr (W == 1) {
+    if (bins.ncap) {
+      hipLaunchKernelGGL((k_lds_insert<W, ONECOL, true>), grid, dim3(LdsCfg<W>::kThreads), lds, g->stream, g->t, (uint32_t)colour, bins, sub0, nsub, g->d_ctr);
+      return;
+    }
+  }
+  hipLaunchKernelGGL((k_lds_insert<W, ONECOL>), grid, dim3(LdsCfg<W>::kThreads), lds, g->stream, g->t, (uint32_t)colour, bins, sub0, nsub, g->d_ctr);
 }
 
 template <int W, bool ONECOL>
@@ -752,12 +804,13 @@
   (void)hipFree(g->l2_base); (void)hipFree(g->l2_hi); (void)hipFree(g->l2_cnt);
   g->l1_keys = g->l2_keys = g->l2_base = g->l2_hi = nullptr; g->l1_cnt = g->l2_cnt = nullptr;
   g->cap1 = g->cap2 = 0;
-  g->l2_regions = 0;
+  g->l2_regions = 0; g->l2_half_regions = 0;
   g->set_colour.clear(); g->set_pending.clear();
 }
 
 __global__ __launch_bounds__(512) void k_l2_probe(uint64_t *keys, uint64_t cap, uint32_t nregions, uint32_t spb, uint32_t iters,
-                                                  uint32_t jit_mask = 0 )
+                                                  uint32_t jit_mask = 0 ,
+                                                  uint32_t run = 16)
 {
   const uint32_t region = blockIdx.x % nregions, blk = blockIdx.x / nregions, nblk = gridDim.x / nregions;
   const uint32_t w = threadIdx.x >> 6, l = threadIdx.x & 63u;
@@ -766,8 +819,8 @@
       const uint32_t front = w * 4u + (l >> 4) + 32u * k;
       const uint32_t seg = region * spb + front;
       const uint64_t jit = ((seg * 0x9E3779B1u) >> 8) & jit_mask & ~15u;
-      const uint64_t at = (uint64_t)seg * cap + jit + ((uint64_t)it * nblk + blk) * 16u + (l & 15u);
-      if (jit + ((uint64_t)it * nblk + blk) * 16u + 16u <= cap) keys[at] = at;
+      const uint64_t at = (uint64_t)seg * cap + jit + ((uint64_t)it * nblk + blk) * run + (l & 15u);
+      if ((l & 15u) < run && jit + ((uint64_t)it * nblk + blk) * run + run <= cap) keys[at] = at;
     }
 }
 
@@ -790,7 +843,7 @@
     if (tries > 1)
       for (int rep = 0; rep < 2; rep++) {
         (void)hipEventRecord(e0, g->stream);
-        hipLaunchKernelGGL(k_l2_probe, dim3(nreg * 64), dim3(512), 0, g->stream, p, g->cap2 * g->W, nreg, g->subs_per_bin, iters);
+        hipLaunchKernelGGL(k_l2_probe, dim3(nreg * 64), dim3(512), 0, g->stream, p, g->cap2 * g->W, nreg, g->subs_per_bin, iters, 0u, narrow_capable(g) ? 12u : 16u);
         (void)hipEventRecord(e1, g->stream);
         if (hipEventSynchronize(e1) != hipSuccess || hipEventElapsedTime(&t, e0, e1) != hipSuccess) { (void)hipGetLastError(); t = 0.f; }
       }
@@ -817,11 +870,16 @@
 static uint32_t flush_group(const mcx_graph *g);
 static int ensure_l2(mcx_graph *g, uint32_t regions, bool whole = false)
 {
-  if (g->l2_keys && g->l2_regions >= regions && !(g->l2_hi && (whole || (regions > g->l2_regions / 2 && regions != g->l2_regions)))) return MCX_OK;
+  {
+    bool keep = g->l2_keys && g->l2_regions >= regions;
+    if (keep && g->l2_hi)
+      keep = !whole && (regions <= g->l2_half_regions || (regions == 2 * g->l2_half_regions && flush_group(g) == g->l2_half_regions));
+    if (keep) return MCX_OK;
+  }
   if (g->pending_l2) return fail(MCX_ERR_ARG, "internal: sub-table bins resized while in use");
   HIP_TRY(hipStreamSynchronize(g->stream));
   (void)hipFree(g->l2_base); (void)hipFree(g->l2_hi); (void)hipFree(g->l2_cnt);
-  g->l2_keys = g->l2_base = g->l2_hi = nullptr; g->l2_cnt = nullptr; g->l2_regions = 0; g->l2_hi_off = 0;
+  g->l2_keys = g->l2_base = g->l2_hi = nullptr; g->l2_cnt = nullptr; g->l2_regions = 0; g->l2_hi_off = 0; g->l2_half_regions = 0;
   const uint64_t nb = (uint64_t)regions * g->subs_per_bin;
   int tries = g->place_tries;
   { const char *e = getenv("MCX_PLACE_BINS"); if (e) tries = atoi(e); }
@@ -834,15 +892,16 @@
     if (g->l2_base) g->l2_hi = l2_place(g, hbytes, G, tries, nullptr);
     if (g->l2_base && !g->l2_hi) { (void)hipFree(g->l2_base); g->l2_base = nullptr; }
     g->l2_hi_off = nb / 2;
+    g->l2_half_regions = G;
   } else {
     g->l2_base = l2_place(g, nb * g->cap2 * 8 * g->W, std::min<uint32_t>(regions, 32), tries, nullptr);
   }
-  if (!g->l2_base || hipMalloc((void **)&g->l2_cnt, nb * 8) != hipSuccess) {
+  if (!g->l2_base || hipMalloc((void **)&g->l2_cnt, nb * 16) != hipSuccess) {
     (void)hipGetLastError();
-    (void)hipFree(g->l2_base); (void)hipFree(g->l2_hi); g->l2_base = g->l2_hi = nullptr;
+    (void)hipFree(g->l2_base); (void)hipFree(g->l2_hi); g->l2_base = g->l2_hi = nullptr; g->l2_half_regions = 0;
     return fail(MCX_ERR_NOMEM, "out of device memory for the sub-table bins (%llu regions)", (unsigned long long)regions);
   }
-  HIP_TRY(hipMemsetAsync(g->l2_cnt, 0, nb * 8, g->stream));
+  HIP_TRY(hipMemsetAsync(g->l2_cnt, 0, nb * 16, g->stream));
   g->l2_keys = g->l2_base;
   g->l2_regions = regions;
   return MCX_OK;
@@ -897,6 +956,7 @@
     g->cap2 = g->nsub == 1 ? tcap + 8192 : (uint64_t)((double)tcap / g->nsub * cap2_slack) + 1024;
     g->cap1 = (g->cap1 + 1) & ~1ull;
     g->cap2 = (g->cap2 + 1) & ~1ull;
+    if (g->t.sub_s) g->cap2 = (g->cap2 + 5) / 6 * 6;
     if (g->cap1 >= 0xFFFFFFFFull || g->cap2 >= 0xFFFFFFFFull) continue;
     const uint64_t n1 = (uint64_t)g->nsets * g->b1 * g->rep1 * g->cap1;
     const bool ok = hipMalloc((void **)&g->l1_keys, n1 * 8 * g->W) == hipSuccess &&
@@ -940,9 +1000,12 @@
     return MCX_OK;
   }
   HIP_TRY(hipSetDevice(g->device));
-  const uint32_t G = g->pending_l2 ? g->b1 : std::min(flush_group(g), g->l2_regions);
+  uint32_t G = g->pending_l2 ? g->b1 : std::min(flush_group(g), g->l2_regions);
+  if (g->l2_hi && !g->pending_l2) G = std::min(G, g->l2_half_regions);
   if (g->pending_l2 && g->l2_regions < g->b1) return fail(MCX_ERR_ARG, "internal: split tuples without bins");
   const bool overlap = flush_overlap(g) && g->pending && !g->pending_l2 && g->l2_regions >= 2 * G && G < g->b1;
+  g->flush_narrow = narrow_capable(g) && !g->window_wide && !g->pending_l2;
+  NarrowOff narrow_off{g};
   hipStream_t s1 = g->stream;
   if (overlap) {
     int rc2 = ensure_flush_stream(g);
@@ -977,8 +1040,9 @@
         in.seg_group = ng;
         in.seg_stride = g->b1;
         in.set_rep = g->nsets > 1 ? g->rep1 : 0;
-        BinSpec bs{BIN_SUBLOCAL, 0, g->subs_per_bin, 1, ng * g->subs_per_bin, ng, 0, r0};
-        BinOut out{l2_ptr(g, g->l2_off), nullptr, g->l2_cnt + g->l2_off, g->cap2, nullptr, nullptr, nullptr, 0};
+        BinSpec bs{BIN_SUBLOCAL, 0, g->subs_per_bin, 1, ng * g->subs_per_bin, ng, 0, r0, 0};
+        if (g->flush_narrow) { bs.nlocal = 2 * g->subs_per_bin; bs.nmain = g->subs_per_bin; }
+        const BinOut out = l2_out(g);
         DISPATCH_WC(g, launch_split_regions, g, in, colour, bs, out);
         HIP_TRY(hipGetLastError());
       }
@@ -999,6 +1063,7 @@
   if (g->pending) HIP_TRY(hipMemsetAsync(g->l1_cnt, 0, (size_t)g->nsets * g->b1 * g->rep1 * 8, g->stream));
   g->pending = 0;
   g->pending_l2 = 0;
+  g->window_wide = false;
   g->n_flushes++;
   g->idle_next = 0; g->idle_base = 0; g->idle_mark.clear();
   sets_release(g);
@@ -1074,7 +1139,7 @@
   }
 }
 
-static int defer_reserve(mcx_graph *g, int colour, uint64_t ub, int *set_out = nullptr)
+static int defer_reserve(mcx_graph *g, int colour, uint64_t ub, int *set_out = nullptr, bool kmerised = false)
 {
   if (set_out) *set_out = 0;
   int rc = ensure_defer(g);
@@ -1086,6 +1151,7 @@
     for (uint32_t s = 0; s < g->nsets; s++) {
       if (g->set_colour[s] == colour && g->set_pending[s] + ub <= g->set_cap) {
         g->set_pending[s] += ub; g->pending += ub;
+        if (!kmerised) g->window_wide = true;
         if (set_out) *set_out = (int)s;
         return MCX_OK;
       }
@@ -1094,6 +1160,7 @@
     if (free_set >= 0) {
       g->set_colour[free_set] = colour;
       g->set_pending[free_set] = ub; g->pending += ub;
+      if (!kmerised) g->window_wide = true;
       if (set_out) *set_out = free_set;
       return MCX_OK;
     }
@@ -1143,7 +1210,7 @@
     if (room < (uint64_t)kTile * 16 && room < L.pos_hi - lo) room = g->set_cap;
     const uint64_t hi = std::min(L.pos_hi, lo + room);
     int set = 0;
-    int rc = defer_reserve(g, colour, hi - lo, &set);
+    int rc = defer_reserve(g, colour, hi - lo, &set, true);
     if (rc != MCX_OK) return rc;
     StreamLaunch P = L;
     P.pos_lo = lo; P.pos_hi = hi;
@@ -1198,6 +1265,12 @@
     g->l2_base = g->l2_keys = nk;
     return MCX_OK;
   }
+  if (!strcmp(key, "narrow_tuples")) {
+    int rc = flush_deferred(g);
+    if (rc != MCX_OK) return rc;
+    g->narrow = value != 0;
+    return MCX_OK;
+  }
   if (!strcmp(key, "place_bins")) {
     if (value < 1 || value > 32) return fail(MCX_ERR_ARG, "place_bins: 1..32");
     g->place_tries = (int)value;
@@ -1409,6 +1482,15 @@
     lo += cnt;
   }
   return MCX_OK;
+}
+
+extern "C" int mcx_graph_tuple_bytes(const mcx_graph *g)
+{
+  if (!g) return fail(MCX_ERR_ARG, "null graph");
+  if (g->as_group) return 8;
+  const bool bins = g->defer && g->t.lb1 >= 6 && (1u << g->t.lb1) <= (uint32_t)kMaxBins && g->t.spb <= (uint32_t)kMaxBins;
+  const bool cap_ok = !g->l1_keys || g->cap2 % 6 == 0;
+  return bins && g->narrow && g->t.sub_s && g->W == 1 && split_wide_blocks() && cap_ok && 2 * g->t.spb <= (uint32_t)kMaxBins ? 6 : 8;
 }
 
 extern "C" int mcx_debug_probe(void *d_buf, uint64_t cap_words, uint32_t nregions, uint32_t spb, uint32_t iters, uint32_t jit_mask, float *ms_out)
@@ -1515,7 +1597,7 @@
   if (!g->defer) return fail(MCX_ERR_ARG, "tuple segments need the deferred insert path (table too small or defer=0)");
   const uint64_t ub = std::min<uint64_t>((uint64_t)nseg * seg_cap, g->set_cap);
   int set = 0;
-  rc = defer_reserve(g, colour, ub, &set);
+  rc = defer_reserve(g, colour, ub, &set, false);
   if (rc != MCX_OK) return rc;
   TupleIn in{(const uint64_t *)d_keys, (const uint8_t *)d_edges, (const unsigned long long *)d_counts, seg_cap, nseg, nseg, nseg};
   BinSpec bs{BIN_GROUP, 0, g->b1, g->rep1, g->b1, 1, 0, 0};
@@ -1706,7 +1788,7 @@
   if (!g->defer) return fail(MCX_ERR_ARG, "super-k-mer records need the deferred insert path (table too small or defer=0)");
   int set = 0;
   const uint64_t ub = std::min(kmers_upper_bound, g->set_cap);
-  rc = defer_reserve(g, colour, ub, &set);
+  rc = defer_reserve(g, colour, ub, &set, true);
   if (rc != MCX_OK) return rc;
   SuperkIn in{d_recs, (const unsigned long long *)d_counts, seg_cap, nseg};
   BinSpec bs{BIN_GROUP, 0, g->b1, g->rep1, g->b1, 1, 0, 0};
@@ -1967,7 +2049,8 @@
   const int mode = mode_env == 3 ? 2 : mode_env;
   const bool on = mode != 0;
   if (!on || !g->defer || g->group || g->nsets != 1 || !g->pending || g->pending_l2 || g->set_colour.empty() || g->set_colour[0] < 0) return MCX_OK;
-  const uint32_t G = std::min(flush_group(g), g->l2_regions);
+  uint32_t G = std::min(flush_group(g), g->l2_regions);
+  if (g->l2_hi) G = std::min(G, g->l2_half_regions);
   if (G >= g->b1) return MCX_OK;
   const uint32_t ngroups = (g->b1 + G - 1) / G;
   if (mode != 2 && g->pending / ngroups < std::max<uint64_t>(g->defer_tuples / 8 / ngroups, 1ull << 24)) return MCX_OK;
@@ -1979,9 +2062,12 @@
   const uint32_t ng = std::min(G, g->b1 - r0);
   const int colour = g->set_colour[0];
   g->l2_off = 0;
+  g->flush_narrow = narrow_capable(g) && !g->window_wide;
+  NarrowOff narrow_off{g};
   TupleIn in{g->l1_keys + (uint64_t)r0 * g->cap1 * g->W, nullptr, g->l1_cnt + r0, g->cap1, ng * g->rep1, ng, g->b1};
-  BinSpec bs{BIN_SUBLOCAL, 0, g->subs_per_bin, 1, ng * g->subs_per_bin, ng, 0, r0};
-  BinOut out{g->l2_keys, nullptr, g->l2_cnt, g->cap2, nullptr, nullptr, nullptr, 0};
+  BinSpec bs{BIN_SUBLOCAL, 0, g->subs_per_bin, 1, ng * g->subs_per_bin, ng, 0, r0, 0};
+  if (g->flush_narrow) { bs.nlocal = 2 * g->subs_per_bin; bs.nmain = g->subs_per_bin; }
+  const BinOut out = l2_out(g);
   DISPATCH_WC(g, launch_split_regions, g, in, colour, bs, out);
   HIP_TRY(hipGetLastError());
   DISPATCH_WC(g, launch_lds_insert_t, g, colour, r0 * g->subs_per_bin, ng * g->subs_per_bin);
diff --git a/mccortex_amd/csrc/mcx_defer.h b/mccortex_amd/csrc/mcx_defer.h
--- a/mccortex_amd/csrc/mcx_defer.h
+++ b/mccortex_amd/csrc/mcx_defer.h
@@ -14,6 +14,7 @@
   uint32_t seg_mod;
   uint32_t lb1;
   uint32_t region0;
+  uint32_t nmain;
 };
 
 __device__ __forceinline__ uint32_t out_seg(const BinSpec &bs, uint32_t ob0, uint32_t b)
@@ -32,6 +33,9 @@
   uint8_t *ov_edges;
   unsigned long long *ov_counts;
   uint64_t ov_cap;
+  unsigned long long *odd_counts;
+  uint64_t odd_cap;
+  uint64_t ncap;
 };
 
 #define MCX_LDS_AS __attribute__((address_space(3)))
@@ -64,6 +68,34 @@
   return q;
 }
 
+constexpr uint32_t kNarrowQlBits = 44;
+MCX_HD bool edges_two_flank(uint32_t e)
+{
+  return ((0x0116u >> (e & 15u)) & (0x0116u >> ((e >> 4) & 15u)) & 1u) != 0;
+}
+MCX_HD uint64_t narrow_pack(uint64_t ql, uint32_t e)
+{
+  const uint32_t code = (uint32_t)__builtin_ctz(e & 15u) | (((uint32_t)__builtin_ctz(e & 0xF0u) - 4u) << 2);
+  return ql | (uint64_t)code << kNarrowQlBits;
+}
+MCX_HD uint32_t narrow_edges(uint64_t v)
+{
+  const uint32_t c = (uint32_t)(v >> kNarrowQlBits) & 15u;
+  return (1u << (c & 3u)) | (16u << (c >> 2));
+}
+MCX_HD uint64_t narrow_unpack(uint64_t v, uint32_t sub_s, uint32_t sub_qlb, uint32_t local)
+{
+  const uint64_t ql = v & ((1ull << kNarrowQlBits) - 1ull);
+  return ((uint64_t)sub_qh_of(sub_s, local, ql) << sub_qlb) | ql | (uint64_t)narrow_edges(v) << 56;
+}
+__device__ __forceinline__ void narrow_store(uint64_t *base, uint64_t at, uint64_t v)
+{
+  unsigned char *p = reinterpret_cast<unsigned char *>(base) + at * 6u;
+  const bool odd = at & 1u;
+  *reinterpret_cast<uint32_t *>(p + (odd ? 2 : 0)) = odd ? (uint32_t)(v >> 16) : (uint32_t)v;
+  *reinterpret_cast<uint16_t *>(p + (odd ? 0 : 4)) = odd ? (uint16_t)v : (uint16_t)(v >> 32);
+}
+
 constexpr int kRounds = 2;
 constexpr int kStage = kTile / kRounds;
 
@@ -93,7 +125,7 @@
 
 template <int NB, int T = kThreads> struct BinRes { unsigned long long g0[(NB + T - 1) / T]; };
 
-template <class LDS, int NB>
+template <class LDS, int NB, bool NARROW = false>
 __device__ __forceinline__ void bin_reserve(LDS &L, const BinSpec &bs, const BinOut &out, uint32_t ob0, BinRes<NB, LDS::geo::kT> &res,
                                             bool trash_beyond = false)
 {
@@ -141,6 +173,9 @@
     res.g0[q] = 0;
     if (b < bs.nlocal) {
       const uint32_t c = L.cnt[b];
+      if (NARROW) {
+        if (c) res.g0[q] = atomicAdd(b < bs.nmain ? &out.counts[ob0 + b] : &out.odd_counts[ob0 + b - bs.nmain], (unsigned long long)c);
+      } else
       if (c) res.g0[q] = atomicAdd(&out.counts[out_seg(bs, ob0, b)], (unsigned long long)c);
     }
   }
@@ -148,19 +183,24 @@
 
 constexpr unsigned long long kDstMask = (1ULL << 48) - 1;
 
-template <class LDS, int NB>
+template <class LDS, int NB, bool NARROW = false>
 __device__ __forceinline__ void bin_commit(LDS &L, const BinSpec &bs, const BinOut &out, uint32_t ob0, const BinRes<NB, LDS::geo::kT> &res)
 {
   constexpr int kT = LDS::geo::kT;
+  const unsigned long long seg_len = NARROW ? out.cap / 3u * 4u : out.cap;
 #pragma unroll
   for (int q = 0; q < (NB + kT - 1) / kT; q++) {
     const uint32_t b = (uint32_t)q * kT + threadIdx.x;
     if (b < bs.nlocal) {
       const uint32_t o0 = L.off[b], o1 = L.off[b + 1];
       const unsigned long long g0 = res.g0[q];
-      const unsigned long long room = out.cap > g0 ? out.cap - g0 : 0;
+      const bool odd = NARROW && b >= bs.nmain;
+      const unsigned long long seg_room = odd ? out.odd_cap : NARROW ? out.ncap : out.cap;
+      const unsigned long long room = seg_room > g0 ? seg_room - g0 : 0;
       const uint32_t lim = o0 + (uint32_t)min((unsigned long long)(o1 - o0), room);
-      const unsigned long long dst = ((unsigned long long)out_seg(bs, ob0, b) * out.cap + g0 - o0) & kDstMask;
+      const unsigned long long seg0 = odd ? ((unsigned long long)(ob0 + b - bs.nmain) + 1u) * out.cap - out.odd_cap
+                                          : (unsigned long long)(NARROW ? ob0 + b : out_seg(bs, ob0, b)) * seg_len;
+      const unsigned long long dst = (seg0 + g0 - o0) & kDstMask;
       L.gbase[b] = dst | ((unsigned long long)lim << 48);
     }
   }
@@ -183,10 +223,10 @@
   if (FULL) L.se[q] = (uint8_t)e;
 }
 
-template <int W, bool ONECOL, bool FULL, int SH, class LDS>
+template <int W, bool ONECOL, bool FULL, int SH, class LDS, bool NARROW = false>
 __device__ __forceinline__ void bin_writeout(LDS &L, int round, const BinSpec &bs, const BinOut &out, uint32_t ob0,
                                              uint32_t region_of_seg, const InsertSink<W, ONECOL> &isink,
-                                             uint32_t &novel, uint32_t &full)
+                                             uint32_t &novel, uint32_t &full, uint64_t ql_mask = 0)
 {
   __syncthreads();
   const uint32_t n = L.off[bs.nlocal];
@@ -196,10 +236,14 @@
   auto emit = [&](uint32_t p, uint32_t b, unsigned long long gb, uint64_t t0, uint64_t t1) {
     if (p < (uint32_t)(gb >> 48)) {
       const uint64_t at = (gb + p) & kDstMask;
-      uint64_t *kd = out.keys + at * W;
-      kd[0] = t0;
-      if (W == 2) kd[1] = t1;
-      if (FULL) out.edges[at] = L.se[p - lo];
+      if (NARROW && b < bs.nmain) {
+        narrow_store(out.keys, at, narrow_pack(t0 & ql_mask, (uint32_t)(t0 >> 56)));
+      } else {
+        uint64_t *kd = out.keys + at * W;
+        kd[0] = t0;
+        if (W == 2) kd[1] = t1;
+        if (FULL) out.edges[at] = L.se[p - lo];
+      }
     } else if (FULL || bs.mode == BIN_OWNER) {
       full = 2;
     } else {
@@ -333,7 +377,7 @@
     uint32_t *s_inv = s_inv_h[H == 1 ? 0 : tid_blk / kThreads];
     MCX_PH(6) MCX_PH_COUNT
     tile_stage<PK>(a_arg, pre, tid, s_code, s_inv);
-    for (uint32_t b = tid_blk; b < bs.nlocal + 64; b += T) { L.cnt[b] = 0; L.rnk[b] = 0; }
+    for (uint32_t b = tid_blk; b < bs.nlocal + 64; b += T) L.cnt[b] = 0;
     if (tid < 4) { s_code[kChunks + tid] = 0; s_inv[kChunks / 2 + tid] = 0xFFFFFFFFu; }
     {
       const uint64_t tn = tile + (uint64_t)gridDim.x * H;
@@ -422,8 +466,7 @@
         } else {
           key = canonical<W>(fw, rc, o);
         }
-        const uint32_t o4 = o << 2;
-        const uint32_t e = (nb << (nuc_next | o4)) | (pb << ((prev_nuc ^ 7u) ^ o4));
+        const uint32_t e = edge_byte(nb, pb, nuc_next, prev_nuc, o);
         if (FULL) {
           uint32_t h2;
           kmer_hash<W>(key, 0, &h2);
@@ -512,7 +555,7 @@
   return (uint64_t)q * in.seg_stride + seg % in.seg_group;
 }
 
-template <int W, bool ONECOL, int NB, bool IN_FULL, bool SHARD, int T = kThreads, int R = kRounds, int P = 16>
+template <int W, bool ONECOL, int NB, bool IN_FULL, bool SHARD, int T = kThreads, int R = kRounds, int P = 16, bool NARROW = false>
 __global__ __launch_bounds__(T, (W == 1 || T > kThreads ? 4 : 3)) void k_tuples_bin(TupleIn in, BinSpec bs, BinOut out,
                                                                          InsertSink<W, ONECOL> isink_arg, Counters *ctr)
 {
@@ -523,8 +566,10 @@
   __shared__ InsertSink<W, ONECOL> isink;
   if (threadIdx.x == 0) isink = isink_arg;
   __syncthreads();
+  static_assert(!NARROW || (W == 1 && !IN_FULL), "narrow output: packed one-word tuples");
   const uint32_t t_spb = isink_arg.t.spb, t_lb1 = isink_arg.t.lb1, t_lbq = isink_arg.t.lb1 + isink_arg.t.lbo, t_part = isink_arg.t.part;
-  const int tid = threadIdx.x;
+  const uint32_t t_subs = isink_arg.t.sub_s, t_qlb = isink_arg.t.sub_qlb;
+  const int tid_blk = threadIdx.x;
   uint32_t n_novel = 0, full = 0;
   const uint64_t chunks_per_seg = (in.seg_cap + kTile - 1) / kTile;
   const bool xcd = bs.mode == BIN_SUBLOCAL && gridDim.x % 8 == 0 && bs.seg_mod % 8 == 0 && in.nseg % bs.seg_mod == 0;
@@ -560,6 +605,7 @@
     if (cnt > in.seg_cap) cnt = in.seg_cap;
     if (start >= cnt) continue;
     const uint32_t n = (uint32_t)min((uint64_t)kTile, cnt - start);
+    const int tid = NARROW ? (int)tid_now() : tid_blk;
     const uint32_t lregion = bs.mode == BIN_SUBLOCAL ? seg % bs.seg_mod : 0;
     const uint32_t region = bs.region0 + lregion;
     const uint32_t ob0 = (bs.mode == BIN_SUBLOCAL ? lregion * t_spb : 0) + (blockIdx.x % bs.rep) * bs.nout;
@@ -628,8 +674,9 @@
           okm &= ~(1u << q);
         }
       } else {
-        hb = sub_hash<W>(tuple_q<W>(tk[q]));
-        loc[q] = __umulhi(hb, t_spb);
+        hb = 0;
+        loc[q] = sub_local_of<W>(t_spb, t_subs, t_qlb, tuple_q<W>(tk[q]));
+        if (NARROW && !edges_two_flank((uint32_t)(tk[q].w[0] >> 56))) loc[q] += bs.nmain;
       }
       if (loc[q] >= bs.nlocal) loc[q] = bs.nlocal - 1;
       loc[q] = (okm >> q & 1u) ? loc[q] : trash;
@@ -638,18 +685,18 @@
     }
     MCX_PH(1)
     BinRes<NB, T> res;
-    bin_reserve<LDS, NB>(L, bs, out, ob0, res, true);
+    bin_reserve<LDS, NB, NARROW>(L, bs, out, ob0, res, true);
     MCX_PH(2)
 #pragma unroll
     for (int q = 0; q < PER; q++)
       loc[q] |= bin_rank<LDS>(L, loc[q]) << 16;
-    bin_commit<LDS, NB>(L, bs, out, ob0, res);
+    bin_commit<LDS, NB, NARROW>(L, bs, out, ob0, res);
     MCX_PH(3)
     for (int round = 0; round < R; round++) {
 #pragma unroll
       for (int q = 0; q < PER; q++)
         bin_place<W, false, LDS>(L, round, loc[q] >> 16, loc[q] & 0xffffu, tk[q], 0);
-      bin_writeout<W, ONECOL, false, 0, LDS>(L, round, bs, out, ob0, region, isink, n_novel, full);
+      bin_writeout<W, ONECOL, false, 0, LDS, NARROW>(L, round, bs, out, ob0, region, isink, n_novel, full, (1ull << t_qlb) - 1ull);
       if (round == 0) { MCX_PH(4) } else { MCX_PH(5) }
     }
   }
@@ -934,7 +981,7 @@
   }
 }
 
-template <int W, bool ONECOL>
+template <int W, bool ONECOL, bool NARROW = false>
 __global__ __launch_bounds__(LdsCfg<W>::kThreads, LdsCfg<W>::kMinWaves) void k_lds_insert(TableView t, uint32_t col, BinOut bins,
                                                                        uint32_t sub0, uint32_t nsub, Counters *ctr)
 {
@@ -950,7 +997,7 @@
   if (tid == 0) s_nq = 0;
 
   auto next_bin = [&](uint32_t from) {
-    while (from < nsub && bins.counts[from] == 0) from += gridDim.x;
+    while (from < nsub && bins.counts[from] == 0 && (!NARROW || bins.odd_counts[from] == 0)) from += gridDim.x;
     return from;
   };
   uint32_t bi = next_bin(blockIdx.x);
@@ -958,15 +1005,30 @@
   const bool zeros_known = t.touch && t.touch[0] == 0;
   constexpr bool kPrefetch = LdsCfg<W>::kPrefetch;
   if (kPrefetch && bi < nsub) slice_fetch<W, ONECOL, kLdsThreads>(t, sub0 + bi, col, tid, v, zeros_known);
-  auto idx = [&](int q) -> uint32_t { return (uint32_t)q * kLdsThreads + tid; };
+  static_assert(!NARROW || (W == 1 && kLdsBatch % 2 == 0), "narrow tuples: one-word keys, loaded in pairs");
+  auto idx = [&](int q) -> uint32_t {
+    return NARROW ? 2u * ((uint32_t)(q >> 1) * kLdsThreads + tid) + (uint32_t)(q & 1) : (uint32_t)q * kLdsThreads + tid;
+  };
   auto load_batch_of = [&](uint32_t bin, uint64_t nfill, uint64_t j0, Kmer<W> (&tk)[kLdsBatch]) {
     const uint64_t *kin = bins.keys + (uint64_t)bin * bins.cap * W;
+    if constexpr (NARROW) {
+#pragma unroll
+      for (int q = 0; q < kLdsBatch; q += 2) {
+        uint64_t i = j0 + idx(q);
+        i = i < nfill ? i : 0;
+        const uint32_t *d = reinterpret_cast<const uint32_t *>(reinterpret_cast<const unsigned char *>(kin) + i * 6u);
+        const uint32_t d0 = d[0], d1 = d[1], d2 = d[2];
+        tk[q].w[0] = (uint64_t)d0 | (uint64_t)d1 << 32;
+        tk[q + 1].w[0] = d2;
+      }
+    } else {
 #pragma unroll
     for (int q = 0; q < kLdsBatch; q++) {
       uint64_t i = j0 + idx(q);
       i = i < nfill ? i : 0;
       tk[q].w[0] = kin[i * W];
       if (W == 2) tk[q].w[W - 1] = kin[i * W + 1];
+    }
     }
   };
   constexpr uint64_t kStep = (uint64_t)kLdsThreads * kLdsBatch;
@@ -976,11 +1038,13 @@
     const uint32_t region = sub / t.spb;
     MCX_PH(6) MCX_PH_COUNT
     uint64_t n = bins.counts[bi];
-    if (n > bins.cap) n = bins.cap;
+    if (n > (NARROW ? bins.ncap : bins.cap)) n = NARROW ? bins.ncap : bins.cap;
+    uint64_t n_odd = NARROW ? (uint64_t)bins.odd_counts[bi] : 0;
+    if (n_odd > bins.odd_cap) n_odd = bins.odd_cap;
     const uint32_t nb = next_bin(bi + gridDim.x);
     __syncthreads();
     MCX_PH(0)
-    if (tid == 0) bins.counts[bi] = 0;
+    if (tid == 0) { bins.counts[bi] = 0; if (NARROW) bins.odd_counts[bi] = 0; }
     if (!kPrefetch) slice_fetch<W, ONECOL, kLdsThreads>(t, sub, col, tid, v, zeros_known);
     slice_to_lds<W, ONECOL, kLdsThreads>(lds, tid, v);
     __syncthreads();
@@ -998,21 +1062,33 @@
       if (!lds_apply<W>(lds, key, bucket, e, n_novel, full))
         probe_insert<W, ONECOL>(t, key, ovf_start<W>(t, key), 0, 0, e, col, n_novel, full, true);
     };
+    auto apply_one = [&](const Kmer<W> &tp) {
+      Kmer<W> key;
+      uint32_t bucket, e;
+      unpack(tp, key, bucket, e);
+      if (!lds_try<W>(lds, key, bucket, e, n_novel)) {
+        const uint32_t qi = atomicAdd(&s_nq, 1u);
+        if (qi < kQueueCap) {
+          queue[qi * W] = tp.w[0];
+          if (W == 2) queue[qi * W + 1] = tp.w[W - 1];
+        } else {
+          apply_slow(key, bucket, e);
+        }
+      }
+    };
+    const uint32_t local = sub & (t.spb - 1u);
     auto apply_batch = [&](uint64_t j0, const Kmer<W> (&tk)[kLdsBatch]) {
 #pragma unroll
       for (int q = 0; q < kLdsBatch; q++)
         if (j0 + idx(q) < n) {
-          Kmer<W> key;
-          uint32_t bucket, e;
-          unpack(tk[q], key, bucket, e);
-          if (!lds_try<W>(lds, key, bucket, e, n_novel)) {
-            const uint32_t qi = atomicAdd(&s_nq, 1u);
-            if (qi < kQueueCap) {
-              queue[qi * W] = tk[q].w[0];
-              if (W == 2) queue[qi * W + 1] = tk[q].w[W - 1];
-            } else {
-              apply_slow(key, bucket, e);
-            }
+          if constexpr (NARROW) {
+            const uint64_t a = tk[q & ~1].w[0], b = tk[q | 1].w[0];
+            const uint64_t v = (q & 1) ? (a >> 48) | (b << 16) : a & ((1ull << 48) - 1ull);
+            Kmer<W> tp;
+            tp.w[0] = narrow_unpack(v, t.sub_s, t.sub_qlb, local);
+            apply_one(tp);
+          } else {
+            apply_one(tk[q]);
           }
         }
     };
@@ -1020,12 +1096,23 @@
       Kmer<W> ta[kLdsBatch], tb[kLdsBatch];
       load_batch(0, ta);
       load_batch(kStep, tb);
+      const uint64_t *odd = bins.keys + ((uint64_t)bi + 1u) * bins.cap * W - bins.odd_cap * W;
+      Kmer<W> to;
+      if constexpr (NARROW) to.w[0] = odd[(uint64_t)tid < n_odd ? tid : 0];
       if (decltype(has_next)::value) slice_fetch<W, ONECOL, kLdsThreads>(t, sub0 + nb, col, tid, v, zeros_known);
       for (uint64_t j0 = 0; j0 < n; j0 += 2 * kStep) {
         apply_batch(j0, ta);
         load_batch(j0 + 2 * kStep, ta);
         apply_batch(j0 + kStep, tb);
         load_batch(j0 + 3 * kStep, tb);
+      }
+      if constexpr (NARROW) {
+        if ((uint64_t)tid < n_odd) apply_one(to);
+        for (uint64_t j = (uint64_t)kLdsThreads + tid; j < n_odd; j += kLdsThreads) {
+          Kmer<W> tp;
+          tp.w[0] = odd[j];
+          apply_one(tp);
+        }
       }
     };
     if (kPrefetch && nb < nsub) run(std::true_type{}); else run(std::false_type{});
diff --git a/mccortex_amd/csrc/mcx_kernels.h b/mccortex_amd/csrc/mcx_kernels.h
--- a/mccortex_amd/csrc/mcx_kernels.h
+++ b/mccortex_amd/csrc/mcx_kernels.h
@@ -28,6 +28,7 @@
   uint64_t *val;
   uint64_t VC;
   uint32_t *touch;
+  uint32_t sub_s, sub_qlb;
 };
 constexpr int kTouchHdr = 32;
 __device__ __forceinline__ void table_mark_written(const TableView &t)
@@ -140,15 +141,47 @@
 }
 __device__ __host__ __forceinline__ uint32_t lbq_of(const TableView &t) { return t.lb1 + t.lbo; }
 
+MCX_HD uint32_t edge_byte(uint32_t nb, uint32_t pb, uint32_t nuc_next, uint32_t prev_nuc, uint32_t o)
+{
+  const uint32_t o4 = o << 2;
+  return (nb << (nuc_next | o4)) | (pb << ((prev_nuc ^ 7u) ^ o4));
+}
+MCX_HD uint32_t sub_bij_bits(int words, int k, uint32_t lbq, uint32_t spb, uint32_t *qlb)
+{
+  *qlb = 0;
+  if (words != 1 || spb < 2 || (spb & (spb - 1u))) return 0;
+  uint32_t s = 0;
+  while ((1u << s) < spb) s++;
+  const int nq = 2 * k - (int)lbq;
+  if (nq - (int)s < 1 || nq - (int)s + 4 > 48) return 0;
+  *qlb = (uint32_t)(nq - (int)s);
+  return s;
+}
+MCX_HD uint32_t mulhi32(uint32_t a, uint32_t b) { return (uint32_t)(((uint64_t)a * b) >> 32); }
+template <int W> __device__ __host__ __forceinline__ uint32_t sub_local_of(uint32_t spb, uint32_t sub_s, uint32_t sub_qlb, const Kmer<W> &q)
+{
+  if (W == 1 && sub_s) {
+    Kmer<W> l = q;
+    l.w[0] = q.w[0] & ((1ull << sub_qlb) - 1ull);
+    return ((uint32_t)(q.w[0] >> sub_qlb) ^ (sub_hash<W>(l) >> (32u - sub_s))) & (spb - 1u);
+  }
+  return mulhi32(sub_hash<W>(q), spb);
+}
+MCX_HD uint32_t sub_qh_of(uint32_t sub_s, uint32_t local, uint64_t ql)
+{
+  Kmer<1> l;
+  l.w[0] = ql;
+  return local ^ (sub_hash<1>(l) >> (32u - sub_s));
+}
+
 struct TableAddr { uint32_t G, region, sub, bucket; };
 template <int W> __device__ __forceinline__ TableAddr addr_of(const TableView &t, const Kmer<W> &q, uint32_t r)
 {
-  const uint32_t b = sub_hash<W>(q);
   const uint32_t lbq = lbq_of(t), m = region_mix<W>(q);
   TableAddr a;
   a.G = r ^ mix_g(m, lbq);
   a.region = a.G & ((1u << t.lb1) - 1u);
-  a.sub = a.region * t.spb + __umulhi(b, t.spb);
+  a.sub = a.region * t.spb + sub_local_of<W>(t.spb, t.sub_s, t.sub_qlb, q);
   a.bucket = mix_bucket(m, lbq, Sub<W>::kBuckets);
   return a;
 }
diff --git a/mccortex_amd/csrc/mcx_streamfc.h b/mccortex_amd/csrc/mcx_streamfc.h
--- a/mccortex_amd/csrc/mcx_streamfc.h
+++ b/mccortex_amd/csrc/mcx_streamfc.h
@@ -160,8 +160,7 @@
         const uint64_t f = ((uint64_t)fh << 32) | fl, r = ((uint64_t)rh << 32) | rl;
         const uint32_t o = f < r ? 0u : 1u;
         const uint64_t sel = f < r ? f : r;
-        const uint32_t o4 = o << 2;
-        const uint32_t e = (nb << (nuc_next | o4)) | (pb << ((prev_nuc ^ 7u) ^ o4));
+        const uint32_t e = edge_byte(nb, pb, nuc_next, prev_nuc, o);
         const uint64_t kk = sel >> key_sh;
         Kmer<W> q;
         q.w[0] = kk >> lbq;
diff --git a/mccortex_amd/graph.py b/mccortex_amd/graph.py
--- a/mccortex_amd/graph.py
+++ b/mccortex_amd/graph.py
@@ -19,7 +19,7 @@
     "mcx_graph_partition_stream_dev", "mcx_graph_insert_tuples_dev", "mcx_key_owner", "mcx_graph_sync",
     "mcx_graph_nkmers", "mcx_graph_device_stats", "mcx_graph_stream", "mcx_graph_export",
     "mcx_kmer_from_str", "mcx_kmer_canonical", "mcx_kmer_hash", "mcx_pack_bases", "mcx_pack_reads_host", "mcx_pack_stream_dev", "mcx_graph_add_packed_dev",
-    "mcx_ubench_stream", "mcx_ubench_random_rmw", "mcx_graph_insert_stats", "mcx_multi_exchange_bytes", "mcx_graph_hashtest", "mcx_hashtest_func", "mcx_debug_probe",
+    "mcx_ubench_stream", "mcx_ubench_random_rmw", "mcx_graph_insert_stats", "mcx_graph_tuple_bytes", "mcx_multi_exchange_bytes", "mcx_graph_hashtest", "mcx_hashtest_func", "mcx_debug_probe",
     "mcx_graph_infer_edges", "mcx_graph_infer_edges_dev", "mcx_graph_unitig_stats", "mcx_graph_clean",
     "mcx_graph_unitigs", "mcx_graph_unitigs_dev", "mcx_graph_pop_bubbles",
     "mcx_graph_subgraph_begin", "mcx_graph_subgraph_seed_reads", "mcx_graph_subgraph_seed_stream_dev", "mcx_graph_subgraph_finish",
@@ -133,6 +133,7 @@
     L.mcx_graph_add_records.argtypes = [vp, vp, C.c_uint64, C.c_int, vp, vp, C.c_int, C.c_uint32, C.POINTER(RecordStats)]
     L.mcx_graph_kmer_covg.argtypes = [vp, u64p, u64p]
     L.mcx_graph_insert_stats.argtypes = [vp, vp]
+    L.mcx_graph_tuple_bytes.argtypes = [vp]
     L.mcx_graph_covg_histogram.argtypes = [vp, u64p, C.c_uint32]
     L.mcx_sort_records.argtypes = [vp, C.c_uint64, C.c_int, C.c_int, C.c_int]
     L.mcx_records_sorted.argtypes = [vp, C.c_uint64, C.c_int, C.c_int, C.c_int, C.POINTER(C.c_int64)]
@@ -458,6 +459,12 @@
         _check(self.L.mcx_graph_insert_stats(self.h, st))
         return dict(zip(("fallback_inserts", "foreign_inserts", "spilled", "flushes"), (int(x) for x in st)))
 
+    def tuple_bytes(self):
+        rc = self.L.mcx_graph_tuple_bytes(self.h)
+        if rc < 0:
+            _check(rc)
+        return int(rc)
+
     @property
     def stream(self):
         return self.L.mcx_graph_stream(self.h)
```

Result: slower. 103.0 billion (-1.1%).
